# 10XGenomics/thermite

Measured on AMD Instinct MI355X. Metric: aligned reads/sec (91 bp), higher is better.
Workload: dtype i32

## Files before the change

### thermite_amd/capi.py

```python
import ctypes as C
import os

import numpy as np

from .refdata import EXON_DT, REF_DT, SPAN_DT, TX_DT

_HERE = os.path.dirname(os.path.abspath(__file__))
SO_PATH = os.environ.get("THM_LIB") or os.path.join(_HERE, "_build", "libthermite_amd.so")

MEM_DT = np.dtype([("ref_idx", "<u8"), ("query_idx", "<u4"), ("len", "<u4")])
ALN_DT = np.dtype(
    [
        ("ystart", "<u8"),
        ("yend", "<u8"),
        ("ylen", "<u8"),
        ("ops_off", "<u8"),
        ("tx_ystart", "<u8"),
        ("tx_yend", "<u8"),
        ("tx_ylen", "<u8"),
        ("tx_ops_off", "<u8"),
        ("score", "<i4"),
        ("ref_id", "<u4"),
        ("xstart", "<u4"),
        ("xend", "<u4"),
# ... 142 lines not shown
        return _lib
    if not os.path.exists(SO_PATH):
        raise ThermiteError(ERR_INTERNAL, "HIP library not built: %s is missing (run __graft_entry__.build())" % SO_PATH)
    L = C.CDLL(SO_PATH)
    vp, u64, i32, u32 = C.c_void_p, C.c_uint64, C.c_int32, C.c_uint32
    L.thm_index_create_in_memory.restype = i32
    L.thm_index_create_in_memory.argtypes = [vp, u64, vp, u32, vp, u32, vp, u64, vp, u64, vp, u32, vp, u32, vp, vp]
    L.thm_index_create_in_memory_ex.restype = i32
    L.thm_index_create_in_memory_ex.argtypes = [vp, u64, vp, u32, vp, u32, vp, u64, vp, u64, vp, u32, vp, u32, vp, u32, u32, vp]
    L.thm_index_coord_bytes.restype = u32
    L.thm_index_coord_bytes.argtypes = [vp]
    L.thm_index_suffix_array64.restype = vp
    L.thm_index_suffix_array64.argtypes = [vp]
    L.thm_build_suffix_array64.restype = i32
    L.thm_build_suffix_array64.argtypes = [vp, u64, vp]
    L.thm_build_suffix_array_gpu.restype = i32
    L.thm_build_suffix_array_gpu.argtypes = [vp, u64, vp, u32]
    if hasattr(L, "thm_debug_check_lut"):
        L.thm_debug_check_lut.restype = i32
        L.thm_debug_check_lut.argtypes = [vp]
    if hasattr(L, "thm_debug_host_lut"):
        L.thm_debug_host_lut.restype = i32
        L.thm_debug_host_lut.argtypes = [vp, vp, vp, u64]
    L.thm_index_free.argtypes = [vp]
    L.thm_index_text_len.restype = u64
    L.thm_index_text_len.argtypes = [vp]
    L.thm_index_suffix_array.restype = vp
    L.thm_index_suffix_array.argtypes = [vp]
    L.thm_index_idx_to_ref.restype = i32
    L.thm_index_idx_to_ref.argtypes = [vp, u64, vp]
    L.thm_build_suffix_array.restype = i32
    L.thm_build_suffix_array.argtypes = [vp, u64, vp]
    L.thm_aligner_create.restype = i32
    L.thm_aligner_create.argtypes = [vp, vp, i32, vp]
    L.thm_aligner_free.argtypes = [vp]
    L.thm_last_error.restype = C.c_char_p
    L.thm_last_error.argtypes = [vp]
    L.thm_aligner_set_opts.restype = i32
    L.thm_aligner_set_opts.argtypes = [vp, vp]
    L.thm_aligner_stream.restype = vp
    L.thm_aligner_stream.argtypes = [vp]
    L.thm_align_batch.restype = i32
    L.thm_align_batch.argtypes = [vp, vp, vp, u64, vp]
    L.thm_batch_upload.restype = i32
    L.thm_batch_upload.argtypes = [vp, vp, vp, u64]
    for f in ("thm_batch_run", "thm_batch_sync", "thm_counters_reset"):
        getattr(L, f).restype = i32
        getattr(L, f).argtypes = [vp]
    L.thm_batch_fetch.restype = i32
    L.thm_batch_fetch.argtypes = [vp, vp]
    L.thm_batch_fetch_cigars.restype = i32
    L.thm_batch_fetch_cigars.argtypes = [vp, vp]
    L.thm_align_batch_cigars.restype = i32
    L.thm_align_batch_cigars.argtypes = [vp, vp, vp, u64, vp]
    L.thm_cigar_encode_batch.restype = i32
    L.thm_cigar_encode_batch.argtypes = [vp, vp, vp, u64, vp]
    L.thm_smems_batch.restype = i32
    L.thm_smems_batch.argtypes = [vp, vp, vp, u64, u64, vp]
    L.thm_swg_extend_batch.restype = i32
    L.thm_swg_extend_batch.argtypes = [vp, vp, vp, vp, vp, vp, vp, u32, u64, vp]
    L.thm_counters_get.restype = i32
    L.thm_extend_left_right_batch.restype = i32
    L.thm_extend_left_right_batch.argtypes = [vp, vp, vp, vp, vp, vp, vp, vp, u32, u64, vp]
    L.thm_align_seed_hits_batch.restype = i32
    L.thm_align_seed_hits_batch.argtypes = [vp, vp, vp, u64, vp, vp, u64, vp, vp, u32, vp]
    L.thm_counters_get.argtypes = [vp, vp]
    L.thm_counters_device_ptr.restype = vp
    L.thm_counters_device_ptr.argtypes = [vp]
    L.thm_timings_get.restype = i32
    L.thm_timings_get.argtypes = [vp, vp]
    L.thm_version.restype = C.c_char_p
    L.thm_device_count.restype = i32
    L.thm_aligner_index.restype = vp
    L.thm_aligner_index.argtypes = [vp]
    L.thm_comm_unique_id.restype = i32
    L.thm_comm_unique_id.argtypes = [vp]
    L.thm_comm_create.restype = i32
    L.thm_comm_create.argtypes = [vp, i32, i32, i32, vp]
    L.thm_comm_free.argtypes = [vp]
    L.thm_counters_allreduce.restype = i32
    L.thm_counters_allreduce.argtypes = [vp, vp]
    cp = C.c_char_p
    L.thm_index_create_from_files.restype = i32
    L.thm_index_create_from_files.argtypes = [cp, cp, vp]
    L.thm_index_set_names.restype = i32
    L.thm_index_set_names.argtypes = [vp, vp, u32, vp, u32, vp, vp, u32]
    L.thm_index_save.restype = i32
    L.thm_index_save.argtypes = [vp, cp]
    L.thm_index_load.restype = i32
    L.thm_index_load.argtypes = [cp, vp]
    L.thm_index_tables.restype = i32
    L.thm_index_tables.argtypes = [vp, vp]
    for f in ("thm_index_contig_name", "thm_index_tx_id", "thm_index_gene_id", "thm_index_gene_name"):
        getattr(L, f).restype = cp
        getattr(L, f).argtypes = [vp, u32]
    L.thm_fastq_open.restype = i32
    L.thm_fastq_open.argtypes = [cp, vp]
    L.thm_fastq_next_batch.restype = i32
    L.thm_fastq_next_batch.argtypes = [vp, u64, vp]
    L.thm_fastq_close.argtypes = [vp]
    if hasattr(L, "thm_debug_deflate_block"):
        L.thm_debug_deflate_block.restype = i32
        L.thm_debug_deflate_block.argtypes = [vp, u64, vp, u64, C.POINTER(u64)]
    if hasattr(L, "thm_debug_gunzip_mt"):
        L.thm_debug_gunzip_mt.restype = i32
        L.thm_debug_gunzip_mt.argtypes = [C.c_char_p, u64, u32, vp, u64, C.POINTER(u64)]
    if hasattr(L, "thm_debug_gunzip"):
        L.thm_debug_gunzip.restype = i32
        L.thm_debug_gunzip.argtypes = [C.c_char_p, u64, vp, u64, C.POINTER(u64)]
    if hasattr(L, "thm_debug_fastq_blocks"):
        L.thm_debug_fastq_blocks.restype = i32
        L.thm_debug_fastq_blocks.argtypes = [vp, u64, vp]
    L.thm_writer_create.restype = i32
    L.thm_writer_create.argtypes = [vp, i32, u32, vp]
    L.thm_writer_free.argtypes = [vp]
    L.thm_writer_header.restype = i32
    L.thm_writer_header.argtypes = [vp, vp]
    L.thm_writer_trailer.restype = i32
    L.thm_writer_trailer.argtypes = [vp, vp]
    L.thm_writer_format_batch.restype = i32
    L.thm_writer_format_batch.argtypes = [vp, vp, vp, vp]
    L.thm_writer_format_batch_cigars.restype = i32
    L.thm_writer_format_batch_cigars.argtypes = [vp, vp, vp, vp]
    L.thm_batch_upload_reads.restype = i32
    L.thm_batch_upload_reads.argtypes = [vp, vp]
    L.thm_batch_fetch_bam.restype = i32
    L.thm_batch_fetch_bam.argtypes = [vp, u32, vp]
    L.thm_align_batch_bam.restype = i32
    L.thm_align_batch_bam.argtypes = [vp, vp, u32, vp]
    L.thm_batch_fetch_bgzf.restype = i32
    L.thm_batch_fetch_bgzf.argtypes = [vp, u32, vp]
    L.thm_align_batch_bgzf.restype = i32
    L.thm_align_batch_bgzf.argtypes = [vp, vp, u32, vp]
    L.thm_debug_bgzf_device.restype = i32
    L.thm_debug_bgzf_device.argtypes = [vp, vp, u64, vp, u64, vp, vp]
    L.thm_batch_upload_fastq.restype = i32
    L.thm_batch_upload_fastq.argtypes = [vp, vp, u64, cp, u64, i32, vp]
    L.thm_batch_fetch_reads.restype = i32
    L.thm_batch_fetch_reads.argtypes = [vp, vp]
    L.thm_debug_fastq_device_blocks.restype = i32
    L.thm_debug_fastq_device_blocks.argtypes = [vp, vp, vp]
    L.thm_writer_wrap_bam.restype = i32
    L.thm_writer_wrap_bam.argtypes = [vp, vp, vp]
    L.thm_align_files.restype = i32
    L.thm_align_files.argtypes = [vp, vp, u32, cp, i32, u64, u32, vp]
    L.thm_align_files_multi.restype = i32
    L.thm_align_files_multi.argtypes = [vp, u32, vp, u32, cp, i32, u64, u32, vp]
    if hasattr(L, "thm_debug_prof_get"):
        L.thm_debug_prof_get.restype = i32
        L.thm_debug_prof_get.argtypes = [vp, vp, i32]
    if hasattr(L, "thm_debug_set_pool_caps"):
        L.thm_debug_set_pool_caps.restype = i32
        L.thm_debug_set_pool_caps.argtypes = [vp, u64, u64, u64, vp]
    if hasattr(L, "thm_debug_set_flags"):
        L.thm_debug_set_flags.restype = i32
        L.thm_debug_set_flags.argtypes = [vp, C.c_uint32]
        L.thm_debug_set_band_clip.restype = i32
        L.thm_debug_set_band_clip.argtypes = [vp, C.c_uint32]
        L.thm_debug_tpr_stats.restype = i32
        L.thm_debug_tpr_stats.argtypes = [vp, vp]
    if hasattr(L, "thm_debug_seed_stats"):
        L.thm_debug_seed_stats.restype = i32
        L.thm_debug_seed_stats.argtypes = [vp, vp]
    if hasattr(L, "thm_debug_seed_direct_stats"):
        L.thm_debug_seed_direct_stats.restype = i32
        L.thm_debug_seed_direct_stats.argtypes = [vp, vp]
    if hasattr(L, "thm_debug_fetch_lut"):
        L.thm_debug_fetch_lut.restype = i32
        L.thm_debug_fetch_lut.argtypes = [vp, vp, u64]
    if hasattr(L, "thm_debug_knobs"):
        L.thm_debug_knobs.restype = i32
        L.thm_debug_knobs.argtypes = [vp, vp]
    if hasattr(L, "thm_debug_calib_gather"):
        L.thm_debug_calib_gather.restype = i32
        L.thm_debug_calib_gather.argtypes = [vp, i32, u64, vp]
    if hasattr(L, "thm_debug_wave_prims"):
        L.thm_debug_wave_prims.restype = i32
        L.thm_debug_wave_prims.argtypes = [vp, vp, vp]
    _lib = L
    return L


def _ptr(a):
    return a.ctypes.data_as(C.c_void_p) if a is not None else None


def _copy(ptr, count, dtype, copy=True):
    if count == 0 or not ptr:
        return np.zeros(0, dtype=dtype)
    nbytes = int(count) * np.dtype(dtype).itemsize
    buf = (C.c_uint8 * nbytes).from_address(ptr)
    a = np.frombuffer(buf, dtype=dtype, count=int(count))
    return a.copy() if copy else a


def _u8(b):
    if isinstance(b, np.ndarray):
        return np.ascontiguousarray(b, np.uint8)
    return np.frombuffer(bytes(b), np.uint8)


def build_suffix_array_gpu(text, wide=False):
    text = np.ascontiguousarray(text, np.uint8)
    out = np.empty(len(text), "<u8" if wide else "<u4")
    rc = lib().thm_build_suffix_array_gpu(_ptr(text), len(text), _ptr(out), 8 if wide else 4)
    if rc != 0:
        raise ThermiteError(rc, _last_error())
    return out


def build_suffix_array(text, wide=False):
    t = _u8(text)
    sa = np.zeros(len(t), "<u8" if wide else "<u4")
    f = lib().thm_build_suffix_array64 if wide else lib().thm_build_suffix_array
    rc = f(_ptr(t), len(t), _ptr(sa))
    if rc != 0:
        raise ThermiteError(rc, "thm_build_suffix_array")
    return sa


INDEX_WIDE = 1


class TablesView(C.Structure):
    _fields_ = [("n_text", C.c_uint64), ("text", C.c_void_p), ("n_refs", C.c_uint32), ("refs", C.c_void_p),
                ("n_txs", C.c_uint32), ("txs", C.c_void_p), ("n_exons", C.c_uint64), ("exons", C.c_void_p),
                ("n_tx_seq", C.c_uint64), ("tx_seq", C.c_void_p), ("n_genes", C.c_uint32), ("genes", C.c_void_p),
                ("name_rank", C.c_void_p), ("n_contigs", C.c_uint32)]


class ReadBatch(C.Structure):

    _fields_ = [("n_reads", C.c_uint64), ("n_bases", C.c_uint64), ("bases", C.c_void_p), ("offsets", C.c_void_p),
                ("quals", C.c_void_p), ("names", C.c_void_p), ("name_off", C.c_void_p)]


class Text(C.Structure):
    _fields_ = [("data", C.c_void_p), ("len", C.c_uint64)]


class RunStats(C.Structure):
    _fields_ = [("n_reads", C.c_uint64), ("n_aligned_reads", C.c_uint64), ("n_records", C.c_uint64),
                ("n_batches", C.c_uint64), ("n_output_bytes", C.c_uint64), ("parse_s", C.c_double),
                ("gpu_s", C.c_double), ("format_s", C.c_double), ("write_s", C.c_double), ("wall_s", C.c_double)]


def _last_error(h=None):
    return (lib().thm_last_error(h) or b"").decode()


def _cstr_array(strs):
    arr = (C.c_char_p * len(strs))(*[s.encode() if isinstance(s, str) else bytes(s) for s in strs])
    return arr


class Index:

    @classmethod
    def _wrap(cls, h):
        self = cls.__new__(cls)
        self.h = h
        self.tables = None
        return self

    @classmethod
    def from_files(cls, fasta_path, gtf_path):
        h = C.c_void_p()
        rc = lib().thm_index_create_from_files(str(fasta_path).encode(), str(gtf_path).encode(), C.byref(h))
        if rc != 0:
            raise ThermiteError(rc, _last_error())
        return cls._wrap(h)

    @classmethod
    def load(cls, path):
        h = C.c_void_p()
        rc = lib().thm_index_load(str(path).encode(), C.byref(h))
        if rc != 0:
            raise ThermiteError(rc, _last_error())
        return cls._wrap(h)

    def save(self, path):
        rc = lib().thm_index_save(self.h, str(path).encode())
        if rc != 0:
            raise ThermiteError(rc, _last_error())

    def set_names(self, contig_names, tx_ids, gene_ids, gene_names):
        a, b, c, d = (_cstr_array(x) for x in (contig_names, tx_ids, gene_ids, gene_names))
        rc = lib().thm_index_set_names(self.h, a, len(contig_names), b, len(tx_ids), c, d, len(gene_ids))
        if rc != 0:
            raise ThermiteError(rc, _last_error())

    def native_tables(self):
        v = TablesView()
        rc = lib().thm_index_tables(self.h, C.byref(v))
        if rc != 0:
            raise ThermiteError(rc, "thm_index_tables")
        L = lib()
        dec = lambda f, n: [f(self.h, i).decode() for i in range(n)]
        names = dec(L.thm_index_contig_name, v.n_contigs)
        refs = _copy(v.refs, v.n_refs, REF_DT)
        rank_per_ref = _copy(v.name_rank, v.n_refs, "<u4")
        name_rank = np.zeros(v.n_contigs, "<u4")
        if v.n_contigs:
            name_rank[refs["name_id"]] = rank_per_ref
        have = v.n_contigs > 0
        return dict(
            text=_copy(v.text, v.n_text, np.uint8), refs=refs, names=names, name_rank=name_rank,
            txs=_copy(v.txs, v.n_txs, TX_DT), exons=_copy(v.exons, v.n_exons, EXON_DT),
            tx_seq=_copy(v.tx_seq, v.n_tx_seq, np.uint8), genes=_copy(v.genes, v.n_genes, SPAN_DT),
            gene_ids=dec(L.thm_index_gene_id, v.n_genes) if have else [],
            gene_names=dec(L.thm_index_gene_name, v.n_genes) if have else [],
            tx_ids=dec(L.thm_index_tx_id, v.n_txs) if have else [],
        )

    def __init__(self, tables, sa=None, wide=False):
        t = tables
        self.tables = t
        h = C.c_void_p()
        sa_arr, sa_bytes = None, 0
        if sa is not None:
            sa_bytes = 8 if np.asarray(sa).dtype.itemsize == 8 else 4
            sa_arr = np.ascontiguousarray(sa, "<u8" if sa_bytes == 8 else "<u4")
        rc = lib().thm_index_create_in_memory_ex(
            _ptr(t["text"]), len(t["text"]), _ptr(t["refs"]), len(t["refs"]), _ptr(t["txs"]), len(t["txs"]),
            _ptr(t["exons"]), len(t["exons"]), _ptr(t["tx_seq"]), len(t["tx_seq"]), _ptr(t["genes"]), len(t["genes"]),
            _ptr(t["name_rank"]), len(t["name_rank"]), _ptr(sa_arr), sa_bytes, INDEX_WIDE if wide else 0, C.byref(h),
        )
        if rc != 0:
            raise ThermiteError(rc, (lib().thm_last_error(None) or b"").decode())
        self.h = h
        if t.get("names") and "tx_ids" in t:
            self.set_names(t["names"], t["tx_ids"], t["gene_ids"], t["gene_names"])

    @property
    def coord_bytes(self):
        return lib().thm_index_coord_bytes(self.h)

    def suffix_array(self):
        n = lib().thm_index_text_len(self.h)
        if self.coord_bytes == 8:
            return _copy(lib().thm_index_suffix_array64(self.h), n, "<u8")
        return _copy(lib().thm_index_suffix_array(self.h), n, "<u4")

    def check_lut(self):
        return lib().thm_debug_check_lut(self.h) == 0

    def debug_host_lut(self):
        kt = C.c_uint32()
        if lib().thm_debug_host_lut(self.h, C.byref(kt), None, 0) != 0:
            raise ThermiteError(ERR_INTERNAL, "thm_debug_host_lut")
        out = np.zeros((4 ** kt.value, 2), "<u8" if self.coord_bytes == 8 else "<u4")
        if lib().thm_debug_host_lut(self.h, C.byref(kt), _ptr(out), out.nbytes) != 0:
            raise ThermiteError(ERR_INTERNAL, "thm_debug_host_lut")
        return out

    def idx_to_ref(self, idx):
        off = C.c_uint64()
        r = lib().thm_index_idx_to_ref(self.h, idx, C.byref(off))
        if r < 0:
            raise ThermiteError(r, "idx_to_ref")
        return r, off.value

    def close(self):
        if getattr(self, "h", None):
            lib().thm_index_free(self.h)
            self.h = None

    def __del__(self):
        self.close()


class BatchResult:

    def __init__(self, view, copy=True):
        self.n_reads = view.n_reads
        self.offsets = _copy(view.read_aln_off, view.n_reads + 1, "<u8", copy)
        self.alns = _copy(view.alns, view.n_alns, ALN_DT, copy)
        self.ops = _copy(view.ops, view.n_op_bytes, np.uint8, copy)
        self.n_failed = view.n_failed_reads
        self.status = _copy(view.read_status, view.n_reads, "<i4", copy) if view.read_status else None


class CigarResult:

    def __init__(self, view, copy=True):
        self.n_reads = view.n_reads
        self.offsets = _copy(view.read_aln_off, view.n_reads + 1, "<u8", copy) if view.read_aln_off else None
        self.alns = _copy(view.alns, view.n_alns, ALN_DT, copy) if view.alns else None
        self.digests = _copy(view.digests, view.n_alns, DIGEST_DT, copy)
        self.cigar = _copy(view.cigar, view.n_cigar_words, "<u4", copy)
        self.n_failed = view.n_failed_reads
        self.status = _copy(view.read_status, view.n_reads, "<i4", copy) if view.read_status else None

    @property
    def nbytes(self):
        return sum(a.nbytes for a in (self.offsets, self.alns, self.digests, self.cigar, self.status) if a is not None)

    def words(self, i, tx=False):
        d = self.digests[i]
        o = int(d["cigar_off"]) + (int(d["n_cigar"]) if tx else 0)
        return self.cigar[o: o + int(d["n_tx_cigar"] if tx else d["n_cigar"])]


class BamResult:

    def __init__(self, view, copy=True):
        self.n_reads = view.n_reads
        self.n_records = view.n_records
        self.data = _copy(view.data, view.n_bytes, np.uint8, copy)
        self.read_rec_off = _copy(view.read_rec_off, view.n_reads + 1, "<u8", copy)
        self.n_failed = view.n_failed_reads
        self.status = _copy(view.read_status, view.n_reads, "<i4", copy) if view.read_status else None

    @property
    def nbytes(self):
        return sum(a.nbytes for a in (self.data, self.read_rec_off, self.status) if a is not None)

    def records(self, r):
        b = self.data[int(self.read_rec_off[r]): int(self.read_rec_off[r + 1])].tobytes()
        out, at = [], 0
        while at < len(b):
            n = 4 + int.from_bytes(b[at: at + 4], "little")
            out.append(b[at: at + n])
            at += n
        return out


class BgzfResult:

    def __init__(self, view, copy=True):
        self.n_reads = view.n_reads
        self.n_records = view.n_records
        self.n_raw_bytes = view.n_raw_bytes
        self.n_blocks = view.n_blocks
        self.data = _copy(view.data, view.n_bytes, np.uint8, copy)
        self.block_off = _copy(view.block_off, view.n_blocks + 1, "<u8", copy)
        self.n_failed = view.n_failed_reads
        self.status = _copy(view.read_status, view.n_reads, "<i4", copy) if view.read_status else None

    @property
    def nbytes(self):
        return sum(a.nbytes for a in (self.data, self.block_off, self.status) if a is not None)

    def block(self, b):
        return self.data[int(self.block_off[b]): int(self.block_off[b + 1])].tobytes()


def cigar_text(words):
    return "".join("%d%s" % (int(w) >> 4, "MIDNSHP=X"[int(w) & 15]) for w in words) or "*"


class Aligner:

    def __init__(self, index, opts=None, device=0):
        self.index = index
        o = dict(DEFAULT_OPTS)
        o.update(opts or {})
        self._opts = self._mk(o)
        h = C.c_void_p()
        rc = lib().thm_aligner_create(index.h, C.byref(self._opts), device, C.byref(h))
        if rc != 0:
            raise ThermiteError(rc, (lib().thm_last_error(None) or b"").decode())
        self.h = h

    @staticmethod
    def _mk(o):
        return Opts(o["min_seed_len"], o["min_aln_score_percent"], o["min_aln_score"], o["multimap_score_range"],
                    int(bool(o["intron_mode"])), 0)

    def _chk(self, rc):
        if rc != 0:
            raise ThermiteError(rc, (lib().thm_last_error(self.h) or b"").decode())

    def set_opts(self, opts):
        o = dict(DEFAULT_OPTS)
        o.update(opts)
        self._opts = self._mk(o)
        self._chk(lib().thm_aligner_set_opts(self.h, C.byref(self._opts)))

    @property
    def stream(self):
        return lib().thm_aligner_stream(self.h)

    def align_batch(self, bases, offsets, copy=True):
        bases, offsets = _u8(bases), np.ascontiguousarray(offsets, "<u8")
        v = BatchView()
        self._chk(lib().thm_align_batch(self.h, _ptr(bases), _ptr(offsets), len(offsets) - 1, C.byref(v)))
        return BatchResult(v, copy)

    def upload(self, bases, offsets):
        bases, offsets = _u8(bases), np.ascontiguousarray(offsets, "<u8")
        self._chk(lib().thm_batch_upload(self.h, _ptr(bases), _ptr(offsets), len(offsets) - 1))

    def run(self):
        self._chk(lib().thm_batch_run(self.h))

    def sync(self):
        self._chk(lib().thm_batch_sync(self.h))

    def fetch(self, copy=True):
        v = BatchView()
        self._chk(lib().thm_batch_fetch(self.h, C.byref(v)))
        return BatchResult(v, copy)

    def fetch_cigars(self, copy=True):
        v = CigarView()
        self._chk(lib().thm_batch_fetch_cigars(self.h, C.byref(v)))
        return CigarResult(v, copy)

    def align_batch_cigars(self, bases, offsets, copy=True):
        bases, offsets = _u8(bases), np.ascontiguousarray(offsets, "<u8")
        v = CigarView()
        self._chk(lib().thm_align_batch_cigars(self.h, _ptr(bases), _ptr(offsets), len(offsets) - 1, C.byref(v)))
        return CigarResult(v, copy)

    def upload_reads(self, batch):
        rb, keep = read_batch_struct(batch)
        self._chk(lib().thm_batch_upload_reads(self.h, C.byref(rb)))

    def fetch_bam(self, flags=0, copy=True):
        v = BamView()
        self._chk(lib().thm_batch_fetch_bam(self.h, flags, C.byref(v)))
        return BamResult(v, copy)

    def align_batch_bam(self, batch, flags=0, copy=True):
        rb, keep = read_batch_struct(batch)
        v = BamView()
        self._chk(lib().thm_align_batch_bam(self.h, C.byref(rb), flags, C.byref(v)))
        return BamResult(v, copy)

    def fetch_bgzf(self, flags=0, copy=True):
        v = BgzfView()
        self._chk(lib().thm_batch_fetch_bgzf(self.h, flags, C.byref(v)))
        return BgzfResult(v, copy)

    def align_batch_bgzf(self, batch, flags=0, copy=True):
        rb, keep = read_batch_struct(batch)
        v = BgzfView()
        self._chk(lib().thm_align_batch_bgzf(self.h, C.byref(rb), flags, C.byref(v)))
        return BgzfResult(v, copy)

    def upload_fastq(self, raw, path=b"", first_line=1, last_block=True):
        src = np.frombuffer(bytes(raw), np.uint8) if len(raw) else None
        info = FastqUploadInfo()
        self._chk(lib().thm_batch_upload_fastq(self.h, _ptr(src), len(raw), os.fsencode(path), first_line, int(bool(last_block)),
                                               C.byref(info)))
        return {k: getattr(info, k) for k, _ in FastqUploadInfo._fields_}

    def fetch_reads(self):
        v = ReadBatch()
        self._chk(lib().thm_batch_fetch_reads(self.h, C.byref(v)))
        off = _copy(v.offsets, v.n_reads + 1, "<u8")
        noff = _copy(v.name_off, v.n_reads + 1, "<u8")
        return dict(bases=_copy(v.bases, v.n_bases, np.uint8), offsets=off,
                    quals=_copy(v.quals, v.n_bases, np.uint8) if v.quals else None,
                    names=_copy(v.names, int(noff[-1]), np.uint8), name_off=noff)

    def debug_fastq_device_blocks(self):
        d, h = C.c_uint64(0), C.c_uint64(0)
        self._chk(lib().thm_debug_fastq_device_blocks(self.h, C.byref(d), C.byref(h)))
        return d.value, h.value

    def debug_bgzf_device(self, data):
        src = np.frombuffer(bytes(data), np.uint8) if len(data) else np.zeros(1, np.uint8)
        out = np.empty(len(data) + 31 * (len(data) // 0xff00 + 1) + 64, np.uint8)
        n, nb = C.c_uint64(0), C.c_uint64(0)
        self._chk(lib().thm_debug_bgzf_device(self.h, src.ctypes.data, len(data), out.ctypes.data, len(out), C.byref(n), C.byref(nb)))
        return out[: n.value].tobytes(), nb.value

    def cigar_encode_batch(self, ops, off):
        ops, off = _u8(ops), np.ascontiguousarray(off, "<u8")
        v = CigarView()
        self._chk(lib().thm_cigar_encode_batch(self.h, _ptr(ops), _ptr(off), len(off) - 1, C.byref(v)))
        return CigarResult(v)

    def smems_batch(self, bases, offsets, min_seed_len):
        bases, offsets = _u8(bases), np.ascontiguousarray(offsets, "<u8")
        v = MemsView()
        self._chk(lib().thm_smems_batch(self.h, _ptr(bases), _ptr(offsets), len(offsets) - 1, min_seed_len, C.byref(v)))
        return _copy(v.read_mem_off, v.n_reads + 1, "<u8"), _copy(v.mems, v.n_mems, MEM_DT)

    def swg_extend_batch(self, x_bases, x_off, y_bases, y_off, bw, xd, max_bw):
        xb, yb = _u8(x_bases), _u8(y_bases)
        xo, yo = np.ascontiguousarray(x_off, "<u8"), np.ascontiguousarray(y_off, "<u8")
        bw, xd = np.ascontiguousarray(bw, "<u4"), np.ascontiguousarray(xd, "<i4")
        v = SwgView()
        self._chk(lib().thm_swg_extend_batch(self.h, _ptr(xb), _ptr(xo), _ptr(yb), _ptr(yo), _ptr(bw), _ptr(xd),
                                             max_bw, len(bw), C.byref(v)))
        return _copy(v.alns, v.n, SWG_DT), _copy(v.ops, v.n_op_bytes, np.uint8)

    def extend_left_right_batch(self, x_bases, x_off, y_bases, y_off, hits, bw, xd, max_bw):
        xb, yb = _u8(x_bases), _u8(y_bases)
        xo, yo = np.ascontiguousarray(x_off, "<u8"), np.ascontiguousarray(y_off, "<u8")
        hits = np.ascontiguousarray(hits, MEM_DT)
        bw, xd = np.ascontiguousarray(bw, "<u4"), np.ascontiguousarray(xd, "<i4")
        v = LrView()
        self._chk(lib().thm_extend_left_right_batch(self.h, _ptr(xb), _ptr(xo), _ptr(yb), _ptr(yo), _ptr(hits), _ptr(bw),
                                                    _ptr(xd), max_bw, len(bw), C.byref(v)))
        return _copy(v.alns, v.n, LR_DT), _copy(v.ops, v.n_op_bytes, np.uint8)

    def align_seed_hits(self, bases, offsets, hit_off, hits, band_width, x_drop, max_band_width):
        bases, offsets = _u8(bases), np.ascontiguousarray(offsets, "<u8")
        hit_off, hits = np.ascontiguousarray(hit_off, "<u8"), np.ascontiguousarray(hits, MEM_DT)
        bw, xd = np.ascontiguousarray(band_width, "<u4"), np.ascontiguousarray(x_drop, "<i4")
        if not (len(hits) == len(bw) == len(xd)):
            raise ThermiteError(ERR_INVALID_ARG, "hits, band_width and x_drop differ in length")
        v = HitsView()
        self._chk(lib().thm_align_seed_hits_batch(self.h, _ptr(bases), _ptr(offsets), len(offsets) - 1, _ptr(hit_off),
                                                  _ptr(hits), len(hits), _ptr(bw), _ptr(xd), max_band_width, C.byref(v)))
        status = (_copy(v.hit_status, v.n_hits, "<i4") if v.hit_status else np.zeros(int(v.n_hits), "<i4"))
        return _copy(v.alns, v.n_hits, ALN_DT), _copy(v.ops, v.n_op_bytes, np.uint8), status

    def counters(self):
        out = np.zeros(N_COUNTERS, "<u8")
        self._chk(lib().thm_counters_get(self.h, _ptr(out)))
        return out

    def reset_counters(self):
        self._chk(lib().thm_counters_reset(self.h))

    def counters_allreduce(self, comm):
        self._chk(lib().thm_counters_allreduce(self.h, comm.h))

    def counters_device_ptr(self):
        return lib().thm_counters_device_ptr(self.h)

    def timings(self):
        out = np.zeros(N_TIMINGS, "<f4")
        self._chk(lib().thm_timings_get(self.h, _ptr(out)))
        return dict(zip(TIMING_NAMES, out.tolist()))

    def debug_prof(self, reset=True):
        out = np.zeros(16, "<u8")
        self._chk(lib().thm_debug_prof_get(self.h, _ptr(out), int(reset)))
        return out

    def debug_set_pool_caps(self, smem_cap=0, cand_cap=0, ops_cap=0):
        n = C.c_uint32()
        self._chk(lib().thm_debug_set_pool_caps(self.h, smem_cap, cand_cap, ops_cap, C.byref(n)))
        return n.value

    def debug_set_flags(self, tpr=None, rounds=0, seed_infer=None, seed_stats=None, seed_direct=None):
        word = (0 if tpr is None else (2 if tpr else 1)) | (int(rounds) << 8)
        word |= 0 if seed_infer is None else (16 if seed_infer else 4)
        word |= 0 if seed_stats is None else (8 if seed_stats else 32)
        word |= 0 if seed_direct is None else (128 if seed_direct else 64)
        self._chk(lib().thm_debug_set_flags(self.h, word))

    def debug_seed_stats(self):
        out = np.zeros(2, "<u8")
        self._chk(lib().thm_debug_seed_stats(self.h, _ptr(out)))
        return int(out[0]), int(out[1])

    def debug_seed_direct_stats(self):
        out = np.zeros(4, "<u8")
        self._chk(lib().thm_debug_seed_direct_stats(self.h, _ptr(out)))
        return tuple(int(x) for x in out)

    def debug_fetch_lut(self, like):
        out = np.zeros_like(like)
        self._chk(lib().thm_debug_fetch_lut(self.h, _ptr(out), out.nbytes))
        return out

    def debug_set_band_clip(self, max_bw=None):
        self._chk(lib().thm_debug_set_band_clip(self.h, 0 if max_bw is None else int(max_bw) + 1))

    def debug_tpr_stats(self):
        out = np.zeros(32, "<u8")
        self._chk(lib().thm_debug_tpr_stats(self.h, _ptr(out)))
        return out

    def debug_knobs(self):
        out = np.zeros(16, "<u4")
        self._chk(lib().thm_debug_knobs(self.h, _ptr(out)))
        return out

    def debug_calib_gather(self, pattern, n_threads):
        b = C.c_uint64()
        self._chk(lib().thm_debug_calib_gather(self.h, pattern, n_threads, C.byref(b)))
        return b.value

    def debug_wave_prims(self, v):
        v = np.ascontiguousarray(v, "<i4")
        out = np.zeros(384, "<i4")
        self._chk(lib().thm_debug_wave_prims(self.h, _ptr(v), _ptr(out)))
        return out.reshape(6, 64)

    def close(self):
        if getattr(self, "h", None):
            lib().thm_aligner_free(self.h)
            self.h = None

    def __del__(self):
        self.close()


KNOB_NAMES = {0: "seed_fill", 1: "compact_k", 2: "hit_gl", 11: "team_div_per_cu", 12: "swg_bpc", 13: "use_tpr", 14: "tpr_rounds",
              15: "n_cu"}


def knobs_dict(raw):
    d = {name: int(raw[i]) for i, name in KNOB_NAMES.items()}
    d["ext_minw"] = {(cpl, bool(wide)): int(raw[3 + 2 * (cpl - 1) + wide]) for cpl in (1, 2, 3, 4) for wide in (0, 1)}
    return d


def comm_unique_id():
    out = np.zeros(128, np.uint8)
    rc = lib().thm_comm_unique_id(_ptr(out))
    if rc != 0:
        raise ThermiteError(rc, _last_error())
    return out


class Comm:

    def __init__(self, unique_id, nranks, rank, device=0):
        uid = np.ascontiguousarray(unique_id, np.uint8)
        h = C.c_void_p()
        rc = lib().thm_comm_create(_ptr(uid), nranks, rank, device, C.byref(h))
        if rc != 0:
            raise ThermiteError(rc, _last_error())
        self.h = h

    def close(self):
        if getattr(self, "h", None):
            lib().thm_comm_free(self.h)
            self.h = None

    def __del__(self):
        self.close()


def debug_deflate_block(data):
    src = np.frombuffer(bytes(data), np.uint8) if len(data) else np.zeros(1, np.uint8)
    out = np.empty(len(data) + len(data) // 8 + 1024, np.uint8)
    n = C.c_uint64(0)
    rc = lib().thm_debug_deflate_block(src.ctypes.data, len(data), out.ctypes.data, len(out), C.byref(n))
    if rc != 0:
        raise ThermiteError(rc, _last_error())
    return out[: n.value].tobytes()


def debug_gunzip(path, chunk=1 << 20, cap=None, threads=1):
    cap = cap if cap is not None else 64 * os.path.getsize(path) + (1 << 20)
    out = np.empty(cap, np.uint8)
    n = C.c_uint64(0)
    rc = lib().thm_debug_gunzip_mt(os.fsencode(str(path)), chunk, threads, out.ctypes.data, cap, C.byref(n))
    if rc != 0:
        raise ThermiteError(rc, _last_error())
    return out[: n.value].tobytes()


class FastqReader:

    def __init__(self, path):
        h = C.c_void_p()
        rc = lib().thm_fastq_open(str(path).encode(), C.byref(h))
        if rc != 0:
            raise ThermiteError(rc, _last_error())
        self.h = h

    def all_by_blocks(self, reads_per_block):
        v = ReadBatch()
        rc = lib().thm_debug_fastq_blocks(self.h, reads_per_block, C.byref(v))
        if rc != 0:
            raise ThermiteError(rc, _last_error())
        off = _copy(v.offsets, v.n_reads + 1, "<u8")
        noff = _copy(v.name_off, v.n_reads + 1, "<u8")
        return dict(bases=_copy(v.bases, v.n_bases, np.uint8), offsets=off, quals=_copy(v.quals, v.n_bases, np.uint8),
                    names=_copy(v.names, int(noff[-1]), np.uint8), name_off=noff)

    def next_batch(self, max_reads):
        v = ReadBatch()
        rc = lib().thm_fastq_next_batch(self.h, max_reads, C.byref(v))
        if rc != 0:
            raise ThermiteError(rc, _last_error())
        if v.n_reads == 0:
            return None
        off = _copy(v.offsets, v.n_reads + 1, "<u8")
        noff = _copy(v.name_off, v.n_reads + 1, "<u8")
        return dict(bases=_copy(v.bases, v.n_bases, np.uint8), offsets=off,
                    quals=_copy(v.quals, v.n_bases, np.uint8) if v.quals else None,
                    names=_copy(v.names, int(noff[-1]), np.uint8), name_off=noff)

    def close(self):
        if getattr(self, "h", None):
            lib().thm_fastq_close(self.h)
            self.h = None

    def __del__(self):
        self.close()


def read_batch_struct(batch):
    keep = [_u8(batch["bases"]), np.ascontiguousarray(batch["offsets"], "<u8"),
            None if batch.get("quals") is None else _u8(batch["quals"]), _u8(batch["names"]),
            np.ascontiguousarray(batch["name_off"], "<u8")]
    rb = ReadBatch(len(keep[1]) - 1, len(keep[0]), _ptr(keep[0]), _ptr(keep[1]), _ptr(keep[2]), _ptr(keep[3]), _ptr(keep[4]))
    return rb, keep


class Writer:

    def __init__(self, index, fmt=FMT_SAM, n_threads=1):
# ... 73 lines not shown
```

### thermite_amd/csrc/aligner.hip

```cpp
#include <hip/hip_runtime.h>

#include <algorithm>
#include <cstdarg>
#include <cstdio>
#include <cstdlib>
#include <cstring>
#include <mutex>
#include <string>
#include <type_traits>
#include <vector>

#include "aligner_internal.h"
#include "lut_direct.h"

namespace thm {
const char* global_error_cstr();
}
using namespace thm;

static int swg_blocks_per_cu() {
  static const int v = [] {
    const char* e = getenv("THM_SWG_BPC");
    const int v = e ? atoi(e) : 4;
    return (v >= 1 && v <= 8) ? v : 4;
// ... 65 lines not shown
    const bool tag = lut_direct_wanted() && (ix->wide ? lutd::can_tag<uint64_t>(ix->n) : lutd::can_tag<uint32_t>(ix->n)) &&
                     (ix->wide ? !ix->lut64.empty() : !ix->lut.empty());
    if (tag) {
      if (e == hipSuccess) e = d->lut_cnt.ensure(16);
      if (e == hipSuccess) e = hipMemsetAsync(d->lut_cnt.p, 0, 16, s);
      if (e == hipSuccess)
        e = ix->wide ? launch_lut_tag(d->lut.as<LutEntryT<uint64_t>>(), d->sa.as<uint64_t>(), ix->lut64.size(), ix->n,
                                      d->lut_cnt.as<unsigned long long>(), s)
                     : launch_lut_tag(d->lut.as<LutEntryT<uint32_t>>(), d->sa.as<uint32_t>(), ix->lut.size(), ix->n,
                                      d->lut_cnt.as<unsigned long long>(), s);
      if (e == hipSuccess) e = hipMemcpyAsync(&d->lut_tagged, d->lut_cnt.p, 8, hipMemcpyDeviceToHost, s);
      d->lut_direct = true;
    }
    if (e == hipSuccess) e = hipStreamSynchronize(s);
    if (e != hipSuccess) {
      free_dev_copy(d);
      return fail(a, e == hipErrorOutOfMemory ? THM_ERR_OOM : THM_ERR_HIP, "index upload failed: %s",
                  hipGetErrorString(e));
    }
    auto fill_view = [&](auto& v) {
      typedef typename std::remove_reference<decltype(v)>::type::coord_t C;
      v.text = d->text.as<uint8_t>() + 16;
      v.sa = d->sa.as<C>();
      v.lut = d->lut.as<LutEntryT<C>>();
      v.refs = d->refs.as<thm_ref>();
      v.name_rank = d->name_rank.as<uint32_t>();
      v.ref_recs = d->ref_recs.as<RefRecT<C>>();
      v.ref_bin = d->ref_bin.as<uint32_t>();
      v.txs = d->txs.as<thm_tx>();
      v.exons = d->exons.as<thm_exon>();
      v.exon_txoff = d->exon_txoff.as<uint64_t>();
      v.tx_seq = d->tx_seq.as<uint8_t>() + 16;
      v.exon_grid_off = d->exon_grid_off.as<uint32_t>();
      v.exon_grid = d->exon_grid.as<ExonEntryT<C>>();
      v.gene_grid_off = d->gene_grid_off.as<uint32_t>();
      v.gene_grid = d->gene_grid.as<GridEntryT<C>>();
      v.n = ix->n;
      v.n_refs = (uint32_t)ix->refs.size();
      v.n_txs = (uint32_t)ix->txs.size();
      v.kt = ix->kt;
      v.max_tx_exons = ix->max_tx_exons;
      v.lut_direct = d->lut_direct ? 1u : 0u;
    };
    memset(&d->view, 0, sizeof d->view);
    memset(&d->view64, 0, sizeof d->view64);
    if (ix->wide)
      fill_view(d->view64);
    else
      fill_view(d->view);
    ix->dev[a->device] = d;
  }
  a->dix = ix->dev[a->device];
  return THM_OK;
}

int reset_queue(thm_aligner* a) {
  HIPCHK(a, hipMemsetAsync(a->d_queue.p, 0, thm::QUEUE_BYTES, a->stream));
  HIPCHK(a, hipMemsetAsync(a->d_fault.p, 0, 64, a->stream));
  return THM_OK;
}

int grid_blocks(const thm_aligner* a, uint64_t n_items, int waves_per_block, int blocks_per_cu) {
  uint64_t need = (n_items + waves_per_block - 1) / waves_per_block;
  uint64_t cap = (uint64_t)a->n_cu * blocks_per_cu;
  return (int)std::max<uint64_t>(1, std::min(need, cap));
}

extern "C" {

const char* thm_version(void) { return "thermite_amd 0.1 (gfx950)"; }

int32_t thm_device_count(void) {
  int n = 0;
  if (hipGetDeviceCount(&n) != hipSuccess) return 0;
  return n;
}

void thm_index_free(thm_index* ix) {
  if (!ix) return;
  for (auto* d : ix->dev) free_dev_copy(d);
  delete (std::mutex*)ix->dev_mu;
  delete ix;
}

const char* thm_last_error(const thm_aligner* a) { return a ? a->err.c_str() : global_error_cstr(); }

int32_t thm_aligner_create(const thm_index* ix, const thm_align_opts* opts, int32_t device_id, thm_aligner** out) {
  if (!out) return THM_ERR_INVALID_ARG;
  *out = nullptr;
  if (!ix || !opts) return fail(nullptr, THM_ERR_INVALID_ARG, "thm_aligner_create: null index or opts");
  int n = 0;
  if (hipGetDeviceCount(&n) != hipSuccess || n <= 0)
    return fail(nullptr, THM_ERR_NO_DEVICE, "no HIP device visible: the MI355X path has no CPU fallback");
  if (device_id < 0 || device_id >= n) return fail(nullptr, THM_ERR_NO_DEVICE, "device id %d out of range", device_id);
  thm_aligner* a = new thm_aligner();
  a->ix = ix;
  a->device = device_id;
  a->opts = *opts;
  {
    const char* e = getenv("THM_TPR");
    if (e && e[0] == '0') a->use_tpr = false;
    if (e && e[0] == '1') a->use_tpr = true;
    e = getenv("THM_TPR_ROUNDS");
    if (e && atoi(e) >= 1 && atoi(e) <= TPR_MAX_ROUNDS) a->tpr_rounds = atoi(e);
  }
  auto bail = [&](int code) {
    thm_aligner_free(a);
    return code;
  };
  if (hipSetDevice(device_id) != hipSuccess) return bail(fail(nullptr, THM_ERR_HIP, "hipSetDevice failed"));
  hipDeviceProp_t prop;
  if (hipGetDeviceProperties(&prop, device_id) == hipSuccess) a->n_cu = prop.multiProcessorCount;
  if (hipStreamCreateWithFlags(&a->stream, hipStreamNonBlocking) != hipSuccess)
    return bail(fail(nullptr, THM_ERR_HIP, "hipStreamCreate failed"));
  for (auto& e : a->ev)
    if (hipEventCreate(&e) != hipSuccess) return bail(fail(nullptr, THM_ERR_HIP, "hipEventCreate failed"));
  if (hipStreamCreateWithFlags(&a->stream2, hipStreamNonBlocking) != hipSuccess ||
      hipStreamCreateWithFlags(&a->stream3, hipStreamNonBlocking) != hipSuccess ||
      hipStreamCreateWithFlags(&a->stream4, hipStreamNonBlocking) != hipSuccess ||
      hipEventCreateWithFlags(&a->ev_dpt_fork, hipEventDisableTiming) != hipSuccess ||
      hipEventCreateWithFlags(&a->ev_dpt_join, hipEventDisableTiming) != hipSuccess ||
      hipEventCreateWithFlags(&a->ev_join3, hipEventDisableTiming) != hipSuccess ||
      hipEventCreateWithFlags(&a->ev_fork, hipEventDisableTiming) != hipSuccess ||
      hipEventCreateWithFlags(&a->ev_join, hipEventDisableTiming) != hipSuccess)
    return bail(fail(nullptr, THM_ERR_HIP, "second stream / events: creation failed"));
  if (a->d_counters.ensure(THM_N_COUNTERS * 8 * 3) != hipSuccess || a->d_ctl.ensure(thm_aligner::CTL_BYTES) != hipSuccess)
    return bail(fail(nullptr, THM_ERR_OOM, "scratch allocation failed"));
  {
    uint8_t* ctl = a->d_ctl.as<uint8_t>();
    a->s_work_counts = {ctl + thm_aligner::CTL_WORK_COUNTS, 128};
    a->d_cursors = {ctl + thm_aligner::CTL_CURSORS, 64};
    a->d_fault = {ctl + thm_aligner::CTL_FAULT, 64};
    a->d_queue = {ctl + thm_aligner::CTL_QUEUE, thm::QUEUE_BYTES};
    a->d_queue_ext = {ctl + thm_aligner::CTL_QUEUE_EXT, thm::QUEUE_BYTES};
  }
  (void)hipMemsetAsync(a->d_counters.p, 0, THM_N_COUNTERS * 8 * 3, a->stream);
  (void)hipMemsetAsync(a->d_ctl.p, 0, thm_aligner::CTL_BYTES, a->stream);
  int rc = get_dev_copy(a);
  if (rc != THM_OK) return bail(rc);
  rc = thm_aligner_set_opts(a, opts);
  if (rc != THM_OK) return bail(rc);
  *out = a;
  return THM_OK;
}

void thm_aligner_free(thm_aligner* a) {
  if (!a) return;
  (void)hipSetDevice(a->device);
  if (a->stream) (void)hipStreamSynchronize(a->stream);
  if (a->stream2) (void)hipStreamSynchronize(a->stream2);
  if (a->stream3) (void)hipStreamSynchronize(a->stream3);
  if (a->stream4) (void)hipStreamSynchronize(a->stream4);
  DBuf* all[] = {&a->d_counters, &a->d_ctl, &a->b0, &a->b1, &a->b2, &a->b3, &a->b4,
                 &a->b5, &a->b6, &a->b7, &a->b8, &a->r_bases, &a->r_offsets, &a->r_san, &a->s_ms_end, &a->s_ms_lo, &a->s_ms_hi, &a->s_work_reads, &a->s_work_long, &a->s_work_cells, &a->s_fill_keys, &a->s_fill_perm, &a->s_fill_hist, &a->s_sel_scratch, &a->s_heavy, &a->s_slow, &a->s_team, &a->r_status, &a->e_slow, &a->e_recs, &a->e_wcnt, &a->t_memos, &a->t_recs, &a->t_dpops, &a->t_qlist, &a->t_act[0], &a->t_act[1], &a->t_ctl, &a->t_bail, &a->t_queue2, &a->t_trace, &a->t_ttrace, &a->t_hdr, &a->t_sums, &a->s_smems, &a->s_off, &a->s_cnt,
                 &a->s_hits, &a->s_cand_off, &a->scan_tmp, &a->e_cands, &a->e_heavy, &a->e_rel, &a->e_order, &a->e_ops, &a->e_nalns,
                 &a->e_opbytes, &a->e_aln_off, &a->e_ops_off, &a->e_trace, &a->o_alns, &a->o_ops, &a->o_mems,
                 &a->sh_bases, &a->sh_san, &a->sh_off, &a->sh_hits, &a->sh_read, &a->sh_bw, &a->sh_xd, &a->sh_list, &a->sh_out,
                 &a->sh_status, &a->sh_ops, &a->sh_ctl, &a->sh_trace, &a->sh_slow, &a->c_sums, &a->c_nwords, &a->c_woff,
                 &a->c_scan_tmp, &a->c_flags, &a->c_dig, &a->c_words, &a->c_in_ops, &a->c_in_off,
                 &a->bn_names, &a->bn_name_off, &a->bn_quals, &a->bt_tx_pool, &a->bt_tx_off, &a->bt_gid_pool, &a->bt_gid_off,
                 &a->bt_gname_pool, &a->bt_gname_off, &a->bt_tx_gene, &a->bt_ref_sq, &a->bm_cnt, &a->bm_first, &a->bm_qn,
                 &a->bm_rec_read, &a->bm_len, &a->bm_off, &a->bm_out, &a->bm_read_off, &a->bm_err, &a->bm_scan_tmp,
                 &a->bz_match, &a->bz_slots, &a->bz_sizes, &a->bz_off, &a->bz_out, &a->bz_scan_tmp, &a->bz_dbg_in,
                 &a->fq_raw, &a->fq_cnt, &a->fq_base, &a->fq_lines, &a->fq_name_len, &a->fq_seq_len, &a->fq_flag, &a->fq_scan_tmp};
  for (DBuf* b : all) b->release();
  for (int k = 0; k < 2; k++) {
    a->r_off[k].release();
    a->r_alns[k].release();
    a->r_ops[k].release();
    a->r_stat[k].release();
    a->ch_off[k].release();
    a->ch_alns[k].release();
    a->ch_dig[k].release();
    a->ch_words[k].release();
    a->ch_stat[k].release();
    a->bh_data[k].release();
    a->bh_off[k].release();
    a->bh_stat[k].release();
    a->zh_data[k].release();
    a->zh_off[k].release();
    a->zh_stat[k].release();
  }
  HBuf* pinned[] = {&a->fq_h_off, &a->fr_bases, &a->fr_off, &a->fr_quals, &a->fr_names, &a->fr_name_off};
  for (HBuf* b : pinned) b->release();
  for (auto& e : a->ev_fq)
    if (e) (void)hipEventDestroy(e);
  for (auto& e : a->ev_cig)
    if (e) (void)hipEventDestroy(e);
  for (auto& e : a->ev_bam)
    if (e) (void)hipEventDestroy(e);
  for (auto& e : a->ev_bgzf)
    if (e) (void)hipEventDestroy(e);
  for (auto& e : a->ev)
    if (e) (void)hipEventDestroy(e);
  if (a->ev_fork) (void)hipEventDestroy(a->ev_fork);
  if (a->ev_join) (void)hipEventDestroy(a->ev_join);
  if (a->ev_join3) (void)hipEventDestroy(a->ev_join3);
  if (a->ev_dpt_fork) (void)hipEventDestroy(a->ev_dpt_fork);
  if (a->ev_dpt_join) (void)hipEventDestroy(a->ev_dpt_join);
  if (a->stream4) (void)hipStreamDestroy(a->stream4);
  if (a->stream3) (void)hipStreamDestroy(a->stream3);
  if (a->stream2) (void)hipStreamDestroy(a->stream2);
  if (a->stream) (void)hipStreamDestroy(a->stream);
  delete a;
}

int32_t thm_aligner_set_opts(thm_aligner* a, const thm_align_opts* o) {
  if (!a || !o) return THM_ERR_INVALID_ARG;
  if (o->min_seed_len < 1 || o->min_seed_len > 65535) return fail(a, THM_ERR_INVALID_ARG, "min_seed_len out of range");
  if (!(o->min_aln_score_percent >= 0.0f && o->min_aln_score_percent <= 1.0f))
    return fail(a, THM_ERR_INVALID_ARG, "min_aln_score_percent must be within [0,1] (src/main.rs:46-49)");
  a->opts = *o;
  return THM_OK;
}

void* thm_aligner_stream(thm_aligner* a) { return a ? (void*)a->stream : nullptr; }

const thm_index* thm_aligner_index(const thm_aligner* a) { return a ? a->ix : nullptr; }

int32_t thm_counters_get(thm_aligner* a, uint64_t out[THM_N_COUNTERS]) {
  if (!a || !out) return THM_ERR_INVALID_ARG;
  HIPCHK(a, hipSetDevice(a->device));
  HIPCHK(a, hipMemcpyAsync(out, a->d_counters.p, THM_N_COUNTERS * 8, hipMemcpyDeviceToHost, a->stream));
  HIPCHK(a, hipStreamSynchronize(a->stream));
  return THM_OK;
}
int32_t thm_counters_reset(thm_aligner* a) {
  if (!a) return THM_ERR_INVALID_ARG;
  HIPCHK(a, hipSetDevice(a->device));
  HIPCHK(a, hipMemsetAsync(a->d_counters.p, 0, THM_N_COUNTERS * 8, a->stream));
  return THM_OK;
}
void* thm_counters_device_ptr(thm_aligner* a) { return a ? a->d_counters.p : nullptr; }

int32_t thm_timings_get(thm_aligner* a, float out[THM_N_TIMINGS]) {
  if (!a || !out) return THM_ERR_INVALID_ARG;
  memcpy(out, a->timings, sizeof(a->timings));
  return THM_OK;
}

int32_t thm_swg_extend_batch(thm_aligner* a, const uint8_t* x_bases, const uint64_t* x_off, const uint8_t* y_bases,
                             const uint64_t* y_off, const uint32_t* band_width, const int32_t* x_drop,
                             uint32_t max_band_width, uint64_t n, thm_swg_view* out) {
  if (!a || !out || !x_off || !y_off || !band_width || !x_drop) return THM_ERR_INVALID_ARG;
  memset(out, 0, sizeof(*out));
  if (n == 0) return THM_OK;
  if (n >= 0xFFFFFFFFull) return fail(a, THM_ERR_UNSUPPORTED, "more than 2^32-1 problems in one call");
  HIPCHK(a, hipSetDevice(a->device));
  uint32_t bw_max = 0, x_max = 0, y_max = 0;
  std::vector<uint64_t> ops_off(n + 1, 0);
  for (uint64_t i = 0; i < n; i++) {
    if (band_width[i] > max_band_width)
      return fail(a, THM_ERR_OUT_OF_CONTRACT, "problem %llu: band_width %u > max_band_width %u (src/swg.rs:32)",
                  (unsigned long long)i, band_width[i], max_band_width);
    if (x_drop[i] < (int64_t)band_width[i])
      return fail(a, THM_ERR_OUT_OF_CONTRACT, "problem %llu: x_drop < band_width is undefined in the reference",
                  (unsigned long long)i);
    uint64_t xl = x_off[i + 1] - x_off[i], yl = y_off[i + 1] - y_off[i];
    if (x_off[i + 1] < x_off[i] || y_off[i + 1] < y_off[i]) return fail(a, THM_ERR_INVALID_ARG, "offsets not monotone");
    if (xl > MAX_READ_LEN || band_width[i] > 2 * MAX_READ_LEN)
      return fail(a, THM_ERR_UNSUPPORTED, "x longer than %u or band wider than +-%u", MAX_READ_LEN, 2 * MAX_READ_LEN);
    uint64_t cols = std::min<uint64_t>(yl, xl + band_width[i] + 1);
    bw_max = std::max(bw_max, band_width[i]);
    x_max = std::max<uint32_t>(x_max, (uint32_t)xl);
    y_max = std::max<uint32_t>(y_max, (uint32_t)cols);
    ops_off[i + 1] = ops_off[i] + xl + cols + 8;
  }
  int cpl = (int)((2 * bw_max + 1 + 63) / 64);
  SwgBatchParams p;
  p.x_cap = (x_max + 15u) & ~15u;
  p.y_cap = (y_max + 15u) & ~15u;
  if (p.x_cap == 0) p.x_cap = 16;
  if (p.y_cap == 0) p.y_cap = 16;
  p.max_bw = bw_max;
  p.scratch = nullptr;
  p.scratch_per_wave = 0;
  if (cpl > 4 || swg_batch_lds_bytes(p, cpl) > EXTEND_LDS_LIMIT) cpl = 0;
  const uint64_t xb_n = x_off[n], yb_n = y_off[n], pool = ops_off[n];
  HIPCHK(a, a->b0.ensure(xb_n + 16));
  HIPCHK(a, a->b1.ensure((n + 1) * 8));
  HIPCHK(a, a->b2.ensure(yb_n + 16));
  HIPCHK(a, a->b3.ensure((n + 1) * 8));
  HIPCHK(a, a->b4.ensure(n * 4));
  HIPCHK(a, a->b5.ensure(n * 4));
  HIPCHK(a, a->b6.ensure((n + 1) * 8));
  HIPCHK(a, a->b7.ensure(pool + 16));
  HIPCHK(a, a->b8.ensure(n * sizeof(thm_swg_aln)));
  hipStream_t s = a->stream;
  if (xb_n) HIPCHK(a, hipMemcpyAsync(a->b0.p, x_bases, xb_n, hipMemcpyHostToDevice, s));
  HIPCHK(a, hipMemcpyAsync(a->b1.p, x_off, (n + 1) * 8, hipMemcpyHostToDevice, s));
  if (yb_n) HIPCHK(a, hipMemcpyAsync(a->b2.p, y_bases, yb_n, hipMemcpyHostToDevice, s));
  HIPCHK(a, hipMemcpyAsync(a->b3.p, y_off, (n + 1) * 8, hipMemcpyHostToDevice, s));
  HIPCHK(a, hipMemcpyAsync(a->b4.p, band_width, n * 4, hipMemcpyHostToDevice, s));
  HIPCHK(a, hipMemcpyAsync(a->b5.p, x_drop, n * 4, hipMemcpyHostToDevice, s));
  HIPCHK(a, hipMemcpyAsync(a->b6.p, ops_off.data(), (n + 1) * 8, hipMemcpyHostToDevice, s));
  int rc = reset_queue(a);
  if (rc != THM_OK) return rc;
  p.xb = a->b0.as<uint8_t>();
  p.xo = a->b1.as<uint64_t>();
  p.yb = a->b2.as<uint8_t>();
  p.yo = a->b3.as<uint64_t>();
  p.bw = a->b4.as<uint32_t>();
  p.xd = a->b5.as<int32_t>();
  p.ops_off = a->b6.as<uint64_t>();
  p.ops = a->b7.as<uint8_t>();
  p.out = a->b8.as<thm_swg_aln>();
  p.counters = a->d_counters.as<unsigned long long>();
// ... 36 lines not shown
  return THM_OK;
}

int32_t thm_extend_left_right_batch(thm_aligner* a, const uint8_t* x_bases, const uint64_t* x_off, const uint8_t* y_bases,
                                    const uint64_t* y_off, const thm_mem* hits, const uint32_t* band_width,
                                    const int32_t* x_drop, uint32_t max_band_width, uint64_t n, thm_lr_view* out) {
  if (!a || !out || !x_off || !y_off || !hits || !band_width || !x_drop) return THM_ERR_INVALID_ARG;
  memset(out, 0, sizeof(*out));
  if (n == 0) return THM_OK;
  if (n >= 0xFFFFFFFFull) return fail(a, THM_ERR_UNSUPPORTED, "more than 2^32-1 problems in one call");
  if ((!x_bases && x_off[n] > 0) || (!y_bases && y_off[n] > 0)) return THM_ERR_INVALID_ARG;
  HIPCHK(a, hipSetDevice(a->device));
  uint32_t bw_max = 0, x_max = 0, y_max = 0;
  std::vector<uint64_t> ops_off(n + 1, 0);
  for (uint64_t i = 0; i < n; i++) {
    if (x_off[i + 1] < x_off[i] || y_off[i + 1] < y_off[i]) return fail(a, THM_ERR_INVALID_ARG, "offsets not monotone");
    const uint64_t xl = x_off[i + 1] - x_off[i], yl = y_off[i + 1] - y_off[i];
    const thm_mem& h = hits[i];
    if (band_width[i] > max_band_width)
      return fail(a, THM_ERR_OUT_OF_CONTRACT, "problem %llu: band_width %u > max_band_width %u (src/swg.rs:32)",
                  (unsigned long long)i, band_width[i], max_band_width);
    if (x_drop[i] < (int64_t)band_width[i])
      return fail(a, THM_ERR_OUT_OF_CONTRACT, "problem %llu: x_drop < band_width is undefined in the reference",
                  (unsigned long long)i);
    if ((uint64_t)h.query_idx + h.len > xl)
      return fail(a, THM_ERR_OUT_OF_CONTRACT, "problem %llu: query_idx + len > read length (src/aligner.rs:360)",
                  (unsigned long long)i);
    if (h.ref_idx > yl || h.ref_idx + h.len > yl)
      return fail(a, THM_ERR_OUT_OF_CONTRACT, "problem %llu: ref_idx + len > reference length (src/aligner.rs:361)",
                  (unsigned long long)i);
    if (xl > MAX_READ_LEN || band_width[i] > 2 * MAX_READ_LEN)
      return fail(a, THM_ERR_UNSUPPORTED, "read longer than %u or band wider than +-%u", MAX_READ_LEN, 2 * MAX_READ_LEN);
    const uint64_t xr = xl - (h.query_idx + h.len), xlft = h.query_idx;
    const uint64_t yr = std::min<uint64_t>(yl - (h.ref_idx + h.len), xr + band_width[i] + 1);
    const uint64_t ylft = std::min<uint64_t>(std::min<uint64_t>(h.ref_idx, xl + band_width[i]), xlft + band_width[i] + 1);
    bw_max = std::max(bw_max, band_width[i]);
    x_max = std::max<uint32_t>(x_max, (uint32_t)std::max(xr, xlft));
    y_max = std::max<uint32_t>(y_max, (uint32_t)std::max(yr, ylft));
    ops_off[i + 1] = ops_off[i] + xr + yr + xlft + ylft + h.len + 16;
  }
  int cpl = (int)((2 * bw_max + 1 + 63) / 64);
  ElrBatchParams p;
  p.x_cap = (x_max + 15u) & ~15u;
  p.y_cap = (y_max + 15u) & ~15u;
  if (p.x_cap == 0) p.x_cap = 16;
  if (p.y_cap == 0) p.y_cap = 16;
  p.max_bw = bw_max;
  p.scratch = nullptr;
  p.scratch_per_wave = 0;
  if (cpl > 4 || elr_batch_lds_bytes(p, cpl) > EXTEND_LDS_LIMIT) cpl = 0;
  const uint64_t xb_n = x_off[n], yb_n = y_off[n], pool = ops_off[n];
  HIPCHK(a, a->b0.ensure(xb_n + 16));
  HIPCHK(a, a->b1.ensure((n + 1) * 8));
  HIPCHK(a, a->b2.ensure(yb_n + 16));
  HIPCHK(a, a->b3.ensure((n + 1) * 8));
  HIPCHK(a, a->b4.ensure(n * 4));
  HIPCHK(a, a->b5.ensure(n * 4));
  HIPCHK(a, a->b6.ensure((n + 1) * 8));
  HIPCHK(a, a->b7.ensure(pool + 16));
  HIPCHK(a, a->b8.ensure(n * sizeof(thm_lr_aln)));
  HIPCHK(a, a->sh_hits.ensure(n * sizeof(thm_mem)));
  hipStream_t s = a->stream;
  if (xb_n) HIPCHK(a, hipMemcpyAsync(a->b0.p, x_bases, xb_n, hipMemcpyHostToDevice, s));
  HIPCHK(a, hipMemcpyAsync(a->b1.p, x_off, (n + 1) * 8, hipMemcpyHostToDevice, s));
  if (yb_n) HIPCHK(a, hipMemcpyAsync(a->b2.p, y_bases, yb_n, hipMemcpyHostToDevice, s));
  HIPCHK(a, hipMemcpyAsync(a->b3.p, y_off, (n + 1) * 8, hipMemcpyHostToDevice, s));
  HIPCHK(a, hipMemcpyAsync(a->b4.p, band_width, n * 4, hipMemcpyHostToDevice, s));
  HIPCHK(a, hipMemcpyAsync(a->b5.p, x_drop, n * 4, hipMemcpyHostToDevice, s));
  HIPCHK(a, hipMemcpyAsync(a->b6.p, ops_off.data(), (n + 1) * 8, hipMemcpyHostToDevice, s));
  HIPCHK(a, hipMemcpyAsync(a->sh_hits.p, hits, n * sizeof(thm_mem), hipMemcpyHostToDevice, s));
  int rc = reset_queue(a);
  if (rc != THM_OK) return rc;
  p.xb = a->b0.as<uint8_t>();
  p.xo = a->b1.as<uint64_t>();
  p.yb = a->b2.as<uint8_t>();
  p.yo = a->b3.as<uint64_t>();
  p.hits = a->sh_hits.as<thm_mem>();
  p.bw = a->b4.as<uint32_t>();
  p.xd = a->b5.as<int32_t>();
  p.ops_off = a->b6.as<uint64_t>();
  p.ops = a->b7.as<uint8_t>();
  p.out = a->b8.as<thm_lr_aln>();
  p.counters = a->d_counters.as<unsigned long long>();
  p.queue = a->d_queue.as<unsigned int>();
  p.fault = a->d_fault.as<int>();
  p.n = n;
  int n_blocks = grid_blocks(a, n, 4, 4);
  if (cpl == 0) {
    p.scratch_per_wave = (elr_batch_scratch_bytes(p) + 255) & ~255ull;
    const uint64_t budget = 16ull << 30;
    if (p.scratch_per_wave > budget) return fail(a, THM_ERR_UNSUPPORTED, "DP trace of %llu bytes per problem exceeds the device-memory budget",
                                                 (unsigned long long)p.scratch_per_wave);
    n_blocks = (int)std::max<uint64_t>(1, std::min<uint64_t>((uint64_t)n_blocks, budget / p.scratch_per_wave / 4));
    HIPCHK(a, a->e_slow.ensure((size_t)n_blocks * 4 * p.scratch_per_wave + 256));
    p.scratch = a->e_slow.as<uint8_t>();
  }
  HIPCHK(a, launch_elr_batch(p, cpl, n_blocks, s));
  std::vector<thm_lr_aln> raw(n);
  std::vector<uint8_t> pool_h(pool);
  int fault = 0;
  HIPCHK(a, hipMemcpyAsync(raw.data(), a->b8.p, n * sizeof(thm_lr_aln), hipMemcpyDeviceToHost, s));
  if (pool) HIPCHK(a, hipMemcpyAsync(pool_h.data(), a->b7.p, pool, hipMemcpyDeviceToHost, s));
  HIPCHK(a, hipMemcpyAsync(&fault, a->d_fault.p, 4, hipMemcpyDeviceToHost, s));
  HIPCHK(a, hipStreamSynchronize(s));
  if (fault) return fail(a, THM_ERR_INTERNAL, "inconsistent trace in elr_batch_kernel");
  a->h_lr.resize(n);
  a->h_ops.clear();
  for (uint64_t i = 0; i < n; i++) {
    thm_lr_aln r = raw[i];
    const uint64_t off = a->h_ops.size();
    a->h_ops.insert(a->h_ops.end(), pool_h.begin() + r.ops_off, pool_h.begin() + r.ops_off + r.ops_len);
    r.ops_off = off;
    a->h_lr[i] = r;
  }
  out->n = n;
  out->n_op_bytes = a->h_ops.size();
  out->alns = a->h_lr.data();
  out->ops = a->h_ops.data();
  return THM_OK;
}

int32_t thm_debug_prof_get(thm_aligner* a, uint64_t out[16], int32_t reset) {
  if (!a || !out) return THM_ERR_INVALID_ARG;
  HIPCHK(a, hipSetDevice(a->device));
  uint8_t* p = a->d_counters.as<uint8_t>() + 2 * THM_N_COUNTERS * 8;
  HIPCHK(a, hipMemcpyAsync(out, p, 16 * 8, hipMemcpyDeviceToHost, a->stream));
  if (reset) HIPCHK(a, hipMemsetAsync(p, 0, 16 * 8, a->stream));
  HIPCHK(a, hipStreamSynchronize(a->stream));
  return THM_OK;
}

int32_t thm_debug_set_pool_caps(thm_aligner* a, uint64_t smem_cap, uint64_t cand_cap, uint64_t ops_cap, uint32_t* n_replays) {
  if (!a) return THM_ERR_INVALID_ARG;
  a->dbg_smem_cap = smem_cap;
  a->dbg_cand_cap = cand_cap;
  a->dbg_ops_cap = ops_cap;
  a->smem_cap = a->cand_cap = a->cand_ops_cap = 0;
  if (n_replays) *n_replays = a->n_replays;
  return THM_OK;
}

int32_t thm_debug_set_flags(thm_aligner* a, uint32_t flags) {
  if (!a) return THM_ERR_INVALID_ARG;
  if (flags & 1u) a->use_tpr = false;
  if (flags & 2u) a->use_tpr = true;
  const int r = (int)((flags >> 8) & 15u);
  if (r >= 1 && r <= TPR_MAX_ROUNDS) a->tpr_rounds = r;
  if (flags & 4u) a->dbg_seed_noinfer = true;
  if (flags & 16u) a->dbg_seed_noinfer = false;
  if (flags & 8u) a->dbg_seed_stats = true;
  if (flags & 32u) a->dbg_seed_stats = false;
  if (flags & 64u) a->dbg_seed_nodirect = true;
  if (flags & 128u) a->dbg_seed_nodirect = false;
  return THM_OK;
}
int32_t thm_debug_seed_stats(thm_aligner* a, uint64_t stats[2]) {
  if (!a || !stats) return THM_ERR_INVALID_ARG;
  stats[0] = stats[1] = 0;
  if (!a->s_work_counts.p || a->s_work_counts.cap < 128) return THM_OK;
  HIPCHK(a, hipSetDevice(a->device));
  HIPCHK(a, hipStreamSynchronize(a->stream));
  HIPCHK(a, hipMemcpy(stats, a->s_work_counts.as<unsigned long long>() + 8, 16, hipMemcpyDeviceToHost));
  return THM_OK;
}
int32_t thm_debug_seed_direct_stats(thm_aligner* a, uint64_t stats[4]) {
  if (!a || !stats) return THM_ERR_INVALID_ARG;
  stats[0] = stats[1] = stats[2] = stats[3] = 0;
  if (!a->dix) return THM_OK;
  stats[0] = a->dix->lut_direct ? 1 : 0;
  stats[1] = a->dix->lut_tagged;
  if (!a->s_work_counts.p || a->s_work_counts.cap < 128) return THM_OK;
  HIPCHK(a, hipSetDevice(a->device));
  HIPCHK(a, hipStreamSynchronize(a->stream));
  HIPCHK(a, hipMemcpy(stats + 2, a->s_work_counts.as<unsigned long long>() + 10, 16, hipMemcpyDeviceToHost));
  return THM_OK;
}
int32_t thm_debug_fetch_lut(thm_aligner* a, void* out, uint64_t bytes) {
  if (!a || !out || !a->dix) return THM_ERR_INVALID_ARG;
  const uint64_t have = a->dix->wide ? a->ix->lut64.size() * sizeof(LutEntryT<uint64_t>) : a->ix->lut.size() * sizeof(LutEntryT<uint32_t>);
  if (bytes != have) return fail(a, THM_ERR_INVALID_ARG, "thm_debug_fetch_lut: the table has %llu bytes", (unsigned long long)have);
  HIPCHK(a, hipSetDevice(a->device));
  HIPCHK(a, hipStreamSynchronize(a->stream));
  if (bytes) HIPCHK(a, hipMemcpy(out, a->dix->lut.p, bytes, hipMemcpyDeviceToHost));
  return THM_OK;
}
int32_t thm_debug_set_band_clip(thm_aligner* a, uint32_t max_bw_plus_1) {
  if (!a) return THM_ERR_INVALID_ARG;
  a->dbg_band_clip = max_bw_plus_1;
  return THM_OK;
}
int32_t thm_debug_tpr_stats(thm_aligner* a, uint64_t stats[32]) {
  if (!a || !stats) return THM_ERR_INVALID_ARG;
  memset(stats, 0, 256);
  if (!a->t_ctl.p) return THM_OK;
  HIPCHK(a, hipSetDevice(a->device));
  HIPCHK(a, hipStreamSynchronize(a->stream));
  unsigned long long c[40];
  HIPCHK(a, hipMemcpy(c, a->t_ctl.p, sizeof c, hipMemcpyDeviceToHost));
  for (int k = 0; k < 16; k++) stats[k] = c[TPRC_STATS + k];
  stats[16] = c[TPRC_REC_CUR];
  stats[17] = c[TPRC_Q_CUR];
  for (int k = 0; k < 4; k++) stats[18 + k] = c[TPRC_Q_CUR + 1 + k];
  stats[22] = c[TPRC_N_ACT + a->tpr_rounds + 1];
  return THM_OK;
}
int32_t thm_debug_knobs(thm_aligner* a, uint32_t out[16]) {
  if (!a || !out) return THM_ERR_INVALID_ARG;
  out[0] = seed_fill_mode();
  out[1] = (uint32_t)compact_k();
  out[2] = (uint32_t)hit_gl();
  for (int cpl = 1; cpl <= 4; cpl++)
    for (int wide = 0; wide < 2; wide++) out[3 + 2 * (cpl - 1) + wide] = (uint32_t)extend_waves_per_simd(cpl, wide != 0);
  out[11] = team_div_per_cu();
  out[12] = (uint32_t)swg_blocks_per_cu();
  out[13] = a->use_tpr ? 1u : 0u;
  out[14] = (uint32_t)a->tpr_rounds;
  out[15] = (uint32_t)a->n_cu;
  return THM_OK;
}

int32_t thm_debug_calib_gather(thm_aligner* a, int32_t pattern, uint64_t n_threads, uint64_t* bytes_requested) {
  if (!a || pattern < 0 || pattern > 2) return THM_ERR_INVALID_ARG;
  HIPCHK(a, hipSetDevice(a->device));
  const uint64_t span = a->dix->lut.cap & ~255ull;
  if (span < 4096) return fail(a, THM_ERR_INVALID_ARG, "k-mer table too small for the calibration gather");
  HIPCHK(a, launch_calib_gather(a->dix->lut.as<uint8_t>(), span, n_threads, pattern, a->d_cursors.as<unsigned long long>() + 4, a->stream));
  HIPCHK(a, hipStreamSynchronize(a->stream));
  if (bytes_requested) *bytes_requested = n_threads * (pattern == 0 ? 8 : (pattern == 1 ? 4 : 16));
  return THM_OK;
}

int32_t thm_debug_wave_prims(thm_aligner* a, const int32_t in[64], int32_t out[384]) {
  if (!a || !in || !out) return THM_ERR_INVALID_ARG;
  HIPCHK(a, hipSetDevice(a->device));
  HIPCHK(a, a->b0.ensure(64 * 4));
  HIPCHK(a, a->b1.ensure(384 * 4));
  HIPCHK(a, hipMemcpyAsync(a->b0.p, in, 64 * 4, hipMemcpyHostToDevice, a->stream));
  HIPCHK(a, launch_wave_prims(a->b0.as<int>(), a->b1.as<int>(), a->stream));
  HIPCHK(a, hipMemcpyAsync(out, a->b1.p, 384 * 4, hipMemcpyDeviceToHost, a->stream));
  HIPCHK(a, hipStreamSynchronize(a->stream));
  return THM_OK;
}

}
```

### thermite_amd/csrc/aligner_internal.h

```cpp
#ifndef THERMITE_ALIGNER_INTERNAL_H
#define THERMITE_ALIGNER_INTERNAL_H
#include <hip/hip_runtime.h>

#include <cstdarg>
#include <cstdio>
#include <string>
#include <vector>

#include "launch.h"
#include "thermite_internal.h"

struct DBuf {
  void* p = nullptr;
  size_t cap = 0;
  hipError_t ensure(size_t bytes) {
    if (bytes <= cap) return hipSuccess;
    if (p) (void)hipFree(p);
    p = nullptr;
    cap = 0;
    size_t want = bytes + bytes / 4 + 256;
    hipError_t e = hipMalloc(&p, want);
    if (e == hipSuccess) cap = want;
    return e;
  }
  void release() {
    if (p) (void)hipFree(p);
    p = nullptr;
    cap = 0;
  }
  template <class T>
  T* as() const {
    return (T*)p;
  }
};

struct DView {
  void* p = nullptr;
  size_t cap = 0;
  template <class T>
  T* as() const {
    return (T*)p;
  }
};

struct HBuf {
  void* p = nullptr;
  size_t cap = 0;
  hipError_t ensure(size_t bytes) {
    if (bytes <= cap) return hipSuccess;
    if (p) (void)hipHostFree(p);
    p = nullptr;
    cap = 0;
    size_t want = bytes + bytes / 4 + 4096;
    hipError_t e = hipHostMalloc(&p, want, hipHostMallocDefault);
    if (e == hipSuccess) cap = want;
    return e;
  }
  void release() {
    if (p) (void)hipHostFree(p);
    p = nullptr;
    cap = 0;
  }
  template <class T>
  T* as() const {
    return (T*)p;
  }
};

struct thm_index::DevCopy {
  int device = -1;
  DBuf text, sa, lut, refs, name_rank, ref_recs, ref_bin, txs, exons, exon_txoff, tx_seq, exon_grid_off, exon_grid, gene_grid_off, gene_grid;
  bool wide = false;
  bool lut_direct = false;
  uint64_t lut_tagged = 0;
  DBuf lut_cnt;
  thm::DeviceIndexT<uint32_t> view;
  thm::DeviceIndexT<uint64_t> view64;
};

inline void free_dev_copy(thm_index::DevCopy* d) {
  if (!d) return;
  int cur = 0;
  (void)hipGetDevice(&cur);
  (void)hipSetDevice(d->device);
  DBuf* all[] = {&d->text, &d->sa,         &d->lut,    &d->refs,      &d->name_rank, &d->ref_recs, &d->ref_bin, &d->txs,
                 &d->exons, &d->exon_txoff, &d->tx_seq, &d->exon_grid_off, &d->exon_grid, &d->gene_grid_off, &d->gene_grid, &d->lut_cnt};
  for (DBuf* b : all) b->release();
  (void)hipSetDevice(cur);
  delete d;
}

struct thm_aligner {
  const thm_index* ix = nullptr;
  thm_index::DevCopy* dix = nullptr;
  int device = 0;
  int n_cu = 256;
  hipStream_t stream = nullptr;
  hipStream_t stream2 = nullptr;
  hipStream_t stream3 = nullptr;
  hipEvent_t ev_join3 = nullptr;
  hipStream_t stream4 = nullptr;
  hipEvent_t ev_dpt_fork = nullptr, ev_dpt_join = nullptr;
  hipEvent_t ev_fork = nullptr, ev_join = nullptr;
  thm_align_opts opts;
  std::string err;

  DBuf d_counters;
  DBuf d_ctl;
  static constexpr size_t CTL_WORK_COUNTS = 0, CTL_CURSORS = 128, CTL_FAULT = 192, CTL_QUEUE = 256,
                          CTL_QUEUE_EXT = CTL_QUEUE + thm::QUEUE_BYTES, CTL_BYTES = CTL_QUEUE_EXT + thm::QUEUE_BYTES;
  static_assert(CTL_BYTES % 16 == 0 && thm::QUEUE_BYTES % 16 == 0, "the block is zeroed 16 bytes at a time");
  DView d_queue;
  DView d_queue_ext;
  DView d_fault, d_cursors;
  DView s_work_counts;
  DBuf b0, b1, b2, b3, b4, b5, b6, b7, b8;

  DBuf r_bases, r_offsets, r_san;
  DBuf r_status;
  uint64_t n_reads = 0, n_bases = 0;
  uint32_t max_read_len = 0;
  std::vector<std::pair<uint32_t, uint64_t>> len_hist;
  uint64_t n_over = 0;
  bool uploaded = false;
  DBuf s_smems, s_off, s_cnt, s_hits, s_cand_off, scan_tmp, s_ms_end, s_ms_lo, s_ms_hi, s_work_reads, s_work_long, s_work_cells,
      s_sel_scratch, s_heavy, s_slow, s_team, s_fill_keys, s_fill_perm, s_fill_hist;
  uint64_t smem_cap = 0;
  DBuf e_heavy, e_rel;
  DBuf e_cands, e_order, e_ops, e_nalns, e_opbytes, e_aln_off, e_ops_off, e_trace, e_slow, e_recs, e_wcnt;
  size_t wcnt_clean_cap = 0;
  DBuf t_memos, t_recs, t_dpops, t_qlist, t_act[2], t_ctl, t_bail, t_queue2, t_trace, t_ttrace, t_hdr, t_sums;
  bool use_tpr = false;
  int tpr_rounds = 8;
  uint64_t n_slow_host = 0;
  uint32_t fast_max_len = 0, slow_max_len = 0;
  uint64_t cand_cap = 0, cand_ops_cap = 0;
  DBuf o_alns, o_ops, o_mems;
  uint64_t out_alns_cap = 0, out_ops_cap = 0;
  uint64_t dbg_smem_cap = 0, dbg_cand_cap = 0, dbg_ops_cap = 0;
  uint32_t dbg_band_clip = 0;
  bool dbg_seed_noinfer = false, dbg_seed_stats = false;
  bool dbg_seed_nodirect = false;
  uint32_t n_replays = 0;
  bool ran = false, synced = false;
  hipEvent_t ev[6] = {nullptr, nullptr, nullptr, nullptr, nullptr, nullptr};
  float timings[THM_N_TIMINGS] = {0};

  HBuf r_off[2], r_alns[2], r_ops[2], r_stat[2];
  int r_cur = 0;
  std::vector<uint64_t> h_off;
  std::vector<thm_aln> h_alns;
  std::vector<uint8_t> h_ops;
  std::vector<thm_mem> h_mems;
  std::vector<thm_swg_aln> h_swg;
  std::vector<thm_lr_aln> h_lr;
  DBuf sh_bases, sh_san, sh_off, sh_hits, sh_read, sh_bw, sh_xd, sh_list, sh_out, sh_status, sh_ops, sh_ctl, sh_trace, sh_slow;
  std::vector<thm_aln> h_hit_alns;
  std::vector<int32_t> h_hit_status;
  std::vector<uint8_t> h_hit_ops;
  DBuf c_sums, c_nwords, c_woff, c_scan_tmp, c_flags, c_dig, c_words, c_in_ops, c_in_off;
  HBuf ch_off[2], ch_alns[2], ch_dig[2], ch_words[2], ch_stat[2];
  int c_cur = 0;
  hipEvent_t ev_cig[4] = {nullptr, nullptr, nullptr, nullptr};
  std::vector<thm_aln_digest> h_cig_dig;
  std::vector<uint32_t> h_cig_words;
  DBuf bn_names, bn_name_off, bn_quals;
  bool reads_named = false, reads_have_quals = false;
  DBuf bt_tx_pool, bt_tx_off, bt_gid_pool, bt_gid_off, bt_gname_pool, bt_gname_off, bt_tx_gene, bt_ref_sq;
  bool bam_tables = false;
  DBuf bm_cnt, bm_first, bm_qn, bm_rec_read, bm_len, bm_off, bm_out, bm_read_off, bm_err, bm_scan_tmp;
  HBuf bh_data[2], bh_off[2], bh_stat[2];
  int b_cur = 0;
  int bam_stage = -1;
  hipEvent_t ev_bam[4] = {nullptr, nullptr, nullptr, nullptr};
  DBuf bz_match, bz_slots, bz_sizes, bz_off, bz_out, bz_scan_tmp, bz_dbg_in;
  HBuf zh_data[2], zh_off[2], zh_stat[2];
  int z_cur = 0;
  hipEvent_t ev_bgzf[2] = {nullptr, nullptr};
  DBuf fq_raw, fq_cnt, fq_base, fq_lines, fq_name_len, fq_seq_len, fq_flag, fq_scan_tmp;
  HBuf fq_h_off;
  uint64_t fq_on_device = 0, fq_on_host = 0;
  hipEvent_t ev_fq[6] = {nullptr, nullptr, nullptr, nullptr, nullptr, nullptr};
  HBuf fr_bases, fr_off, fr_quals, fr_names, fr_name_off;
};

inline int fail(thm_aligner* a, int code, const char* fmt, ...) {
  char buf[512];
  va_list ap;
  va_start(ap, fmt);
  vsnprintf(buf, sizeof buf, fmt, ap);
  va_end(ap);
  if (a) a->err = buf;
  thm::set_global_error(buf);
  return code;
}

#define HIPCHK(a, call)                                                                             \
  do {                                                                                              \
    hipError_t e_ = (call);                                                                         \
    if (e_ != hipSuccess)                                                                           \
      return fail(a, e_ == hipErrorOutOfMemory ? THM_ERR_OOM : THM_ERR_HIP, "%s failed: %s (%s:%d)", \
                  #call, hipGetErrorString(e_), __FILE__, __LINE__);                                \
  } while (0)

int run_cigar_passes(thm_aligner* a, thm::CigarParams p, uint64_t n_digests, uint64_t* n_words, unsigned* any_flags);
int cigar_ensure_events(thm_aligner* a);
struct BamOnDevice {
  uint64_t n_reads = 0, n_alns = 0, n_records = 0, n_bytes = 0;
  bool any_failed = false;
};
int bam_records_on_device(thm_aligner* a, uint32_t flags, int timing, BamOnDevice* r);
void bam_failed_reads(const int32_t* st, uint64_t n, uint64_t* n_failed, const int32_t** status);
int batch_length_classes(thm_aligner* a, const uint64_t* offsets, uint64_t n_reads);
int reset_queue(thm_aligner* a);
int grid_blocks(const thm_aligner* a, uint64_t n_items, int waves_per_block, int blocks_per_cu);
uint32_t seed_fill_mode();
unsigned team_div_per_cu();
#endif
```

### thermite_amd/csrc/index.cpp

```cpp
#include <algorithm>
#include <cmath>
#include <cstdio>
#include <chrono>
#include <cstdlib>
#include <cstring>
#include <mutex>
#include <thread>
#include <new>
#include <string>
#include <type_traits>

#include "thermite_internal.h"

namespace thm {

static thread_local std::string g_err;
void set_global_error(const std::string& msg) { g_err = msg; }
const char* global_error_cstr() { return g_err.c_str(); }

template <class C>
bool verify_suffix_array(const uint8_t* text, uint64_t n, const C* sa) {
  if (n == 0) return true;
  std::vector<C> rank(n + 1, 0);
  std::vector<uint8_t> seen(n, 0);
// ... 424 lines not shown
    }
    if (n >= (4u << 20) && !getenv("THM_SA_HOST")) {
      const int grc = build_suffix_array_gpu(text, n, dst.data(), (int)sizeof(C));
      if (grc == 0) {
        sa_on_gpu = true;
        return THM_OK;
      }
      if (getenv("THM_INDEX_TIMING")) fprintf(stderr, "thm_index_create: device suffix sort declined (%d): sorting on the host\n", grc);
    }
    if (sizeof(C) == 4) return build_suffix_array(text, n, (uint32_t*)dst.data()) == 0 ? THM_OK : THM_ERR_UNSUPPORTED;
    return build_suffix_array64(text, n, (uint64_t*)dst.data()) == 0 ? THM_OK : THM_ERR_UNSUPPORTED;
  };
  const bool timing = getenv("THM_INDEX_TIMING") != nullptr;
  auto now = [] { return std::chrono::steady_clock::now(); };
  auto lap = [&](const char* what, std::chrono::steady_clock::time_point& t0) {
    const auto t1 = now();
    if (timing) fprintf(stderr, "thm_index_create: %-28s %8.2f s\n", what, std::chrono::duration<double>(t1 - t0).count());
    t0 = t1;
  };
  auto t_phase = now();
  const int src = wide ? fill_sa(ix->sa64) : fill_sa(ix->sa);
  if (src != THM_OK) {
    delete ix;
    return src;
  }
  lap(sa ? "suffix array (checked)" : sa_on_gpu ? "suffix array (GPU)" : "suffix array (SA-IS)", t_phase);
  if (wide)
    build_lut<uint64_t>(ix, ix->lut64);
  else
    build_lut<uint32_t>(ix, ix->lut);
  lap("k-mer table", t_phase);

  {
    Avl a;
    int32_t root = -1;
    for (uint32_t t = 0; t < n_txs; t++) {
      const thm_tx& tx = ix->txs[t];
      for (uint32_t k = 0; k < tx.n_exons; k++) {
        uint32_t e = tx.strand ? k : tx.n_exons - 1 - k;
        const thm_exon& x = ix->exons[tx.exon_begin + e];
        root = a.insert(root, x.start, x.end, x.tx_idx);
        ix->exon_node_exon.push_back((uint32_t)(tx.exon_begin + e));
      }
    }
    ix->exon_tree.swap(a.nd);
    ix->exon_root = root;
  }
  {
    Avl a;
    int32_t root = -1;
    for (uint32_t g = 0; g < n_genes; g++) root = a.insert(root, genes[g].start, genes[g].end, g);
    ix->gene_tree.swap(a.nd);
    ix->gene_root = root;
  }
  if (wide) {
    build_exon_grid<uint64_t>(ix, ix->exon_grid_off, ix->exon_grid64);
    build_grid<uint64_t>(ix->gene_tree, ix->gene_root, n, ix->gene_grid_off, ix->gene_grid64);
  } else {
    build_exon_grid<uint32_t>(ix, ix->exon_grid_off, ix->exon_grid);
    build_grid<uint32_t>(ix->gene_tree, ix->gene_root, n, ix->gene_grid_off, ix->gene_grid);
  }
  lap("interval trees and grids", t_phase);
  {
    const uint64_t nbins = (n >> GRID_SHIFT) + 1;
    ix->ref_bin.assign(nbins, 0);
    uint32_t r = 0;
    for (uint64_t b = 0; b < nbins; b++) {
      const uint64_t pos0 = b << GRID_SHIFT;
      while (r + 1 < n_refs && ix->refs[r].end_idx <= pos0) r++;
      ix->ref_bin[b] = r;
    }
    auto fill = [&](auto& v) {
      typedef typename std::remove_reference<decltype(v)>::type::value_type R;
      v.resize(n_refs);
      for (uint32_t i = 0; i < n_refs; i++) {
        R x;
        x.start = (decltype(x.start))ix->refs[i].start_idx;
        x.end = (decltype(x.end))ix->refs[i].end_idx;
        x.len = (decltype(x.len))ix->refs[i].len;
        x.name_rank = ix->name_rank[i];
        x.strand = ix->refs[i].strand ? 1u : 0u;
        v[i] = x;
      }
    };
    if (wide)
      fill(ix->ref_recs64);
    else
      fill(ix->ref_recs);
  }
  ix->dev_mu = new std::mutex();
  *out = ix;
  return THM_OK;
}

template <class F>
static int32_t guarded(F&& f) {
  try {
    return f();
  } catch (const std::bad_alloc&) {
    set_global_error("out of memory");
    return THM_ERR_OOM;
  } catch (const std::exception& e) {
    set_global_error(std::string("internal error: ") + e.what());
    return THM_ERR_INTERNAL;
  } catch (...) {
    set_global_error("internal error");
    return THM_ERR_INTERNAL;
  }
}

extern "C" {

int32_t thm_index_create_in_memory(const uint8_t* text, uint64_t n, const thm_ref* refs, uint32_t n_refs,
                                   const thm_tx* txs, uint32_t n_txs, const thm_exon* exons, uint64_t n_exons,
                                   const uint8_t* tx_seq, uint64_t n_tx_seq, const thm_span* genes, uint32_t n_genes,
                                   const uint32_t* name_rank, uint32_t n_names, const uint32_t* sa, thm_index** out) {
  return guarded([&] {
    return index_create_impl(text, n, refs, n_refs, txs, n_txs, exons, n_exons, tx_seq, n_tx_seq, genes, n_genes, name_rank,
                             n_names, sa, 4, 0, out);
  });
}

int32_t thm_index_create_in_memory_ex(const uint8_t* text, uint64_t n, const thm_ref* refs, uint32_t n_refs,
                                      const thm_tx* txs, uint32_t n_txs, const thm_exon* exons, uint64_t n_exons,
                                      const uint8_t* tx_seq, uint64_t n_tx_seq, const thm_span* genes, uint32_t n_genes,
                                      const uint32_t* name_rank, uint32_t n_names, const void* sa, uint32_t sa_elem_bytes,
                                      uint32_t flags, thm_index** out) {
  return guarded([&] {
    return index_create_impl(text, n, refs, n_refs, txs, n_txs, exons, n_exons, tx_seq, n_tx_seq, genes, n_genes, name_rank,
                             n_names, sa, sa_elem_bytes, flags, out);
  });
}

uint32_t thm_index_coord_bytes(const thm_index* ix) { return ix ? (ix->wide ? 8u : 4u) : 0u; }
const uint64_t* thm_index_suffix_array64(const thm_index* ix) { return (ix && ix->wide) ? ix->sa64.data() : nullptr; }

int32_t thm_debug_check_lut(const thm_index* ix) {
  if (!ix) return THM_ERR_INVALID_ARG;
  const bool ok = ix->wide ? check_lut<uint64_t>(ix, ix->lut64, ix->sa64.data()) : check_lut<uint32_t>(ix, ix->lut, ix->sa.data());
  return ok ? THM_OK : THM_ERR_INTERNAL;
}

int32_t thm_debug_host_lut(const thm_index* ix, uint32_t* kt, void* out, uint64_t bytes) {
  if (!ix || !kt) return THM_ERR_INVALID_ARG;
  *kt = ix->kt;
  if (!out) return THM_OK;
  const void* src = ix->wide ? (const void*)ix->lut64.data() : (const void*)ix->lut.data();
  const uint64_t have = ix->wide ? ix->lut64.size() * sizeof(ix->lut64[0]) : ix->lut.size() * sizeof(ix->lut[0]);
  if (bytes != have) return THM_ERR_INVALID_ARG;
  if (bytes) memcpy(out, src, bytes);
  return THM_OK;
}

uint64_t thm_index_text_len(const thm_index* ix) { return ix ? ix->n : 0; }
const uint32_t* thm_index_suffix_array(const thm_index* ix) { return (ix && !ix->wide) ? ix->sa.data() : nullptr; }

int32_t thm_index_idx_to_ref(const thm_index* ix, uint64_t idx, uint64_t* offset) {
  if (!ix || idx >= ix->n) return THM_ERR_INVALID_ARG;
  size_t lo = 0, hi = ix->refs.size();
  while (lo < hi) {
    size_t mid = (lo + hi) / 2;
    if (ix->refs[mid].end_idx <= idx)
      lo = mid + 1;
    else
      hi = mid;
  }
  if (offset) *offset = idx - ix->refs[lo].start_idx;
  return (int32_t)lo;
}

}
```

### thermite_amd/csrc/kernels_seed.hip

```cpp
#include <hip/hip_runtime.h>

#include <algorithm>

#include "launch.h"
#include "lut_direct.h"
#include "swg_device.h"

namespace thm {
namespace dev {

__device__ __forceinline__ int base_code(uint8_t c) {
  return c == 'A' ? 0 : c == 'C' ? 1 : c == 'G' ? 2 : c == 'T' ? 3 : -1;
}
__device__ __forceinline__ uint8_t sanitize_base(uint8_t c) {
  if (c >= 'a' && c <= 'z') c = (uint8_t)(c - 32);
  return (c == 'A' || c == 'C' || c == 'G' || c == 'T' || c == 'N') ? c : (uint8_t)0;
}
__device__ __forceinline__ uint64_t load8_global(const uint8_t* p) {
  uint64_t v;
  __builtin_memcpy(&v, p, 8);
  return v;
}
__device__ __forceinline__ uint64_t load8_lds(const uint8_t* base16, int off) {
  const uint64_t* q = (const uint64_t*)(base16 + (off & ~7));
// ... 702 lines not shown
        int rank = 0;
        for (int u = 0; u < n_sm; u++) {
          const int lu = s_len[u], eu = s_em[u];
          rank += (lu > len || (lu == len && eu > em)) ? 1 : 0;
        }
        if (fits) {
          SmemT<C> sm;
          sm.lo = s_lo[t];
          sm.hi = s_hi[t];
          sm.qpos = s_pos[t];
          sm.len = (uint16_t)len;
          p.smems[base_out + rank] = sm;
        }
        hits += (unsigned long long)(s_hi[t] - s_lo[t]);
      }
    }
    for (int o = 32; o > 0; o >>= 1) hits += __shfl_xor(hits, o);
    if (lane == 0) {
      if (!fits) atomicExch(p.fault, 1);
      p.read_smem_off[idx] = base_out;
      p.read_smem_cnt[idx] = (uint32_t)n_sm;
      p.read_hits[idx] = hits;
    }
    c_smems += (unsigned long long)n_sm;
    c_hits += hits;
    sync();
  }
  if (lane == 0 && (c_smems | c_hits)) {
    atomicAdd(&p.counters[THM_CNT_SMEMS], c_smems);
    atomicAdd(&p.counters[THM_CNT_HITS], c_hits);
  }
}

constexpr int SEL_CAP = 6;

template <class C>
__global__ __launch_bounds__(256) void seed_select_thread_kernel(SeedParamsT<C> p, unsigned long long* over_list,
                                                                 unsigned long long* over_count) {
  extern __shared__ __attribute__((aligned(16))) uint8_t smem[];
  const unsigned T = blockDim.x, tid = threadIdx.x;
  C* l_lo = (C*)smem;
  C* l_hi = l_lo + (size_t)SEL_CAP * T;
  uint32_t* l_pl = (uint32_t*)(l_hi + (size_t)SEL_CAP * T);
  const int lane = lane_id();
  const uint64_t wi = (uint64_t)blockIdx.x * T + tid;
  const bool active = wi < p.work_counts[0];
  const int k = (int)p.min_seed_len;
  int n_sm = 0;
  bool overflow = false;
  uint64_t read = 0;
  if (active) {
    read = p.work_short[wi];
    const uint64_t r0 = p.reads.offsets[read];
    const int L = (int)(p.reads.offsets[read + 1] - r0);
    const int npos = max(L - k + 1, 0);
    const uint64_t item0 = ms_row(r0, read);
    int prev = 0;
    const uint4* row = (const uint4*)(p.ms_end + item0);
    for (int c0 = 0; c0 < npos; c0 += 8) {
      const uint4 v = row[c0 >> 3];
      const uint32_t w[4] = {v.x, v.y, v.z, v.w};
#pragma unroll
      for (int j = 0; j < 8; j++) {
        const int pos = c0 + j;
        const int e = (int)((w[j >> 1] >> (16 * (j & 1))) & 0xffffu);
        if (pos < npos && e > 0 && e > prev) {
          if (n_sm < SEL_CAP) {
            l_lo[(size_t)n_sm * T + tid] = p.ms_lo[item0 + (uint64_t)pos];
            l_hi[(size_t)n_sm * T + tid] = p.ms_hi[item0 + (uint64_t)pos];
            l_pl[(size_t)n_sm * T + tid] = (uint32_t)pos | ((uint32_t)(e - pos) << 8);
          } else {
            overflow = true;
          }
          n_sm++;
        }
        prev = e;
      }
    }
    if (overflow) n_sm = 0;
  }
  block_append(overflow, read, over_list, over_count);

  if (n_sm > 1) {
    int t = 0, em = 0, i0 = 0;
    while (t < n_sm) {
      const int st = (int)(l_pl[(size_t)t * T + tid] & 0xffu);
      if (st > i0) i0 = st;
      int u = t;
      while (u < n_sm && (int)(l_pl[(size_t)u * T + tid] & 0xffu) <= i0) u++;
      for (int v = u - 1; v >= t; v--) l_pl[(size_t)v * T + tid] |= (uint32_t)(em + (u - 1 - v)) << 16;
      em += u - t;
      const uint32_t z = l_pl[(size_t)(u - 1) * T + tid];
      i0 = (int)(z & 0xffu) + (int)((z >> 8) & 0xffu);
      t = u;
    }
  }
  int incl = n_sm;
  for (int o = 1; o < 64; o <<= 1) {
    const int v = __shfl_up(incl, o);
    if (lane >= o) incl += v;
  }
  const int total = __shfl(incl, 63);
  unsigned long long base = 0;
  if (total > 0) {
    if (lane == 0) base = atomicAdd(p.cursor, (unsigned long long)total);
    base = ((unsigned long long)(unsigned)bcast_first((int)(base >> 32)) << 32) | (unsigned)bcast_first((int)(base & 0xffffffffu));
  }
  const bool fits = base + (unsigned long long)total <= p.smem_cap;
  const unsigned long long mine = base + (unsigned long long)(incl - n_sm);
  unsigned long long hits = 0;
  for (int t = 0; t < n_sm; t++) {
    const uint32_t a = l_pl[(size_t)t * T + tid];
    const int len = (int)((a >> 8) & 0xffu), em = (int)(a >> 16);
    int rank = 0;
    for (int u = 0; u < n_sm; u++) {
      const uint32_t b = l_pl[(size_t)u * T + tid];
      const int lu = (int)((b >> 8) & 0xffu), eu = (int)(b >> 16);
      rank += (lu > len || (lu == len && eu > em)) ? 1 : 0;
    }
    const C slo = l_lo[(size_t)t * T + tid], shi = l_hi[(size_t)t * T + tid];
    if (fits) {
      SmemT<C> sm;
      sm.lo = slo;
      sm.hi = shi;
      sm.qpos = (uint16_t)(a & 0xffu);
      sm.len = (uint16_t)len;
      p.smems[mine + rank] = sm;
    }
    hits += (unsigned long long)(shi - slo);
  }
  if (active && !overflow) {
    p.read_smem_off[read] = mine;
    p.read_smem_cnt[read] = (uint32_t)n_sm;
    p.read_hits[read] = hits;
  }
  int fault = (total > 0 && !fits) ? 1 : 0;
  for (int o = 32; o > 0; o >>= 1) {
    hits += __shfl_xor(hits, o);
    fault |= __shfl_xor(fault, o);
  }
  if (lane == 0) {
    if (fault) atomicExch(p.fault, 1);
    if (total > 0) {
      atomicAdd(&p.counters[THM_CNT_SMEMS], (unsigned long long)total);
      atomicAdd(&p.counters[THM_CNT_HITS], hits);
    }
  }
}

template <class C>
__global__ __launch_bounds__(256) void plan_pack_kernel(PlanParams p, PackParamsT<C> q) {
  const uint64_t r = (uint64_t)blockIdx.x * 256 + threadIdx.x;
  const bool active = r < p.n_reads;
  uint64_t b0 = 0, L = 0, hits = 0;
  if (active) {
    b0 = p.offsets[r];
    L = p.offsets[r + 1] - b0;
    hits = p.read_hits[r];
  }
  const bool fast = active && L <= p.fast_max_len;
  const bool slow = active && !fast && L <= p.slow_max_len;
  if (active && !fast && !slow) {
    p.read_status[r] = THM_ERR_UNSUPPORTED;
    p.read_n_alns[r] = 0;
    p.read_op_bytes[r] = 0;
  }
  const uint64_t team_thr = p.tpr_max_hits ? (uint64_t)max(p.tpr_max_hits, TEAM_MIN_HITS)
                                           : min((uint64_t)TEAM_HITS, max((uint64_t)TEAM_MIN_HITS, *p.total_hits / max(p.team_div, 1u)));
  const bool team = fast && p.team_ok && hits >= team_thr && hits <= TEAM_MAX_HITS;
  block_append(fast && !team && hits >= (p.tpr_max_hits ? (uint64_t)p.tpr_max_hits : (uint64_t)HEAVY_HITS), r, p.heavy, &p.counts[2]);
  block_append(slow, r, p.slow, &p.counts[5]);
  block_append(team, r, p.team, &p.counts[7]);
  if (!active) return;
  ReadRecT<C> rec;
  rec.base_off = b0;
  rec.len = L > 0xFFFFFFFEull ? 0xFFFFFFFFu : (uint32_t)L;
  rec.smem_off = q.read_smem_off[r];
  rec.smem_cnt = q.read_smem_cnt[r];
  const uint64_t c0 = q.read_cand_off[r] + q.tile_offs[r / SCAN_TILE];
  q.read_cand_off[r] = c0;
  rec.cand_off = c0;
  rec.n_hits = hits > 0xFFFFFFFFull ? 0xFFFFFFFFu : (uint32_t)hits;
  rec.qpos0 = rec.len0 = 0;
  rec.lo0 = rec.hi0 = rec.sa0 = 0;
  if (rec.smem_cnt > 0 && *q.fault_seed == 0) {
    const SmemT<C> sm = q.smems[rec.smem_off];
    rec.qpos0 = sm.qpos;
    rec.len0 = sm.len;
    rec.lo0 = sm.lo;
    rec.hi0 = sm.hi;
    if (sm.hi > sm.lo) rec.sa0 = q.sa[sm.hi - 1];
  }
  q.recs[r] = rec;
}

template <class C>
__global__ __launch_bounds__(256) void expand_kernel(ExpandParamsT<C> p) {
  const int lane = lane_id();
  const uint64_t r = (uint64_t)blockIdx.x * 4 + (threadIdx.x >> 6);
  if (r >= p.n_reads) return;
  const uint64_t s0 = p.read_smem_off[r];
  const uint32_t ns = p.read_smem_cnt[r];
  uint64_t out = p.read_mem_off[r];
  for (uint32_t s = 0; s < ns; s++) {
    const SmemT<C> sm = p.smems[s0 + s];
    const uint64_t cnt = (uint64_t)(sm.hi - sm.lo);
    for (uint64_t t = lane; t < cnt; t += 64) {
      thm_mem m;
      m.ref_idx = p.ix.sa[sm.hi - 1 - t];
      m.query_idx = sm.qpos;
      m.len = sm.len;
      p.mems[out + t] = m;
    }
    out += cnt;
  }
}

}

static uint32_t sel_lcap(uint32_t max_read_len) { return (max_read_len + 31u) & ~15u; }
size_t seed_select_scratch_bytes(uint32_t max_read_len) { return (size_t)sel_lcap(max_read_len) * (2 * 8 + 8); }
size_t seed_select_lds_bytes(uint32_t max_read_len) { return 4 * seed_select_scratch_bytes(max_read_len); }

hipError_t launch_sanitize(const uint8_t* in, uint8_t* out, uint64_t n, uint64_t n_padded, hipStream_t s) {
  if (n_padded == 0) return hipSuccess;
  hipLaunchKernelGGL(dev::sanitize_kernel, dim3((unsigned)((n_padded / 16 + 255) / 256 + 1)), dim3(256), 0, s, in, out, n, n_padded);
  return hipGetLastError();
}

hipError_t launch_sanitize_reset(const uint8_t* in, uint8_t* out, uint64_t n, uint64_t n_padded, const RunResetParams& rp, hipStream_t s) {
  const uint64_t threads = std::max<uint64_t>(std::max<uint64_t>(n_padded / 16 + 1, rp.status_vec4), std::max<uint64_t>(rp.ctl_vec4, THM_N_COUNTERS));
  hipLaunchKernelGGL(dev::sanitize_reset_kernel, dim3((unsigned)((threads + 255) / 256)), dim3(256), 0, s, in, out, n, n_padded, rp);
  return hipGetLastError();
}

template <class C>
static hipError_t launch_seed_t(const SeedParamsT<C>& p, int n_blocks, hipStream_t s) {
  const uint64_t n = p.reads.n_reads;
  if (n == 0) return hipSuccess;
  const uint32_t k = p.min_seed_len;
  auto blocks = [](uint64_t threads) { return dim3((unsigned)((threads + 255) / 256)); };
  auto cells_of = [&](uint32_t max_len) -> uint64_t {
    const uint32_t P = (max_len >= k) ? max_len - k + 1 : 1;
    return (P + dev::PROBE_STRIDE - 1) / dev::PROBE_STRIDE;
  };
  hipError_t e;
  hipLaunchKernelGGL(dev::seed_first_kernel<C>, blocks(n), dim3(256), 0, s, p);
  if ((e = hipGetLastError()) != hipSuccess) return e;
  const uint64_t n_short = n - p.n_long;
  struct Cls {
    uint64_t n;
    uint32_t max_len;
    const unsigned long long* list;
    const unsigned long long* count;
    bool fused;
  } cls[2] = {{n_short, p.max_len_short, p.work_short, p.work_counts + 0, true},
              {p.n_long, p.max_len_long, p.work_long, p.work_counts + 4, false}};
  uint64_t fill_cells = 0;
  for (const Cls& c : cls) {
    if (c.n == 0 || c.max_len < k + 1) continue;
    const uint64_t NC = cells_of(c.max_len), G = NC + 1;
    if (c.fused && G <= 256) {
      const uint64_t per = 256 / G;
      hipLaunchKernelGGL(dev::seed_grid_cells_kernel<C>, dim3((unsigned)((c.n + per - 1) / per)), dim3(256), 0, s, p, c.list, c.count,
                         (uint32_t)G);
      if ((e = hipGetLastError()) != hipSuccess) return e;
    } else {
      hipLaunchKernelGGL(dev::seed_grid_kernel<C>, blocks(c.n * G), dim3(256), 0, s, p, c.list, c.count, (uint32_t)G);
      if ((e = hipGetLastError()) != hipSuccess) return e;
      hipLaunchKernelGGL(dev::seed_cells_kernel<C>, blocks(c.n * NC), dim3(256), 0, s, p, c.list, c.count, (uint32_t)NC);
      if ((e = hipGetLastError()) != hipSuccess) return e;
    }
    fill_cells += c.n * NC;
  }
  if (fill_cells) {
    const dim3 worst = blocks(fill_cells * dev::PROBE_STRIDE);
    const dim3 fixed(std::min<unsigned>(worst.x, 256u * 8u * 4u));
    if (p.fill_mode == 2 && fill_cells * dev::PROBE_STRIDE < (1ull << 32)) {
      hipLaunchKernelGGL(dev::seed_fill_keys_kernel<C>, fixed, dim3(256), 0, s, p);
      hipLaunchKernelGGL(dev::seed_fill_scan_kernel, dim3(1), dim3(1024), 0, s, p.fill_hist);
      hipLaunchKernelGGL(dev::seed_fill_scatter_kernel<C>, fixed, dim3(256), 0, s, p);
      hipLaunchKernelGGL(dev::seed_fill_bucketed_kernel<C>, fixed, dim3(256), 0, s, p);
    } else {
      hipLaunchKernelGGL(dev::seed_fill_kernel<C>, p.fill_mode == 1 ? fixed : worst, dim3(256), 0, s, p);
    }
    if ((e = hipGetLastError()) != hipSuccess) return e;
  }
  auto select_waves = [&](const unsigned long long* list, const unsigned long long* count, unsigned int* queue, uint32_t max_len,
                          int nb) -> hipError_t {
    const uint32_t lcap = sel_lcap(max_len);
    const size_t lds = 4 * (size_t)lcap * (2 * sizeof(C) + 8);
    if (lds <= SEED_SELECT_LDS_LIMIT) {
      hipLaunchKernelGGL((dev::seed_select_kernel<C, false>), dim3(nb), dim3(256), lds, s, p, list, count, queue, lcap);
    } else {
      hipLaunchKernelGGL((dev::seed_select_kernel<C, true>), dim3(nb), dim3(256), 0, s, p, list, count, queue, lcap);
    }
    return hipGetLastError();
  };
  if (n_short) {
    unsigned long long* over_list = p.work_cells;
    unsigned long long* over_count = p.work_counts + 3;
    hipLaunchKernelGGL(dev::seed_select_thread_kernel<C>, dim3((unsigned)((n_short + 255) / 256)), dim3(256),
                       (size_t)256 * (2 * sizeof(C) + 4) * dev::SEL_CAP, s, p, over_list, over_count);
    if ((e = hipGetLastError()) != hipSuccess) return e;
    if ((e = select_waves(over_list, over_count, p.queue, p.max_len_short, std::min(n_blocks, 256))) != hipSuccess) return e;
  }
// ... 30 lines not shown
```

### thermite_amd/csrc/launch.h

```cpp
#ifndef THERMITE_LAUNCH_H
#define THERMITE_LAUNCH_H

#include <hip/hip_runtime.h>

#include "thermite_internal.h"

namespace thm {

struct SwgBatchParams {
  const uint8_t* xb;
  const uint64_t* xo;
  const uint8_t* yb;
  const uint64_t* yo;
  const uint32_t* bw;
  const int32_t* xd;
  const uint64_t* ops_off;
  uint8_t* ops;
  thm_swg_aln* out;
  unsigned long long* counters;
  unsigned int* queue;
  int* fault;
  uint64_t n;
  uint32_t x_cap, y_cap;
  uint8_t* scratch;
  uint64_t scratch_per_wave;
  uint32_t max_bw;
};
size_t swg_batch_lds_bytes(const SwgBatchParams& p, int cpl);
size_t swg_batch_scratch_bytes(const SwgBatchParams& p);
hipError_t launch_swg_batch(const SwgBatchParams& p, int cpl, int n_blocks, hipStream_t s);
hipError_t launch_wave_prims(const int* in, int* out, hipStream_t s);

struct ElrBatchParams {
  const uint8_t* xb;
  const uint64_t* xo;
  const uint8_t* yb;
  const uint64_t* yo;
  const thm_mem* hits;
  const uint32_t* bw;
  const int32_t* xd;
  const uint64_t* ops_off;
  uint8_t* ops;
  thm_lr_aln* out;
  unsigned long long* counters;
  unsigned int* queue;
  int* fault;
  uint64_t n;
  uint32_t x_cap, y_cap;
  uint8_t* scratch;
  uint64_t scratch_per_wave;
  uint32_t max_bw;
};
size_t elr_batch_lds_bytes(const ElrBatchParams& p, int cpl);
size_t elr_batch_scratch_bytes(const ElrBatchParams& p);
hipError_t launch_elr_batch(const ElrBatchParams& p, int cpl, int n_blocks, hipStream_t s);

struct ReadBatch {
  const uint8_t* bases;
  const uint64_t* offsets;
  uint64_t n_reads;
};

constexpr uint32_t MAX_READ_LEN = 65535;
constexpr uint32_t SHORT_READ_MAX = 255;

__host__ __device__ inline uint64_t ms_row(uint64_t base_off, uint64_t r) { return (base_off + 8 * r) & ~7ull; }

template <class C>
struct SeedParamsT {
  DeviceIndexT<C> ix;
  ReadBatch reads;
  uint32_t min_seed_len;
  uint32_t max_len_short;
  uint32_t max_len_long;
  uint64_t n_long;
  uint16_t* ms_end;
  C* ms_lo;
  C* ms_hi;
  unsigned long long* work_short;
  unsigned long long* work_long;
  unsigned long long* work_cells;
  unsigned long long* work_counts;
  uint32_t flags;
  SmemT<C>* smems;
  uint64_t smem_cap;
  unsigned long long* cursor;
  uint64_t* read_smem_off;
  uint32_t* read_smem_cnt;
  uint64_t* read_hits;
  int32_t* read_status;
  unsigned long long* counters;
  unsigned int* queue;
  int* fault;
  uint8_t* sel_scratch;
  uint64_t sel_scratch_per_wave;
  uint32_t fill_mode;
  uint16_t* fill_keys;
  uint32_t* fill_perm;
  unsigned int* fill_hist;
};
constexpr uint32_t SEED_INFER = 1u, SEED_STATS = 2u, SEED_NODIRECT = 4u;
constexpr int FILL_KEY_BASES = 7;
constexpr unsigned FILL_BUCKETS = 1u << (2 * FILL_KEY_BASES);
size_t seed_select_lds_bytes(uint32_t max_read_len);
size_t seed_select_scratch_bytes(uint32_t max_read_len);
constexpr size_t SEED_SELECT_LDS_LIMIT = 64 * 1024;
hipError_t launch_seed(const SeedParamsT<uint32_t>& p, int n_blocks, hipStream_t s);
hipError_t launch_seed(const SeedParamsT<uint64_t>& p, int n_blocks, hipStream_t s);
hipError_t launch_sanitize(const uint8_t* in, uint8_t* out, uint64_t n, uint64_t n_padded, hipStream_t s);
hipError_t launch_lut_tag(LutEntryT<uint32_t>* lut, const uint32_t* sa, uint64_t n_entries, uint64_t n, unsigned long long* count, hipStream_t s);
hipError_t launch_lut_tag(LutEntryT<uint64_t>* lut, const uint64_t* sa, uint64_t n_entries, uint64_t n, unsigned long long* count, hipStream_t s);

struct RunResetParams {
  uint4* ctl;
  uint32_t ctl_vec4;
  uint4* status;
  uint64_t status_vec4;
  uint4* san_head;
  unsigned long long* counters;
};
hipError_t launch_sanitize_reset(const uint8_t* in, uint8_t* out, uint64_t n, uint64_t n_padded, const RunResetParams& rp, hipStream_t s);

struct PlanParams {
  const uint64_t* offsets;
  const uint64_t* read_hits;
  uint64_t n_reads;
  uint32_t fast_max_len;
  uint32_t slow_max_len;
  unsigned long long* heavy;
  unsigned long long* slow;
  unsigned long long* team;
  uint32_t team_ok;
  const uint64_t* total_hits;
  uint32_t team_div;
  uint32_t tpr_max_hits;
  unsigned long long* counts;
  int32_t* read_status;
  uint32_t* read_n_alns;
  uint64_t* read_op_bytes;
};

template <class C>
struct ReadRecT {
  uint64_t base_off;
  uint64_t smem_off;
  uint64_t cand_off;
  uint32_t len;
  uint32_t smem_cnt;
  uint32_t n_hits;
  uint16_t qpos0, len0;
  C lo0, hi0;
  C sa0;
};
static_assert(sizeof(ReadRecT<uint32_t>) == 56 && sizeof(ReadRecT<uint64_t>) == 64, "ReadRec layout");
template <class C>
struct PackParamsT {
  const C* sa;
  const uint64_t* offsets;
  uint64_t n_reads;
  const SmemT<C>* smems;
  const uint64_t* read_smem_off;
  const uint32_t* read_smem_cnt;
  uint64_t* read_cand_off;
  const uint64_t* tile_offs;
  const int* fault_seed;
  ReadRecT<C>* recs;
};
hipError_t launch_plan_pack(const PlanParams& pl, const PackParamsT<uint32_t>& pk, hipStream_t s);
hipError_t launch_plan_pack(const PlanParams& pl, const PackParamsT<uint64_t>& pk, hipStream_t s);

template <class C>
struct ExpandParamsT {
  DeviceIndexT<C> ix;
  uint64_t n_reads;
  const SmemT<C>* smems;
  const uint64_t* read_smem_off;
  const uint32_t* read_smem_cnt;
  const uint64_t* read_mem_off;
  thm_mem* mems;
};
hipError_t launch_expand(const ExpandParamsT<uint32_t>& p, hipStream_t s);
hipError_t launch_expand(const ExpandParamsT<uint64_t>& p, hipStream_t s);

hipError_t launch_exclusive_scan_u64(const uint64_t* in, uint64_t* out, uint64_t n, uint64_t* block_tmp,
                                     hipStream_t s);
size_t scan_tmp_entries(uint64_t n);
constexpr unsigned SCAN_TILE = 2048;
hipError_t launch_scan_tiles_sums_u64(const uint64_t* in, uint64_t* out, uint64_t n, uint64_t* block_tmp, hipStream_t s);
hipError_t launch_exclusive_scan2(const uint32_t* in_a, const uint64_t* in_b, uint64_t* out_a, uint64_t* out_b, uint64_t n,
                                  uint64_t* block_tmp, hipStream_t s);

struct Cand {
  uint64_t ystart, yend, ylen;
  uint64_t tx_ystart, tx_yend, tx_ylen;
  uint64_t ops_off;
  uint64_t tx_ops_off;
  int32_t score;
  uint32_t ref_id;
  uint32_t xstart, xend;
  uint32_t ops_len, tx_ops_len;
  uint32_t tx_or_gene_idx;
  int32_t tx_score;
  uint32_t tx_xstart, tx_xend;
  uint32_t name_rank;
  uint8_t strand, aln_type, primary, pad_;
};

constexpr unsigned EXT_NQ = 8, EXT_QSTRIDE = 64;
constexpr size_t QUEUE_BYTES = (EXT_NQ + 3) * EXT_QSTRIDE * 4;
constexpr unsigned HEAVY_HITS = 8;
constexpr unsigned TEAM_HITS = 256;
constexpr unsigned TEAM_MIN_HITS = 32;
constexpr unsigned TEAM_DIV_PER_CU = 22;
constexpr int TEAM_WAVES = 16;
constexpr unsigned TEAM_MAX_HITS = 60000;
constexpr int FAST_MAX_YCLIPS = 64;

template <class C>
struct ExtendParamsT {
  DeviceIndexT<C> ix;
  ReadBatch reads;
  thm_align_opts opts;
  const SmemT<C>* smems;
  const ReadRecT<C>* read_recs;
  const unsigned long long* heavy;
  const unsigned long long* heavy_count;
  const unsigned long long* team;
  const unsigned long long* team_count;
  uint32_t team_limit;
  Cand* cands;
  uint64_t cand_cap;
  uint32_t* order;
  uint8_t* cand_ops;
  uint64_t cand_ops_cap;
  unsigned long long* ops_cursor;
  uint32_t* read_n_alns;
  uint64_t* read_op_bytes;
  int32_t* read_status;
  unsigned long long* retry;
  unsigned long long* retry_count;
  unsigned long long* n_contract;
  unsigned long long* counters;
  unsigned long long* wave_counters;
  unsigned int* queue;
  int* fault;
  const int* fault_seed;
  uint32_t max_read_len;
  uint32_t max_bw;
  uint32_t mk_cap;
  uint32_t list_only;
  uint32_t skip_scan;
  unsigned long long* trace_scratch;
  uint8_t* slow_scratch;
  uint64_t slow_scratch_per_wave;
  unsigned long long* prof;
};
size_t extend_lds_bytes(uint32_t max_read_len, uint32_t max_bw, int cpl);
int extend_waves_per_simd(int cpl, bool wide);
int compact_k();
int hit_gl();
size_t extend_trace_scratch_bytes(uint32_t max_read_len, uint32_t max_bw, int cpl);
size_t extend_slow_scratch_bytes(uint32_t max_read_len, uint32_t max_bw, uint32_t mk_cap);
constexpr size_t EXTEND_LDS_LIMIT = 160 * 1024;
constexpr size_t TEAM_STATIC_LDS = 16384 + TEAM_WAVES * 32 + 64;
inline bool team_fits_lds(size_t lds4) { return lds4 / 4 * TEAM_WAVES + TEAM_STATIC_LDS + 256 <= EXTEND_LDS_LIMIT; }
hipError_t launch_extend(const ExtendParamsT<uint32_t>& p, int cpl, int n_blocks, hipStream_t s, bool team = false);
hipError_t launch_extend(const ExtendParamsT<uint64_t>& p, int cpl, int n_blocks, hipStream_t s, bool team = false);
enum : uint16_t {
  SK_EMPTY = 0,
  SK_SINGLE = 1,
  SK_SHORTCUT = 2,
  SK_UNK_DEL = 3,
  SK_UNK = 4,
  SK_UNK_EQ = 5
};
struct HitSide {
  uint16_t kind;
  uint16_t eq;
  uint32_t A;
};
struct HitTgt {
  uint32_t tx, ent;
  int32_t tr;
  uint16_t t_q, t_len;
  HitSide r, l;
  uint32_t pos;
};
constexpr int HIT_MAX_OPEN = 3;
constexpr int HIT_MAX_VAR = 4;
enum : uint8_t { HF_COMPLEX = 1, HF_KNOWN = 2 };
struct HitSum {
  uint64_t hr;
  uint32_t ref_id;
  uint16_t q, len;
  HitSide gr, gl;
  uint32_t win_fixed;
  uint8_t win_nl, win_nr, win_nvl, win_nvr;
  uint16_t win_var[HIT_MAX_VAR];
  uint8_t n_tgt;
  uint8_t n_open;
  uint8_t flags;
  uint8_t why;
  HitTgt known;
  HitTgt open[HIT_MAX_OPEN];
  uint32_t pad_;
};
static_assert(sizeof(HitSide) == 8 && sizeof(HitTgt) == 36 && sizeof(HitSum) == 200, "hit summary layout");
struct HitHdr {
  uint64_t hr;
  uint32_t read;
  uint16_t q, len;
};
template <class C>
struct HitParamsT {
  DeviceIndexT<C> ix;
  ReadBatch reads;
  thm_align_opts opts;
  const SmemT<C>* smems;
  const ReadRecT<C>* read_recs;
  uint32_t max_read_len, max_hits;
  HitHdr* hdr;
  HitSum* sums;
  const uint64_t* total_hits;
  uint64_t slot_cap;
  const int* fault_seed;
};
hipError_t launch_hit_expand(const HitParamsT<uint32_t>& p, hipStream_t s);
hipError_t launch_hit_expand(const HitParamsT<uint64_t>& p, hipStream_t s);
hipError_t launch_hit_summaries(const HitParamsT<uint32_t>& p, int n_blocks, hipStream_t s);
hipError_t launch_hit_summaries(const HitParamsT<uint64_t>& p, int n_blocks, hipStream_t s);

constexpr int DP_MAX_EDITS = 8;
struct DpRec {
  const uint8_t* x0;
  const uint8_t* y0;
  uint64_t pad0_;
  uint16_t xlen, ylen, bw, xd;
  int8_t dir;
  uint8_t cls;
  uint16_t n_edits;
  uint32_t read;
  int32_t score;
  uint16_t xend, yend, nops;
  uint16_t done;
  uint32_t cells, cols;
  uint32_t pad2_;
};
static_assert(sizeof(DpRec) == 64, "DpRec layout");
constexpr int DPT_SLOTS = 16;
constexpr int DP_NQ = 5;
constexpr int TPR_MAX_ROUNDS = 8;
constexpr unsigned TPR_MAX_HITS = 32;
struct ReadMemo {
  uint32_t base[TPR_MAX_ROUNDS];
  uint16_t cnt[TPR_MAX_ROUNDS];
  uint16_t first_hit[TPR_MAX_ROUNDS];
  uint8_t n_rounds;
  uint8_t pad_[7];
};
static_assert(sizeof(ReadMemo) == 72, "ReadMemo layout");
template <class C>
struct TprParamsT {
  ReadRecT<C>* recs_rw;
  ReadMemo* memos;
  DpRec* recs;
  uint64_t rec_cap;
  unsigned long long* rec_cursor;
  uint32_t* q_list;
  uint64_t q_stride;
  unsigned long long* q_cur;
  const uint32_t* act_in;
  const unsigned long long* n_act_in;
  uint32_t* act_out;
  unsigned long long* n_act_out;
  unsigned long long* bail;
  unsigned long long* bail_count;
  unsigned long long* team;
  unsigned long long* team_count;
  uint32_t max_hits;
  uint32_t dpt_cols;
  const HitSum* sums;
  uint32_t round;
  uint32_t last_round;
  unsigned long long* stats;
};
struct DpParams {
  DpRec* recs;
  const uint32_t* q_list;
  uint64_t q_stride;
  const unsigned long long* q_cur;
  const unsigned long long* q_done;
  unsigned int* work;
  int* fault;
  uint32_t x_cap, y_cap;
  unsigned long long* trace_scratch;
  uint64_t trace_per_wave;
  uint32_t tcols;
};
size_t extend_dpt_lds_bytes(uint32_t tcols);
hipError_t launch_extend_dpt(const DpParams& p, int n_blocks, hipStream_t s);
size_t extend_dp_lds_bytes(uint32_t x_cap, uint32_t y_cap);
size_t extend_dp_trace_bytes(uint32_t y_cap, int cpl_max);
hipError_t launch_extend_ctl(const ExtendParamsT<uint32_t>& p, const TprParamsT<uint32_t>& tp, int n_blocks, hipStream_t s);
hipError_t launch_extend_ctl(const ExtendParamsT<uint64_t>& p, const TprParamsT<uint64_t>& tp, int n_blocks, hipStream_t s);
hipError_t launch_extend_dp(const DpParams& p, int cpl_max, int n_blocks, hipStream_t s);
hipError_t launch_tpr_order(const ReadRecT<uint32_t>* recs, uint64_t n, uint32_t max_len, uint32_t max_hits, unsigned long long* bins, uint32_t* out,
                            unsigned long long* n_out, const int* fault_seed, hipStream_t s);
hipError_t launch_tpr_order(const ReadRecT<uint64_t>* recs, uint64_t n, uint32_t max_len, uint32_t max_hits, unsigned long long* bins, uint32_t* out,
                            unsigned long long* n_out, const int* fault_seed, hipStream_t s);
constexpr int TPR_CTL_BLOCKS_PER_CU = 4, TPR_DP_BLOCKS_PER_CU = 8;
enum { TPRC_REC_CUR = 0, TPRC_Q_CUR = 2 , TPRC_Q_DONE = 7 , TPRC_N_ACT = 12 , TPRC_STATS = 24 , TPRC_BAIL_CNT = 23,
       TPRC_BINS = 40 ,
       TPRC_WORK_BYTES = 2048  };
constexpr size_t TPRC_BYTES = TPRC_WORK_BYTES + (size_t)(TPR_MAX_ROUNDS + 1) * 4 * 64;

struct CompactParams {
  uint64_t n_reads;
  const uint64_t* read_cand_off;
  const Cand* cands;
  const uint32_t* order;
// ... 139 lines not shown
```

### thermite_amd/csrc/pipeline.hip

```cpp
#include <hip/hip_runtime.h>

#include <algorithm>
#include <cstring>

#include "aligner_internal.h"

using namespace thm;

uint32_t seed_fill_mode() {
  static const uint32_t v = [] {
    const char* e = getenv("THM_SEED_FILL");
    const int v = e ? atoi(e) : 0;
    return (uint32_t)(v >= 0 && v <= 2 ? v : 0);
  }();
  return v;
}
unsigned team_div_per_cu() {
  static const unsigned v = [] {
    const char* e = getenv("THM_TEAM_DIV_PER_CU");
    const int v = e ? atoi(e) : 0;
    return v > 0 ? (unsigned)v : TEAM_DIV_PER_CU;
  }();
  return v;
}

namespace {

int band_for_len(const thm_align_opts& o, uint32_t L) {
  volatile float prod = o.min_aln_score_percent * (float)L;
  float pv = prod;
  int pct = (pv != pv) ? 0 : (pv >= 2147483648.0f ? 2147483647 : (pv <= -2147483648.0f ? (-2147483647 - 1) : (int)pv));
  int ms = std::max(pct, o.min_aln_score);
  if (ms < 0) return 0;
  return std::max((int)L - ms, 0);
}

int blocks_for(const thm_aligner* a, uint64_t n, size_t lds_per_block) {
  int per_cu = 8;
  if (lds_per_block > 0) per_cu = (int)std::min<size_t>(8, (160 * 1024) / lds_per_block);
  if (per_cu < 1) per_cu = 1;
  return grid_blocks(a, n, 4, per_cu);
}

constexpr uint64_t SLOW_SCRATCH_BUDGET = 24ull << 30;

template <class C>
const DeviceIndexT<C>& dev_view(const thm_aligner* a);
template <>
const DeviceIndexT<uint32_t>& dev_view<uint32_t>(const thm_aligner* a) {
  return a->dix->view;
}
template <>
const DeviceIndexT<uint64_t>& dev_view<uint64_t>(const thm_aligner* a) {
  return a->dix->view64;
}

template <class C>
int enqueue_seed_t(thm_aligner* a, uint32_t min_seed_len, bool finish_scan) {
  const uint64_t n = a->n_reads;
  hipStream_t s = a->stream;
  HIPCHK(a, a->s_off.ensure((n + 1) * 8));
  HIPCHK(a, a->s_cnt.ensure((n + 1) * 4));
  HIPCHK(a, a->s_hits.ensure((n + 1) * 8));
  HIPCHK(a, a->s_cand_off.ensure((n + 2) * 8));
  HIPCHK(a, a->scan_tmp.ensure(2 * scan_tmp_entries(n + 1) * 8 + 64));
  HIPCHK(a, a->r_status.ensure((n + 1) * 4 + 16));
  const uint64_t smem_min = a->dbg_smem_cap ? a->dbg_smem_cap : n * 4 + (4u << 20);
  if (a->smem_cap < smem_min) a->smem_cap = smem_min;
  HIPCHK(a, a->s_smems.ensure(a->smem_cap * sizeof(SmemT<C>)));
  if (!a->dbg_smem_cap) a->smem_cap = std::max<uint64_t>(a->smem_cap, a->s_smems.cap / sizeof(SmemT<C>));
  HIPCHK(a, a->r_san.ensure(a->n_bases + 256 + 16));
  {
    RunResetParams rp;
    rp.ctl = a->d_ctl.as<uint4>();
    rp.ctl_vec4 = (uint32_t)(thm_aligner::CTL_BYTES / 16);
    rp.status = a->r_status.as<uint4>();
    rp.status_vec4 = ((n + 1) * 4 + 15) / 16;
    rp.san_head = a->r_san.as<uint4>();
    rp.counters = a->d_counters.as<unsigned long long>();
    HIPCHK(a, launch_sanitize_reset(a->r_bases.as<uint8_t>(), a->r_san.as<uint8_t>() + 16, a->n_bases, a->n_bases + 128, rp, s));
  }
  uint64_t n_long = 0;
  uint32_t max_short = 0, max_long = 0;
  for (const auto& lc : a->len_hist) {
    if (lc.first <= SHORT_READ_MAX) {
      max_short = std::max(max_short, lc.first);
    } else {
      max_long = std::max(max_long, lc.first);
      n_long += lc.second;
    }
  }
  const uint64_t n_short = n - n_long;
  const uint64_t items = ms_row(a->n_bases, n) + 64;
  HIPCHK(a, a->s_ms_end.ensure(items * 2 + 64));
  HIPCHK(a, a->s_ms_lo.ensure(items * sizeof(C) + 64));
  HIPCHK(a, a->s_ms_hi.ensure(items * sizeof(C) + 64));
  auto cells_of = [&](uint32_t max_len) -> uint64_t {
    const uint32_t P = (max_len >= min_seed_len) ? max_len - min_seed_len + 1 : 1;
    return (P + 7) / 8;
  };
  const uint64_t cells = n_short * cells_of(max_short) + n_long * cells_of(max_long);
  HIPCHK(a, a->s_work_reads.ensure((n + 1) * 8));
  HIPCHK(a, a->s_work_long.ensure((n_long + 1) * 8));
  HIPCHK(a, a->s_work_cells.ensure((std::max(cells, n) + 1) * 8));
  const int n_blocks = blocks_for(a, n, std::min(seed_select_lds_bytes(std::max(max_short, 1u)), SEED_SELECT_LDS_LIMIT));
  SeedParamsT<C> sp;
  sp.ix = dev_view<C>(a);
  sp.reads.bases = a->r_san.as<uint8_t>() + 16;
  sp.reads.offsets = a->r_offsets.as<uint64_t>();
  sp.reads.n_reads = n;
  sp.min_seed_len = min_seed_len;
  sp.max_len_short = max_short;
  sp.max_len_long = max_long;
  sp.n_long = n_long;
  sp.ms_end = a->s_ms_end.as<uint16_t>();
  sp.ms_lo = a->s_ms_lo.as<C>();
  sp.ms_hi = a->s_ms_hi.as<C>();
  sp.work_short = a->s_work_reads.as<unsigned long long>();
  sp.work_long = a->s_work_long.as<unsigned long long>();
  sp.work_cells = a->s_work_cells.as<unsigned long long>();
  sp.work_counts = a->s_work_counts.as<unsigned long long>();
  sp.flags = (a->dbg_seed_noinfer ? 0u : SEED_INFER) | (a->dbg_seed_stats ? SEED_STATS : 0u) | (a->dbg_seed_nodirect ? SEED_NODIRECT : 0u);
  sp.smems = a->s_smems.as<SmemT<C>>();
  sp.smem_cap = a->smem_cap;
  sp.cursor = a->d_cursors.as<unsigned long long>();
  sp.read_smem_off = a->s_off.as<uint64_t>();
  sp.read_smem_cnt = a->s_cnt.as<uint32_t>();
  sp.read_hits = a->s_hits.as<uint64_t>();
  sp.read_status = a->r_status.as<int32_t>();
  sp.counters = a->d_counters.as<unsigned long long>();
  sp.queue = a->d_queue.as<unsigned int>();
  sp.fault = a->d_fault.as<int>();
  sp.sel_scratch = nullptr;
  sp.sel_scratch_per_wave = 0;
  const uint32_t fill_mode = seed_fill_mode();
  sp.fill_mode = fill_mode;
  sp.fill_keys = nullptr;
  sp.fill_perm = nullptr;
  sp.fill_hist = nullptr;
  if (fill_mode == 2) {
    const uint64_t slots = (std::max(cells, n) + 1) * 8;
    HIPCHK(a, a->s_fill_keys.ensure(slots * 2));
    HIPCHK(a, a->s_fill_perm.ensure(slots * 4));
    HIPCHK(a, a->s_fill_hist.ensure((2 * (FILL_BUCKETS + 1) + 1) * 4));
    HIPCHK(a, hipMemsetAsync(a->s_fill_hist.p, 0, (2 * (FILL_BUCKETS + 1) + 1) * 4, s));
    sp.fill_keys = a->s_fill_keys.as<uint16_t>();
    sp.fill_perm = a->s_fill_perm.as<uint32_t>();
    sp.fill_hist = a->s_fill_hist.as<unsigned int>();
  }
  if (n_long && seed_select_lds_bytes(max_long) > SEED_SELECT_LDS_LIMIT) {
    const int nb = (int)std::max<uint64_t>(1, std::min<uint64_t>((uint64_t)n_blocks, (n_long + 3) / 4));
    sp.sel_scratch_per_wave = (seed_select_scratch_bytes(max_long) + 255) & ~255ull;
    HIPCHK(a, a->s_sel_scratch.ensure((size_t)nb * 4 * sp.sel_scratch_per_wave + 256));
    sp.sel_scratch = a->s_sel_scratch.as<uint8_t>();
  }
  HIPCHK(a, launch_seed(sp, n_blocks, s));
  if (finish_scan)
    HIPCHK(a, launch_exclusive_scan_u64(a->s_hits.as<uint64_t>(), a->s_cand_off.as<uint64_t>(), n, a->scan_tmp.as<uint64_t>(), s));
  else
    HIPCHK(a, launch_scan_tiles_sums_u64(a->s_hits.as<uint64_t>(), a->s_cand_off.as<uint64_t>(), n, a->scan_tmp.as<uint64_t>(), s));
  return THM_OK;
}

int enqueue_seed(thm_aligner* a, uint32_t min_seed_len, bool finish_scan) {
  return a->dix->wide ? enqueue_seed_t<uint64_t>(a, min_seed_len, finish_scan) : enqueue_seed_t<uint32_t>(a, min_seed_len, finish_scan);
}

template <class C>
int enqueue_plan_pack_t(thm_aligner* a, const PlanParams& pp) {
  HIPCHK(a, a->e_recs.ensure((a->n_reads + 1) * sizeof(ReadRecT<C>)));
  PackParamsT<C> pk;
  pk.sa = dev_view<C>(a).sa;
  pk.offsets = a->r_offsets.as<uint64_t>();
  pk.n_reads = a->n_reads;
  pk.smems = a->s_smems.as<SmemT<C>>();
  pk.read_smem_off = a->s_off.as<uint64_t>();
  pk.read_smem_cnt = a->s_cnt.as<uint32_t>();
  pk.read_cand_off = a->s_cand_off.as<uint64_t>();
  pk.tile_offs = a->scan_tmp.as<uint64_t>();
  pk.fault_seed = a->d_fault.as<int>();
  pk.recs = a->e_recs.as<ReadRecT<C>>();
  HIPCHK(a, launch_plan_pack(pp, pk, a->stream));
  return THM_OK;
}

struct ExtClasses {
  uint32_t fast_max = 0, fast_len = 0, fast_bw = 0;
  uint32_t slow_max = 0, slow_len = 0, slow_bw = 0;
  uint64_t n_slow = 0;
};
ExtClasses classify(const thm_aligner* a, uint32_t mk_cap_slow) {
  ExtClasses c;
  bool fast_open = true;
  for (const auto& lc : a->len_hist) {
    const uint32_t L = lc.first;
    const uint32_t bw = (uint32_t)band_for_len(a->opts, L);
    const int cpl = (int)((2 * bw + 1 + 63) / 64);
    if (fast_open && cpl <= 4 && extend_lds_bytes(L, bw, cpl) <= EXTEND_LDS_LIMIT) {
      c.fast_len = L;
      c.fast_bw = bw;
      continue;
    }
    fast_open = false;
    if (extend_slow_scratch_bytes(L, bw, mk_cap_slow) > SLOW_SCRATCH_BUDGET) break;
    c.slow_len = L;
    c.slow_bw = bw;
    c.n_slow += lc.second;
  }
  c.fast_max = c.fast_len;
  c.slow_max = std::max(c.slow_len, c.fast_len);
  return c;
}

template <class C>
int enqueue_extend_t(thm_aligner* a, const ExtClasses& cls, uint32_t mk_cap_slow, bool retry_possible) {
  const uint64_t n = a->n_reads;
  hipStream_t s = a->stream;
  ExtendParamsT<C> ep;
  ep.ix = dev_view<C>(a);
  ep.reads.bases = a->r_san.as<uint8_t>() + 16;
  ep.reads.offsets = a->r_offsets.as<uint64_t>();
  ep.reads.n_reads = n;
  ep.opts = a->opts;
  ep.smems = a->s_smems.as<SmemT<C>>();
  ep.read_recs = a->e_recs.as<ReadRecT<C>>();
  ep.heavy = a->s_heavy.as<unsigned long long>();
  ep.heavy_count = a->s_work_counts.as<unsigned long long>() + 2;
  ep.team = a->s_team.as<unsigned long long>();
  ep.team_count = a->s_work_counts.as<unsigned long long>() + 7;
  ep.team_limit = 2u * (uint32_t)a->n_cu;
  ep.cands = a->e_cands.as<Cand>();
  ep.cand_cap = a->cand_cap;
  ep.order = a->e_order.as<uint32_t>();
  ep.cand_ops = a->e_ops.as<uint8_t>();
  ep.cand_ops_cap = a->cand_ops_cap;
  ep.ops_cursor = a->d_cursors.as<unsigned long long>() + 1;
  ep.read_n_alns = a->e_nalns.as<uint32_t>();
  ep.read_op_bytes = a->e_opbytes.as<uint64_t>();
  ep.read_status = a->r_status.as<int32_t>();
  ep.retry = a->s_slow.as<unsigned long long>();
  ep.retry_count = a->s_work_counts.as<unsigned long long>() + 5;
  ep.n_contract = a->s_work_counts.as<unsigned long long>() + 6;
  ep.counters = a->d_counters.as<unsigned long long>();
  ep.queue = a->d_queue_ext.as<unsigned int>();
  ep.fault = a->d_fault.as<int>() + 1;
  ep.fault_seed = a->d_fault.as<int>();
  ep.prof = a->d_counters.as<unsigned long long>() + 2 * THM_N_COUNTERS;
  ep.slow_scratch = nullptr;
  ep.slow_scratch_per_wave = 0;
  ep.trace_scratch = nullptr;
  ep.max_read_len = cls.fast_len;
  ep.max_bw = cls.fast_bw;
  if (a->dbg_band_clip) ep.max_bw = std::min<uint32_t>(ep.max_bw, a->dbg_band_clip - 1);
  ep.mk_cap = FAST_MAX_YCLIPS;
  ep.list_only = 0;
  const int cpl = std::max(1, (int)((2 * cls.fast_bw + 1 + 63) / 64));
  const size_t lds = extend_lds_bytes(cls.fast_len, cls.fast_bw, cpl);
  const int ext_blocks = std::min(blocks_for(a, n, lds), a->n_cu * extend_waves_per_simd(cpl, sizeof(C) == 8));
  const bool team_ok = cpl <= 2 && team_fits_lds(lds);
  const size_t trace_per_wave = extend_trace_scratch_bytes(cls.fast_len, cls.fast_bw, cpl);
  const size_t main_trace_waves = (size_t)ext_blocks * 4, team_trace_waves = team_ok ? (size_t)a->n_cu * TEAM_WAVES : 0;
  HIPCHK(a, a->e_trace.ensure((main_trace_waves + team_trace_waves) * trace_per_wave + 64));
  ep.trace_scratch = a->e_trace.as<unsigned long long>();
  uint64_t slow_waves = 0, slow_per_wave = 0;
  if (cls.n_slow || retry_possible) {
    const uint32_t sl_len = std::max(cls.slow_len, cls.fast_len), sl_bw = std::max(cls.slow_bw, cls.fast_bw);
    slow_per_wave = (extend_slow_scratch_bytes(sl_len, sl_bw, mk_cap_slow) + 255) & ~255ull;
    slow_waves = std::max<uint64_t>(1, std::min<uint64_t>(SLOW_SCRATCH_BUDGET / std::max<uint64_t>(slow_per_wave, 1), (uint64_t)a->n_cu * 8));
    if (!retry_possible) slow_waves = std::min(slow_waves, std::max<uint64_t>(cls.n_slow, 1));
    slow_waves = (slow_waves + 3) / 4 * 4;
  }
  const uint64_t main_rows = (uint64_t)ext_blocks * 4, team_rows = team_ok ? (uint64_t)a->n_cu * TEAM_WAVES : 0;
  const bool tpr = a->use_tpr && n > 0 && cpl <= 4;
  const int ctl_blocks = tpr ? (int)std::min<uint64_t>((n + 255) / 256, (uint64_t)a->n_cu * TPR_CTL_BLOCKS_PER_CU) : 0;
  const uint32_t dp_x_cap = (cls.fast_len + 64u + 15u) & ~15u, dp_y_cap = (cls.fast_len + cls.fast_bw + 2u + 64u + 15u) & ~15u;
  const int dp_per_cu = (int)std::max<size_t>(1, std::min<size_t>(TPR_DP_BLOCKS_PER_CU, EXTEND_LDS_LIMIT / std::max<size_t>(1, extend_dp_lds_bytes(dp_x_cap, dp_y_cap))));
  const int dp_blocks = tpr ? a->n_cu * dp_per_cu : 0;
  const uint32_t dpt_tcols = std::min<uint32_t>(std::min<uint32_t>(dp_y_cap, 128u), std::max<uint32_t>(cls.fast_len + DPT_SLOTS / 2 + 2, DPT_SLOTS + cls.fast_bw + 2));
  const int dpt_per_cu = (int)std::max<size_t>(1, std::min<size_t>(8, EXTEND_LDS_LIMIT / std::max<size_t>(1, extend_dpt_lds_bytes(dpt_tcols))));
  const int dpt_blocks = tpr ? a->n_cu * dpt_per_cu : 0;
  const int bail_blocks = tpr ? std::min(ext_blocks, a->n_cu) : 0;
  const uint64_t tpr_rows = (uint64_t)ctl_blocks + (uint64_t)bail_blocks * 4;
  const uint64_t n_rows = main_rows + team_rows + slow_waves + tpr_rows;
  HIPCHK(a, a->e_wcnt.ensure(n_rows * THM_N_COUNTERS * 8 + 64));
  if (a->wcnt_clean_cap != a->e_wcnt.cap) HIPCHK(a, hipMemsetAsync(a->e_wcnt.p, 0, a->e_wcnt.cap, s));
  a->wcnt_clean_cap = 0;
  ep.wave_counters = a->e_wcnt.as<unsigned long long>();
  ep.skip_scan = 0;
  if (tpr) {
    const uint64_t rec_cap = std::min<uint64_t>(4 * n + 65536, 64ull << 20);
    HIPCHK(a, a->t_memos.ensure(n * sizeof(ReadMemo) + 64));
    HIPCHK(a, a->t_recs.ensure(rec_cap * sizeof(DpRec) + 64));
    HIPCHK(a, a->t_qlist.ensure((size_t)DP_NQ * rec_cap * 4 + 64));
    HIPCHK(a, a->t_act[0].ensure(n * 4 + 64));
    HIPCHK(a, a->t_act[1].ensure(n * 4 + 64));
    HIPCHK(a, a->t_bail.ensure((n + 1) * 8));
    HIPCHK(a, a->t_queue2.ensure(thm::QUEUE_BYTES));
    HIPCHK(a, hipMemsetAsync(a->t_queue2.p, 0, thm::QUEUE_BYTES, s));
    HIPCHK(a, a->t_ctl.ensure(TPRC_BYTES));
    HIPCHK(a, hipMemsetAsync(a->t_ctl.p, 0, TPRC_BYTES, s));
    unsigned long long* ctl = a->t_ctl.as<unsigned long long>();
    TprParamsT<C> tq;
    tq.recs_rw = a->e_recs.as<ReadRecT<C>>();
    tq.memos = a->t_memos.as<ReadMemo>();
    tq.recs = a->t_recs.as<DpRec>();
    tq.rec_cap = rec_cap;
    tq.rec_cursor = ctl + TPRC_REC_CUR;
    tq.q_list = a->t_qlist.as<uint32_t>();
    tq.q_stride = rec_cap;
    tq.q_cur = ctl + TPRC_Q_CUR;
    tq.bail = a->t_bail.as<unsigned long long>();
    tq.bail_count = ctl + TPRC_BAIL_CNT;
    tq.team = nullptr;
    tq.team_count = nullptr;
    tq.max_hits = TPR_MAX_HITS;
    tq.dpt_cols = dpt_tcols;
    tq.stats = ctl + TPRC_STATS;
    ExtendParamsT<C> zp = ep;
    zp.wave_counters = ep.wave_counters + (main_rows + team_rows + slow_waves) * THM_N_COUNTERS;
    DpParams dq;
    dq.recs = tq.recs;
    dq.q_list = tq.q_list;
    dq.q_stride = tq.q_stride;
    dq.q_cur = ctl + TPRC_Q_CUR;
    dq.q_done = ctl + TPRC_Q_DONE;
    dq.fault = ep.fault;
    dq.x_cap = dp_x_cap;
    dq.y_cap = dp_y_cap;
    {
      const size_t tb = extend_dp_trace_bytes(dp_y_cap, cpl);
      HIPCHK(a, a->t_trace.ensure((size_t)dp_blocks * 4 * tb + 64));
      dq.trace_scratch = a->t_trace.as<unsigned long long>();
      dq.trace_per_wave = tb / 8;
      dq.tcols = dpt_tcols;
    }
    {
      const uint64_t slot_cap = a->cand_cap;
      HIPCHK(a, a->t_hdr.ensure(slot_cap * sizeof(HitHdr) + 64));
      HIPCHK(a, a->t_sums.ensure(slot_cap * sizeof(HitSum) + 64));
      HIPCHK(a, hipMemsetAsync(a->t_hdr.p, 0xFF, slot_cap * sizeof(HitHdr), s));
      HitParamsT<C> hq;
      hq.ix = ep.ix;
      hq.reads = ep.reads;
      hq.opts = ep.opts;
      hq.smems = ep.smems;
      hq.read_recs = ep.read_recs;
      hq.max_read_len = cls.fast_len;
      hq.max_hits = TPR_MAX_HITS;
      hq.hdr = a->t_hdr.as<HitHdr>();
      hq.sums = a->t_sums.as<HitSum>();
      hq.total_hits = a->s_cand_off.as<uint64_t>() + n;
      hq.slot_cap = slot_cap;
      hq.fault_seed = a->d_fault.as<int>();
      HIPCHK(a, launch_hit_expand(hq, s));
      HIPCHK(a, launch_hit_summaries(hq, a->n_cu * 12, s));
      tq.sums = a->t_sums.as<HitSum>();
    }
    {
      ExtendParamsT<C> hp = ep;
      hp.skip_scan = 1;
      hp.team_limit = 16u * (uint32_t)a->n_cu;
      HIPCHK(a, hipEventRecord(a->ev_fork, s));
      HIPCHK(a, hipStreamWaitEvent(a->stream2, a->ev_fork, 0));
      HIPCHK(a, hipStreamWaitEvent(a->stream3, a->ev_fork, 0));
      if (team_ok) {
        ExtendParamsT<C> tp = hp;
        tp.list_only = 1;
        tp.wave_counters = ep.wave_counters + main_rows * THM_N_COUNTERS;
        tp.trace_scratch = ep.trace_scratch + main_trace_waves * trace_per_wave / 8;
        HIPCHK(a, launch_extend(tp, cpl, a->n_cu, a->stream2, true));
      }
      HIPCHK(a, launch_extend(hp, cpl, std::min(ext_blocks, a->n_cu), a->stream3));
      HIPCHK(a, hipEventRecord(a->ev_join, a->stream2));
      HIPCHK(a, hipEventRecord(a->ev_join3, a->stream3));
    }
    HIPCHK(a, launch_tpr_order(a->e_recs.as<ReadRecT<C>>(), n, cls.fast_len, TPR_MAX_HITS, ctl + TPRC_BINS, a->t_act[0].as<uint32_t>(), ctl + TPRC_N_ACT,
                               a->d_fault.as<int>(), s));
    const int n_rounds = a->tpr_rounds;
    for (int r = 0; r <= n_rounds; r++) {
      tq.round = (uint32_t)r;
      tq.act_in = a->t_act[r & 1].as<uint32_t>();
      tq.n_act_in = ctl + TPRC_N_ACT + r;
      tq.act_out = a->t_act[(r + 1) & 1].as<uint32_t>();
      tq.n_act_out = ctl + TPRC_N_ACT + r + 1;
      tq.last_round = r == n_rounds ? 1u : 0u;
      HIPCHK(a, launch_extend_ctl(zp, tq, ctl_blocks, s));
      if (r == n_rounds) break;
      dq.work = (unsigned int*)((uint8_t*)a->t_ctl.p + TPRC_WORK_BYTES + (size_t)r * 4 * 64);
      HIPCHK(a, hipEventRecord(a->ev_dpt_fork, s));
      HIPCHK(a, hipStreamWaitEvent(a->stream4, a->ev_dpt_fork, 0));
      HIPCHK(a, launch_extend_dpt(dq, dpt_blocks, a->stream4));
      HIPCHK(a, hipEventRecord(a->ev_dpt_join, a->stream4));
      HIPCHK(a, launch_extend_dp(dq, cpl, dp_blocks, s));
      HIPCHK(a, hipStreamWaitEvent(s, a->ev_dpt_join, 0));
      HIPCHK(a, hipMemcpyAsync(ctl + TPRC_Q_DONE, ctl + TPRC_Q_CUR, DP_NQ * 8, hipMemcpyDeviceToDevice, s));
    }
    HIPCHK(a, hipStreamWaitEvent(s, a->ev_join, 0));
    HIPCHK(a, hipStreamWaitEvent(s, a->ev_join3, 0));
    {
      ExtendParamsT<C> bp = ep;
      bp.skip_scan = 1;
      bp.heavy = a->t_bail.as<unsigned long long>();
      bp.heavy_count = ctl + TPRC_BAIL_CNT;
      bp.team = nullptr;
      bp.team_count = nullptr;
      bp.queue = a->t_queue2.as<unsigned int>();
      bp.wave_counters = zp.wave_counters + (uint64_t)ctl_blocks * THM_N_COUNTERS;
      HIPCHK(a, launch_extend(bp, cpl, bail_blocks, s));
    }
  } else if (team_ok) {
    ExtendParamsT<C> tp = ep;
    tp.list_only = 1;
    tp.wave_counters = ep.wave_counters + main_rows * THM_N_COUNTERS;
    tp.trace_scratch = ep.trace_scratch + main_trace_waves * trace_per_wave / 8;
    HIPCHK(a, hipEventRecord(a->ev_fork, s));
    HIPCHK(a, launch_extend(tp, cpl, a->n_cu, s, true));
    HIPCHK(a, hipStreamWaitEvent(a->stream2, a->ev_fork, 0));
    HIPCHK(a, launch_extend(ep, cpl, ext_blocks, a->stream2));
    HIPCHK(a, hipEventRecord(a->ev_join, a->stream2));
    HIPCHK(a, hipStreamWaitEvent(s, a->ev_join, 0));
  } else {
    HIPCHK(a, launch_extend(ep, cpl, ext_blocks, s));
  }
  if (cls.n_slow || retry_possible) {
    const uint32_t sl_len = std::max(cls.slow_len, cls.fast_len), sl_bw = std::max(cls.slow_bw, cls.fast_bw);
    const uint64_t per_wave = slow_per_wave;
    const int blocks = (int)(slow_waves / 4);
    ep.wave_counters = a->e_wcnt.as<unsigned long long>() + (main_rows + team_rows) * THM_N_COUNTERS;
    HIPCHK(a, a->e_slow.ensure((size_t)blocks * 4 * per_wave + 256));
    ep.max_read_len = sl_len;
    ep.max_bw = sl_bw;
    ep.mk_cap = mk_cap_slow;
    ep.list_only = 1;
    ep.heavy = a->s_slow.as<unsigned long long>();
    ep.heavy_count = a->s_work_counts.as<unsigned long long>() + 5;
    ep.team = nullptr;
    ep.team_count = nullptr;
    ep.slow_scratch = a->e_slow.as<uint8_t>();
    ep.slow_scratch_per_wave = per_wave;
    HIPCHK(a, launch_extend(ep, 0, blocks, s));
  }
  HIPCHK(a, launch_counters_reduce(a->e_wcnt.as<unsigned long long>(), (uint32_t)n_rows, a->d_counters.as<unsigned long long>(), s));
  a->wcnt_clean_cap = a->e_wcnt.cap;
  return THM_OK;
}

int enqueue_run(thm_aligner* a) {
  const uint64_t n = a->n_reads;
  hipStream_t s = a->stream;
  HIPCHK(a, hipEventRecord(a->ev[0], s));
  int rc = enqueue_seed(a, (uint32_t)a->opts.min_seed_len, false);
  if (rc != THM_OK) return rc;
  HIPCHK(a, hipEventRecord(a->ev[1], s));

  const uint64_t cand_min = a->dbg_cand_cap ? a->dbg_cand_cap : n * 3 + 1024;
  const uint64_t ops_min = a->dbg_ops_cap ? a->dbg_ops_cap : std::max<uint64_t>(n * 384, a->n_bases * 3) + 65536;
  if (a->cand_cap < cand_min) a->cand_cap = cand_min;
  if (a->cand_ops_cap < ops_min) a->cand_ops_cap = ops_min;
  HIPCHK(a, a->e_cands.ensure(a->cand_cap * sizeof(Cand)));
  HIPCHK(a, a->e_order.ensure(a->cand_cap * 2 * 4));
  HIPCHK(a, a->e_heavy.ensure((a->cand_cap / 2 + 16) * 2 * 8));
  HIPCHK(a, a->e_rel.ensure(a->cand_cap * 4));
  HIPCHK(a, a->e_ops.ensure(a->cand_ops_cap + 64));
  HIPCHK(a, a->e_nalns.ensure((n + 1) * 4));
  HIPCHK(a, a->e_opbytes.ensure((n + 1) * 8));
  HIPCHK(a, a->e_aln_off.ensure((n + 2) * 8));
  HIPCHK(a, a->e_ops_off.ensure((n + 2) * 8));
  HIPCHK(a, a->o_alns.ensure(a->cand_cap * sizeof(thm_aln)));
  HIPCHK(a, a->o_ops.ensure(a->cand_ops_cap + 64));
  HIPCHK(a, a->s_heavy.ensure((n + 1) * 8));
  HIPCHK(a, a->s_slow.ensure((n + 1) * 8));
  HIPCHK(a, a->s_team.ensure((n + 1) * 8));

  const uint32_t mk_cap_slow = std::max<uint32_t>(a->ix->max_tx_exons, 1);
  const bool retry_possible = a->ix->max_tx_exons > (uint32_t)FAST_MAX_YCLIPS + 1;
  const ExtClasses cls = classify(a, mk_cap_slow);
  a->n_slow_host = cls.n_slow;
  a->fast_max_len = cls.fast_max;
  a->slow_max_len = cls.slow_max;
  PlanParams pp;
  pp.offsets = a->r_offsets.as<uint64_t>();
  pp.read_hits = a->s_hits.as<uint64_t>();
  pp.n_reads = n;
  pp.fast_max_len = cls.fast_max;
  pp.slow_max_len = cls.slow_max;
  pp.heavy = a->s_heavy.as<unsigned long long>();
  pp.slow = a->s_slow.as<unsigned long long>();
  pp.team = a->s_team.as<unsigned long long>();
  {
    const int cpl_f = std::max(1, (int)((2 * cls.fast_bw + 1 + 63) / 64));
    pp.team_ok = (cpl_f <= 2 && team_fits_lds(extend_lds_bytes(cls.fast_len, cls.fast_bw, cpl_f))) ? 1u : 0u;
  }
  pp.total_hits = a->s_cand_off.as<uint64_t>() + n;
  pp.team_div = team_div_per_cu() * (uint32_t)std::max(a->n_cu, 1);
  pp.tpr_max_hits = (a->use_tpr && std::max(1, (int)((2 * cls.fast_bw + 1 + 63) / 64)) <= 4) ? TPR_MAX_HITS : 0u;
  pp.counts = a->s_work_counts.as<unsigned long long>();
  pp.read_status = a->r_status.as<int32_t>();
  pp.read_n_alns = a->e_nalns.as<uint32_t>();
  pp.read_op_bytes = a->e_opbytes.as<uint64_t>();
  rc = a->dix->wide ? enqueue_plan_pack_t<uint64_t>(a, pp) : enqueue_plan_pack_t<uint32_t>(a, pp);
  if (rc != THM_OK) return rc;
  HIPCHK(a, hipEventRecord(a->ev[2], s));

  rc = a->dix->wide ? enqueue_extend_t<uint64_t>(a, cls, mk_cap_slow, retry_possible)
                    : enqueue_extend_t<uint32_t>(a, cls, mk_cap_slow, retry_possible);
  if (rc != THM_OK) return rc;
  HIPCHK(a, hipEventRecord(a->ev[3], s));

  HIPCHK(a, launch_exclusive_scan2(a->e_nalns.as<uint32_t>(), a->e_opbytes.as<uint64_t>(), a->e_aln_off.as<uint64_t>(),
                                   a->e_ops_off.as<uint64_t>(), n, a->scan_tmp.as<uint64_t>(), s));
  CompactParams cp;
  cp.n_reads = n;
  cp.read_cand_off = a->s_cand_off.as<uint64_t>();
  cp.cands = a->e_cands.as<Cand>();
  cp.order = a->e_order.as<uint32_t>();
  cp.cand_ops = a->e_ops.as<uint8_t>();
  cp.read_n_alns = a->e_nalns.as<uint32_t>();
  cp.read_aln_off = a->e_aln_off.as<uint64_t>();
  cp.read_ops_off = a->e_ops_off.as<uint64_t>();
  cp.read_offsets = a->r_offsets.as<uint64_t>();
  cp.alns = a->o_alns.as<thm_aln>();
  cp.ops = a->o_ops.as<uint8_t>();
  cp.fault = a->d_fault.as<int>();
  cp.alns_cap = a->cand_cap;
  cp.ops_cap = a->cand_ops_cap;
  cp.heavy_cap = a->cand_cap / 2 + 16;
  cp.heavy_cnt = a->d_cursors.as<unsigned long long>() + 2;
  cp.heavy_list = a->e_heavy.as<uint64_t>();
  cp.heavy_desc = a->e_heavy.as<uint64_t>() + cp.heavy_cap;
  cp.rel = a->e_rel.as<uint32_t>();
  HIPCHK(a, launch_compact(cp, s));
  HIPCHK(a, hipEventRecord(a->ev[4], s));
  return THM_OK;
}

struct RunStatus {
  int fault_seed = 0, fault_ext = 0;
  unsigned long long smem_used = 0, ops_used = 0, total_hits = 0;
};
int read_status(thm_aligner* a, RunStatus* st) {
  hipStream_t s = a->stream;
  int f[2] = {0, 0};
  unsigned long long cur[2] = {0, 0};
  HIPCHK(a, hipMemcpyAsync(f, a->d_fault.p, 8, hipMemcpyDeviceToHost, s));
  HIPCHK(a, hipMemcpyAsync(cur, a->d_cursors.p, 16, hipMemcpyDeviceToHost, s));
  HIPCHK(a, hipMemcpyAsync(&st->total_hits, a->s_cand_off.as<uint64_t>() + a->n_reads, 8, hipMemcpyDeviceToHost, s));
  HIPCHK(a, hipStreamSynchronize(s));
  st->fault_seed = f[0];
  st->fault_ext = f[1];
  st->smem_used = cur[0];
  st->ops_used = cur[1];
  return THM_OK;
}

template <class C>
int expand_mems_t(thm_aligner* a, uint64_t n) {
  ExpandParamsT<C> xp;
  xp.ix = dev_view<C>(a);
  xp.n_reads = n;
  xp.smems = a->s_smems.as<SmemT<C>>();
  xp.read_smem_off = a->s_off.as<uint64_t>();
  xp.read_smem_cnt = a->s_cnt.as<uint32_t>();
  xp.read_mem_off = a->s_cand_off.as<uint64_t>();
  xp.mems = a->o_mems.as<thm_mem>();
  HIPCHK(a, launch_expand(xp, a->stream));
  return THM_OK;
}

}

int batch_length_classes(thm_aligner* a, const uint64_t* offsets, uint64_t n_reads) {
  if (n_reads >= 0xFFFFFFF0ull) return fail(a, THM_ERR_UNSUPPORTED, "more than 2^32-16 reads in one batch");
  if (offsets[0] != 0) return fail(a, THM_ERR_INVALID_ARG, "offsets[0] must be 0");
  uint32_t lmax = 0;
  uint64_t n_over = 0;
  a->len_hist.clear();
  {
    std::vector<uint64_t> cnt(1024, 0);
    std::vector<std::pair<uint32_t, uint64_t>> big;
    for (uint64_t i = 0; i < n_reads; i++) {
      if (offsets[i + 1] < offsets[i]) return fail(a, THM_ERR_INVALID_ARG, "read offsets are not monotone");
      const uint64_t L = offsets[i + 1] - offsets[i];
      if (L > MAX_READ_LEN) {
        n_over++;
        continue;
      }
      if (L < cnt.size())
        cnt[L]++;
      else
        big.emplace_back((uint32_t)L, 1);
      lmax = std::max<uint32_t>(lmax, (uint32_t)L);
    }
    for (uint32_t L = 0; L < cnt.size(); L++)
      if (cnt[L]) a->len_hist.emplace_back(L, cnt[L]);
    std::sort(big.begin(), big.end());
    for (const auto& b : big) {
      if (!a->len_hist.empty() && a->len_hist.back().first == b.first)
        a->len_hist.back().second++;
      else
        a->len_hist.push_back(b);
    }
  }
  a->n_over = n_over;
  a->n_reads = n_reads;
  a->n_bases = offsets[n_reads];
  a->max_read_len = lmax;
  return THM_OK;
}

extern "C" {

int32_t thm_batch_upload(thm_aligner* a, const uint8_t* bases, const uint64_t* offsets, uint64_t n_reads) {
  if (!a || !offsets || (!bases && n_reads && offsets[n_reads] > 0)) return THM_ERR_INVALID_ARG;
  HIPCHK(a, hipSetDevice(a->device));
  a->uploaded = a->ran = a->synced = false;
  a->reads_named = false;
  const int rc = batch_length_classes(a, offsets, n_reads);
  if (rc != THM_OK) return rc;
  HIPCHK(a, a->r_bases.ensure(a->n_bases + 64));
  HIPCHK(a, a->r_offsets.ensure((n_reads + 1) * 8));
  if (a->n_bases) HIPCHK(a, hipMemcpyAsync(a->r_bases.p, bases, a->n_bases, hipMemcpyHostToDevice, a->stream));
  HIPCHK(a, hipMemcpyAsync(a->r_offsets.p, offsets, (n_reads + 1) * 8, hipMemcpyHostToDevice, a->stream));
  HIPCHK(a, hipStreamSynchronize(a->stream));
  a->uploaded = true;
  return THM_OK;
}

int32_t thm_batch_run(thm_aligner* a) {
  if (!a) return THM_ERR_INVALID_ARG;
  if (!a->uploaded) return fail(a, THM_ERR_INVALID_ARG, "thm_batch_run before thm_batch_upload");
  HIPCHK(a, hipSetDevice(a->device));
  a->ran = false;
  a->synced = false;
  int rc = enqueue_run(a);
  if (rc == THM_OK) a->ran = true;
  return rc;
}

int32_t thm_batch_sync(thm_aligner* a) {
  if (!a) return THM_ERR_INVALID_ARG;
  if (!a->ran) return fail(a, THM_ERR_INVALID_ARG, "thm_batch_sync before thm_batch_run");
  if (a->synced) return THM_OK;
  HIPCHK(a, hipSetDevice(a->device));
  for (int attempt = 0; attempt < 6; attempt++) {
    RunStatus st;
    int rc = read_status(a, &st);
    if (rc != THM_OK) return rc;
    if (!st.fault_seed && (st.fault_ext & 2)) return fail(a, THM_ERR_INTERNAL, "extend kernel reported an internal inconsistency (fault word 0x%x)", st.fault_ext);
    const bool grow = st.fault_seed || (st.fault_ext & 1);
    if (!grow) {
      float ms = 0;
      for (int k = 0; k < 4; k++) {
        if (hipEventElapsedTime(&ms, a->ev[k], a->ev[k + 1]) == hipSuccess) a->timings[k] = ms;
      }
      if (hipEventElapsedTime(&ms, a->ev[0], a->ev[4]) == hipSuccess) a->timings[THM_T_TOTAL] = ms;
      a->synced = true;
      return THM_OK;
    }
    if (st.fault_seed) a->smem_cap = std::max<uint64_t>(a->smem_cap * 2, st.smem_used + 1024);
    if (st.total_hits > a->cand_cap) a->cand_cap = st.total_hits + st.total_hits / 8 + 1024;
    if (st.ops_used > a->cand_ops_cap) a->cand_ops_cap = st.ops_used + st.ops_used / 2 + 65536;
    if (a->cand_cap * sizeof(Cand) > (160ull << 30))
      return fail(a, THM_ERR_OOM, "batch has %llu seed hits: candidate pool would exceed 160 GiB", st.total_hits);
    HIPCHK(a, hipMemcpyAsync(a->d_counters.p, a->d_counters.as<uint8_t>() + THM_N_COUNTERS * 8, THM_N_COUNTERS * 8,
                             hipMemcpyDeviceToDevice, a->stream));
    a->n_replays++;
    rc = enqueue_run(a);
    if (rc != THM_OK) return rc;
  }
  return fail(a, THM_ERR_INTERNAL, "pools kept overflowing after 6 attempts");
}

int32_t thm_batch_fetch(thm_aligner* a, thm_batch_view* out) {
  if (!a || !out) return THM_ERR_INVALID_ARG;
  memset(out, 0, sizeof(*out));
  int rc = thm_batch_sync(a);
  if (rc != THM_OK) return rc;
  const uint64_t n = a->n_reads;
// ... 97 lines not shown
```

Baseline: 90.17 million.

## Add seed-stage fast finish for exact and single-substitution unique reads

Adds a finish kernel that runs after seeding. It fully resolves reads whose seeds show an exact unique full-length match, or a single substitution between two unique adjacent SMEMs, and emits their candidate directly. Those reads are marked so the extend stage and SWG skip them. Their ops point into a precomputed match/substitution run buffer through ops_off offsets instead of being written per read. The cost is an extra kernel launch, extra host-side tables and branching, and a correctness risk in matching extend semantics for exon and gene classification.

```diff
diff --git a/thermite_amd/capi.py b/thermite_amd/capi.py
--- a/thermite_amd/capi.py
+++ b/thermite_amd/capi.py
@@ -318,6 +318,12 @@
     if hasattr(L, "thm_debug_set_pool_caps"):
         L.thm_debug_set_pool_caps.restype = i32
         L.thm_debug_set_pool_caps.argtypes = [vp, u64, u64, u64, vp]
+    if hasattr(L, "thm_debug_host_table"):
+        L.thm_debug_host_table.restype = i32
+        L.thm_debug_host_table.argtypes = [vp, i32, vp, u64, vp]
+    if hasattr(L, "thm_debug_smem_finish_stats"):
+        L.thm_debug_smem_finish_stats.restype = i32
+        L.thm_debug_smem_finish_stats.argtypes = [vp, vp]
     if hasattr(L, "thm_debug_set_flags"):
         L.thm_debug_set_flags.restype = i32
         L.thm_debug_set_flags.argtypes = [vp, C.c_uint32]
@@ -520,6 +526,18 @@
             raise ThermiteError(ERR_INTERNAL, "thm_debug_host_lut")
         return out
 
+    HOST_TABLES = ("ref_bin", "ref_recs", "exon_grid_off", "exon_grid", "gene_grid_off", "gene_grid")
+
+    def debug_host_table(self, name):
+        which = self.HOST_TABLES.index(name)
+        n = C.c_uint64()
+        if lib().thm_debug_host_table(self.h, which, None, 0, C.byref(n)) != 0:
+            raise ThermiteError(ERR_INTERNAL, "thm_debug_host_table")
+        out = np.zeros(n.value, np.uint8)
+        if lib().thm_debug_host_table(self.h, which, _ptr(out), out.nbytes, C.byref(n)) != 0:
+            raise ThermiteError(ERR_INTERNAL, "thm_debug_host_table")
+        return out
+
     def idx_to_ref(self, idx):
         off = C.c_uint64()
         r = lib().thm_index_idx_to_ref(self.h, idx, C.byref(off))
@@ -806,17 +824,25 @@
         self._chk(lib().thm_debug_set_pool_caps(self.h, smem_cap, cand_cap, ops_cap, C.byref(n)))
         return n.value
 
-    def debug_set_flags(self, tpr=None, rounds=0, seed_infer=None, seed_stats=None, seed_direct=None):
+    def debug_set_flags(self, tpr=None, rounds=0, seed_infer=None, seed_stats=None, seed_direct=None, finish_exact=None,
+                        finish_subst=None):
         word = (0 if tpr is None else (2 if tpr else 1)) | (int(rounds) << 8)
         word |= 0 if seed_infer is None else (16 if seed_infer else 4)
         word |= 0 if seed_stats is None else (8 if seed_stats else 32)
         word |= 0 if seed_direct is None else (128 if seed_direct else 64)
+        word |= 0 if finish_exact is None else (0x2000 if finish_exact else 0x1000)
+        word |= 0 if finish_subst is None else (0x8000 if finish_subst else 0x4000)
         self._chk(lib().thm_debug_set_flags(self.h, word))
 
     def debug_seed_stats(self):
         out = np.zeros(2, "<u8")
         self._chk(lib().thm_debug_seed_stats(self.h, _ptr(out)))
         return int(out[0]), int(out[1])
+
+    def debug_smem_finish_stats(self):
+        out = np.zeros(4, "<u8")
+        self._chk(lib().thm_debug_smem_finish_stats(self.h, _ptr(out)))
+        return tuple(int(x) for x in out)
 
     def debug_seed_direct_stats(self):
         out = np.zeros(4, "<u8")
diff --git a/thermite_amd/csrc/aligner.hip b/thermite_amd/csrc/aligner.hip
--- a/thermite_amd/csrc/aligner.hip
+++ b/thermite_amd/csrc/aligner.hip
@@ -241,7 +241,7 @@
   if (a->stream3) (void)hipStreamSynchronize(a->stream3);
   if (a->stream4) (void)hipStreamSynchronize(a->stream4);
   DBuf* all[] = {&a->d_counters, &a->d_ctl, &a->b0, &a->b1, &a->b2, &a->b3, &a->b4,
-                 &a->b5, &a->b6, &a->b7, &a->b8, &a->r_bases, &a->r_offsets, &a->r_san, &a->s_ms_end, &a->s_ms_lo, &a->s_ms_hi, &a->s_work_reads, &a->s_work_long, &a->s_work_cells, &a->s_fill_keys, &a->s_fill_perm, &a->s_fill_hist, &a->s_sel_scratch, &a->s_heavy, &a->s_slow, &a->s_team, &a->r_status, &a->e_slow, &a->e_recs, &a->e_wcnt, &a->t_memos, &a->t_recs, &a->t_dpops, &a->t_qlist, &a->t_act[0], &a->t_act[1], &a->t_ctl, &a->t_bail, &a->t_queue2, &a->t_trace, &a->t_ttrace, &a->t_hdr, &a->t_sums, &a->s_smems, &a->s_off, &a->s_cnt,
+                 &a->b5, &a->b6, &a->b7, &a->b8, &a->r_bases, &a->r_offsets, &a->r_san, &a->s_ms_end, &a->s_ms_lo, &a->s_ms_hi, &a->s_work_reads, &a->s_work_long, &a->s_work_cells, &a->s_fill_keys, &a->s_fill_perm, &a->s_fill_hist, &a->s_sel_scratch, &a->s_heavy, &a->s_slow, &a->s_team, &a->r_status, &a->e_slow, &a->e_recs, &a->e_wcnt, &a->e_finstats, &a->t_memos, &a->t_recs, &a->t_dpops, &a->t_qlist, &a->t_act[0], &a->t_act[1], &a->t_ctl, &a->t_bail, &a->t_queue2, &a->t_trace, &a->t_ttrace, &a->t_hdr, &a->t_sums, &a->s_smems, &a->s_off, &a->s_cnt,
                  &a->s_hits, &a->s_cand_off, &a->scan_tmp, &a->e_cands, &a->e_heavy, &a->e_rel, &a->e_order, &a->e_ops, &a->e_nalns,
                  &a->e_opbytes, &a->e_aln_off, &a->e_ops_off, &a->e_trace, &a->o_alns, &a->o_ops, &a->o_mems,
                  &a->sh_bases, &a->sh_san, &a->sh_off, &a->sh_hits, &a->sh_read, &a->sh_bw, &a->sh_xd, &a->sh_list, &a->sh_out,
@@ -584,6 +584,22 @@
   if (flags & 32u) a->dbg_seed_stats = false;
   if (flags & 64u) a->dbg_seed_nodirect = true;
   if (flags & 128u) a->dbg_seed_nodirect = false;
+  if (flags & 0x1000u) a->fin_classes &= ~1u;
+  if (flags & 0x2000u) a->fin_classes |= 1u;
+  if (flags & 0x4000u) a->fin_classes &= ~2u;
+  if (flags & 0x8000u) a->fin_classes |= 2u;
+  return THM_OK;
+}
+int32_t thm_debug_smem_finish_stats(thm_aligner* a, uint64_t stats[4]) {
+  if (!a || !stats) return THM_ERR_INVALID_ARG;
+  stats[0] = stats[1] = stats[2] = stats[3] = 0;
+  if (!a->fin_blocks || !a->e_finstats.p) return THM_OK;
+  HIPCHK(a, hipSetDevice(a->device));
+  HIPCHK(a, hipStreamSynchronize(a->stream));
+  std::vector<unsigned long long> rows((size_t)a->fin_blocks * 4);
+  HIPCHK(a, hipMemcpy(rows.data(), a->e_finstats.p, rows.size() * 8, hipMemcpyDeviceToHost));
+  for (size_t b = 0; b < a->fin_blocks; b++)
+    for (int k = 0; k < 4; k++) stats[k] += rows[b * 4 + k];
   return THM_OK;
 }
 int32_t thm_debug_seed_stats(thm_aligner* a, uint64_t stats[2]) {
diff --git a/thermite_amd/csrc/aligner_internal.h b/thermite_amd/csrc/aligner_internal.h
--- a/thermite_amd/csrc/aligner_internal.h
+++ b/thermite_amd/csrc/aligner_internal.h
@@ -141,6 +141,12 @@
   uint32_t dbg_band_clip = 0;
   bool dbg_seed_noinfer = false, dbg_seed_stats = false;
   bool dbg_seed_nodirect = false;
+  uint32_t fin_classes = 3;
+  const void* ops_run_ptr = nullptr;
+  size_t ops_run_cap = 0;
+  uint32_t ops_run_half = 0;
+  uint32_t fin_run_classes = 0, fin_blocks = 0;
+  DBuf e_finstats;
   uint32_t n_replays = 0;
   bool ran = false, synced = false;
   hipEvent_t ev[6] = {nullptr, nullptr, nullptr, nullptr, nullptr, nullptr};
diff --git a/thermite_amd/csrc/index.cpp b/thermite_amd/csrc/index.cpp
--- a/thermite_amd/csrc/index.cpp
+++ b/thermite_amd/csrc/index.cpp
@@ -600,6 +600,30 @@
   return THM_OK;
 }
 
+int32_t thm_debug_host_table(const thm_index* ix, int32_t which, void* out, uint64_t cap, uint64_t* bytes) {
+  if (!ix || !bytes) return THM_ERR_INVALID_ARG;
+  const void* src = nullptr;
+  uint64_t have = 0;
+  auto pick = [&](const auto& v) {
+    src = v.data();
+    have = (uint64_t)v.size() * sizeof(v[0]);
+  };
+  switch (which) {
+    case 0: pick(ix->ref_bin); break;
+    case 1: ix->wide ? pick(ix->ref_recs64) : pick(ix->ref_recs); break;
+    case 2: pick(ix->exon_grid_off); break;
+    case 3: ix->wide ? pick(ix->exon_grid64) : pick(ix->exon_grid); break;
+    case 4: pick(ix->gene_grid_off); break;
+    case 5: ix->wide ? pick(ix->gene_grid64) : pick(ix->gene_grid); break;
+    default: return THM_ERR_INVALID_ARG;
+  }
+  *bytes = have;
+  if (!out) return THM_OK;
+  if (cap < have) return THM_ERR_INVALID_ARG;
+  if (have) memcpy(out, src, have);
+  return THM_OK;
+}
+
 uint64_t thm_index_text_len(const thm_index* ix) { return ix ? ix->n : 0; }
 const uint32_t* thm_index_suffix_array(const thm_index* ix) { return (ix && !ix->wide) ? ix->sa.data() : nullptr; }
 
diff --git a/thermite_amd/csrc/kernels_finish.hip b/thermite_amd/csrc/kernels_finish.hip
--- /dev/null
+++ b/thermite_amd/csrc/kernels_finish.hip
@@ -0,0 +1,138 @@
+#include <hip/hip_runtime.h>
+
+#include "launch.h"
+#include "smem_finish.h"
+
+namespace thm {
+namespace dev {
+
+constexpr int FIN_SLOTS = THM_N_COUNTERS + 4;
+
+template <class C>
+__global__ __launch_bounds__(256) void smem_finish_kernel(FinishParamsT<C> p) {
+  __shared__ unsigned long long part[FIN_SLOTS];
+  if (*p.fault_seed != 0) {
+    if (threadIdx.x < 4) p.stats[(size_t)blockIdx.x * 4 + threadIdx.x] = 0;
+    return;
+  }
+  if (threadIdx.x < FIN_SLOTS) part[threadIdx.x] = 0;
+  __syncthreads();
+  fin::Tables<C> tb;
+  tb.ref_bin = p.ix.ref_bin;
+  tb.ref_recs = p.ix.ref_recs;
+  tb.n_refs = p.ix.n_refs;
+  tb.exon_grid_off = p.ix.exon_grid_off;
+  tb.exon_grid = p.ix.exon_grid;
+  tb.gene_grid_off = p.ix.gene_grid_off;
+  tb.gene_grid = p.ix.gene_grid;
+  unsigned k_reads = 0, k_alns = 0, k_type[3] = {0, 0, 0}, k_calls = 0, k_opb = 0, k_win = 0, k_st[4] = {0, 0, 0, 0};
+  const uint64_t n = p.reads.n_reads, step = (uint64_t)gridDim.x * 256;
+  for (uint64_t r = (uint64_t)blockIdx.x * 256 + threadIdx.x; r < n; r += step) {
+    const ReadRecT<C> rec = p.recs[r];
+    if (rec.len == 0 || rec.len > p.max_read_len) continue;
+    if (rec.cand_off + (uint64_t)rec.n_hits > p.cand_cap) continue;
+    const int L = (int)rec.len;
+    const uint64_t occ0 = (uint64_t)(rec.hi0 - rec.lo0);
+    fin::Outcome o;
+    o.what = fin::LEAVE;
+    o.shape = fin::SHAPE_NONE;
+    if ((p.classes & fin::CLASS_E) && fin::shape_exact(rec.smem_cnt, rec.n_hits, rec.qpos0, rec.len0, occ0, rec.len)) {
+      o = fin::finish_exact<C>(tb, rec.sa0, L, fin::setup(p.opts, L, p.max_bw, (int)p.cpl), p.run_half);
+    } else if ((p.classes & fin::CLASS_S) && rec.smem_cnt == 2 && rec.n_hits == 2 && occ0 == 1) {
+      const SmemT<C> s1 = p.smems[rec.smem_off + 1];
+      if (s1.hi > s1.lo && s1.hi - s1.lo == 1) {
+        fin::Hit<C> h1, h2;
+        h1.hr = rec.sa0;
+        h1.q = rec.qpos0;
+        h1.len = rec.len0;
+        h2.hr = p.ix.sa[s1.hi - 1];
+        h2.q = s1.qpos;
+        h2.len = s1.len;
+        int sp = 0;
+        C a0 = 0;
+        if (fin::shape_subst<C>(rec.smem_cnt, rec.n_hits, 1, 1, h1, h2, rec.len, sp, a0))
+          o = fin::finish_subst<C>(tb, p.reads.bases + rec.base_off, h1, h2, L, sp, a0, fin::setup(p.opts, L, p.max_bw, (int)p.cpl), p.run_half);
+      }
+    }
+    if (o.shape != fin::SHAPE_NONE) k_st[2 * (o.shape - 1) + (o.what == fin::FINISHED ? 0 : 1)]++;
+    if (o.what != fin::FINISHED) continue;
+    if (o.accepted) {
+      Cand cd;
+      cd.ystart = o.ystart;
+      cd.yend = o.yend;
+      cd.ylen = o.ylen;
+      cd.tx_ystart = o.tx_ystart;
+      cd.tx_yend = o.tx_yend;
+      cd.tx_ylen = o.tx_ylen;
+      cd.ops_off = o.ops_off;
+      cd.tx_ops_off = o.tx_ops_off;
+      cd.score = o.score;
+      cd.ref_id = o.ref_id;
+      cd.xstart = 0;
+      cd.xend = rec.len;
+      cd.ops_len = rec.len;
+      const bool exonic = o.aln_type == THM_ALN_EXONIC;
+      cd.tx_ops_len = exonic ? rec.len : 0u;
+      cd.tx_or_gene_idx = o.type_idx;
+      cd.tx_score = exonic ? o.score : 0;
+      cd.tx_xstart = 0;
+      cd.tx_xend = exonic ? rec.len : 0u;
+      cd.name_rank = o.name_rank;
+      cd.strand = o.strand;
+      cd.aln_type = o.aln_type;
+      cd.primary = 0;
+      cd.pad_ = 0;
+      p.cands[rec.cand_off] = cd;
+      p.order[2 * rec.cand_off] = 0;
+      k_alns++;
+      k_type[0] += o.aln_type == THM_ALN_EXONIC;
+      k_type[1] += o.aln_type == THM_ALN_INTRONIC;
+      k_type[2] += o.aln_type == THM_ALN_INTERGENIC;
+      k_opb += o.op_bytes;
+    }
+    p.read_n_alns[r] = (uint32_t)o.accepted;
+    p.read_op_bytes[r] = o.accepted ? (uint64_t)o.op_bytes : 0ull;
+    p.recs[r].len = fin::MARK;
+    k_reads++;
+    k_calls += o.calls;
+    k_win += o.window_bytes;
+  }
+  unsigned v[11] = {k_reads, k_alns, k_type[0], k_type[1], k_type[2], k_calls, k_opb, k_win, k_st[0], k_st[1], k_st[2]};
+  unsigned v11 = k_st[3];
+#pragma unroll
+  for (int o = 32; o > 0; o >>= 1) {
+#pragma unroll
+    for (int k = 0; k < 11; k++) v[k] += __shfl_xor(v[k], o);
+    v11 += __shfl_xor(v11, o);
+  }
+  if ((threadIdx.x & 63u) == 0) {
+    const int slot[11] = {THM_CNT_READS, THM_CNT_ALNS, THM_CNT_EXONIC, THM_CNT_INTRONIC, THM_CNT_INTERGENIC, THM_CNT_SWG_CALLS,
+                          THM_CNT_OP_BYTES, THM_CNT_WINDOW_BYTES, THM_N_COUNTERS + 0, THM_N_COUNTERS + 1, THM_N_COUNTERS + 2};
+#pragma unroll
+    for (int k = 0; k < 11; k++)
+      if (v[k]) atomicAdd(&part[slot[k]], (unsigned long long)v[k]);
+    if (v11) atomicAdd(&part[THM_N_COUNTERS + 3], (unsigned long long)v11);
+  }
+  __syncthreads();
+  if (threadIdx.x < THM_N_COUNTERS) {
+    unsigned long long w = part[threadIdx.x];
+    if (threadIdx.x == THM_CNT_ALIGNED) w = part[THM_CNT_ALNS];
+    if (threadIdx.x == THM_CNT_UNMAPPED) w = part[THM_CNT_READS] - part[THM_CNT_ALNS];
+    if (w) p.rows[(size_t)blockIdx.x * THM_N_COUNTERS + threadIdx.x] = w;
+  } else if (threadIdx.x < FIN_SLOTS) {
+    p.stats[(size_t)blockIdx.x * 4 + (threadIdx.x - THM_N_COUNTERS)] = part[threadIdx.x];
+  }
+}
+
+}
+
+template <class C>
+static hipError_t launch_smem_finish_t(const FinishParamsT<C>& p, int n_blocks, hipStream_t s) {
+  if (n_blocks <= 0 || p.reads.n_reads == 0) return hipSuccess;
+  hipLaunchKernelGGL(dev::smem_finish_kernel<C>, dim3((unsigned)n_blocks), dim3(256), 0, s, p);
+  return hipGetLastError();
+}
+hipError_t launch_smem_finish(const FinishParamsT<uint32_t>& p, int n_blocks, hipStream_t s) { return launch_smem_finish_t(p, n_blocks, s); }
+hipError_t launch_smem_finish(const FinishParamsT<uint64_t>& p, int n_blocks, hipStream_t s) { return launch_smem_finish_t(p, n_blocks, s); }
+
+}
diff --git a/thermite_amd/csrc/kernels_seed.hip b/thermite_amd/csrc/kernels_seed.hip
--- a/thermite_amd/csrc/kernels_seed.hip
+++ b/thermite_amd/csrc/kernels_seed.hip
@@ -878,6 +878,7 @@
 __global__ __launch_bounds__(256) void plan_pack_kernel(PlanParams p, PackParamsT<C> q) {
   const uint64_t r = (uint64_t)blockIdx.x * 256 + threadIdx.x;
   const bool active = r < p.n_reads;
+  if (r == 0 && p.ops_start) *p.ops_cursor = p.ops_start;
   uint64_t b0 = 0, L = 0, hits = 0;
   if (active) {
     b0 = p.offsets[r];
diff --git a/thermite_amd/csrc/launch.h b/thermite_amd/csrc/launch.h
--- a/thermite_amd/csrc/launch.h
+++ b/thermite_amd/csrc/launch.h
@@ -138,6 +138,8 @@
   int32_t* read_status;
   uint32_t* read_n_alns;
   uint64_t* read_op_bytes;
+  unsigned long long* ops_cursor;
+  uint64_t ops_start;
 };
 
 template <class C>
@@ -266,6 +268,29 @@
 inline bool team_fits_lds(size_t lds4) { return lds4 / 4 * TEAM_WAVES + TEAM_STATIC_LDS + 256 <= EXTEND_LDS_LIMIT; }
 hipError_t launch_extend(const ExtendParamsT<uint32_t>& p, int cpl, int n_blocks, hipStream_t s, bool team = false);
 hipError_t launch_extend(const ExtendParamsT<uint64_t>& p, int cpl, int n_blocks, hipStream_t s, bool team = false);
+template <class C>
+struct FinishParamsT {
+  DeviceIndexT<C> ix;
+  ReadBatch reads;
+  thm_align_opts opts;
+  const SmemT<C>* smems;
+  ReadRecT<C>* recs;
+  Cand* cands;
+  uint64_t cand_cap;
+  uint32_t* order;
+  uint32_t* read_n_alns;
+  uint64_t* read_op_bytes;
+  unsigned long long* rows;
+  unsigned long long* stats;
+  const int* fault_seed;
+  uint32_t max_read_len, max_bw, cpl;
+  uint32_t classes;
+  uint32_t run_half;
+};
+hipError_t launch_smem_finish(const FinishParamsT<uint32_t>& p, int n_blocks, hipStream_t s);
+hipError_t launch_smem_finish(const FinishParamsT<uint64_t>& p, int n_blocks, hipStream_t s);
+constexpr int FINISH_BLOCKS_PER_CU = 8;
+
 enum : uint16_t {
   SK_EMPTY = 0,
   SK_SINGLE = 1,
diff --git a/thermite_amd/csrc/pipeline.hip b/thermite_amd/csrc/pipeline.hip
--- a/thermite_amd/csrc/pipeline.hip
+++ b/thermite_amd/csrc/pipeline.hip
@@ -4,6 +4,7 @@
 #include <cstring>
 
 #include "aligner_internal.h"
+#include "smem_finish.h"
 
 using namespace thm;
 
@@ -281,12 +282,36 @@
   const int dpt_blocks = tpr ? a->n_cu * dpt_per_cu : 0;
   const int bail_blocks = tpr ? std::min(ext_blocks, a->n_cu) : 0;
   const uint64_t tpr_rows = (uint64_t)ctl_blocks + (uint64_t)bail_blocks * 4;
-  const uint64_t n_rows = main_rows + team_rows + slow_waves + tpr_rows;
+  const int fin_blocks = (!tpr && a->fin_run_classes && n > 0) ? (int)std::min<uint64_t>((n + 255) / 256, (uint64_t)a->n_cu * FINISH_BLOCKS_PER_CU) : 0;
+  a->fin_blocks = (uint32_t)fin_blocks;
+  const uint64_t n_rows = main_rows + team_rows + slow_waves + tpr_rows + (uint64_t)fin_blocks;
   HIPCHK(a, a->e_wcnt.ensure(n_rows * THM_N_COUNTERS * 8 + 64));
   if (a->wcnt_clean_cap != a->e_wcnt.cap) HIPCHK(a, hipMemsetAsync(a->e_wcnt.p, 0, a->e_wcnt.cap, s));
   a->wcnt_clean_cap = 0;
   ep.wave_counters = a->e_wcnt.as<unsigned long long>();
   ep.skip_scan = 0;
+  FinishParamsT<C> fp;
+  if (fin_blocks) {
+    HIPCHK(a, a->e_finstats.ensure((size_t)fin_blocks * 4 * 8));
+    fp.ix = ep.ix;
+    fp.reads = ep.reads;
+    fp.opts = ep.opts;
+    fp.smems = ep.smems;
+    fp.recs = a->e_recs.as<ReadRecT<C>>();
+    fp.cands = ep.cands;
+    fp.cand_cap = ep.cand_cap;
+    fp.order = ep.order;
+    fp.read_n_alns = ep.read_n_alns;
+    fp.read_op_bytes = ep.read_op_bytes;
+    fp.rows = ep.wave_counters + (main_rows + team_rows + slow_waves + tpr_rows) * THM_N_COUNTERS;
+    fp.stats = a->e_finstats.as<unsigned long long>();
+    fp.fault_seed = ep.fault_seed;
+    fp.max_read_len = ep.max_read_len;
+    fp.max_bw = ep.max_bw;
+    fp.cpl = (uint32_t)cpl;
+    fp.classes = a->fin_run_classes;
+    fp.run_half = a->ops_run_half;
+  }
   if (tpr) {
     const uint64_t rec_cap = std::min<uint64_t>(4 * n + 65536, 64ull << 20);
     HIPCHK(a, a->t_memos.ensure(n * sizeof(ReadMemo) + 64));
@@ -413,6 +438,7 @@
     tp.list_only = 1;
     tp.wave_counters = ep.wave_counters + main_rows * THM_N_COUNTERS;
     tp.trace_scratch = ep.trace_scratch + main_trace_waves * trace_per_wave / 8;
+    if (fin_blocks) HIPCHK(a, launch_smem_finish(fp, fin_blocks, s));
     HIPCHK(a, hipEventRecord(a->ev_fork, s));
     HIPCHK(a, launch_extend(tp, cpl, a->n_cu, s, true));
     HIPCHK(a, hipStreamWaitEvent(a->stream2, a->ev_fork, 0));
@@ -420,6 +446,7 @@
     HIPCHK(a, hipEventRecord(a->ev_join, a->stream2));
     HIPCHK(a, hipStreamWaitEvent(s, a->ev_join, 0));
   } else {
+    if (fin_blocks) HIPCHK(a, launch_smem_finish(fp, fin_blocks, s));
     HIPCHK(a, launch_extend(ep, cpl, ext_blocks, s));
   }
   if (cls.n_slow || retry_possible) {
@@ -467,7 +494,7 @@
   HIPCHK(a, a->e_aln_off.ensure((n + 2) * 8));
   HIPCHK(a, a->e_ops_off.ensure((n + 2) * 8));
   HIPCHK(a, a->o_alns.ensure(a->cand_cap * sizeof(thm_aln)));
-  HIPCHK(a, a->o_ops.ensure(a->cand_ops_cap + 64));
+  HIPCHK(a, a->o_ops.ensure(a->cand_ops_cap + 2 * a->n_bases + 64));
   HIPCHK(a, a->s_heavy.ensure((n + 1) * 8));
   HIPCHK(a, a->s_slow.ensure((n + 1) * 8));
   HIPCHK(a, a->s_team.ensure((n + 1) * 8));
@@ -478,6 +505,19 @@
   a->n_slow_host = cls.n_slow;
   a->fast_max_len = cls.fast_max;
   a->slow_max_len = cls.slow_max;
+  const bool run_valid = a->ops_run_half > 0 && a->ops_run_ptr == a->e_ops.p && a->ops_run_cap == a->e_ops.cap;
+  if (!run_valid) a->ops_run_half = 0;
+  const bool fin_wanted = !a->use_tpr && a->fin_classes && cls.fast_len > 0;
+  if (fin_wanted && a->ops_run_half < cls.fast_len && fin::run_bytes(cls.fast_len) <= a->cand_ops_cap) {
+    HIPCHK(a, hipMemsetAsync(a->e_ops.p, THM_OP_MATCH, fin::run_bytes(cls.fast_len), s));
+    HIPCHK(a, hipMemsetAsync(a->e_ops.as<uint8_t>() + cls.fast_len, THM_OP_SUBST, 1, s));
+    a->ops_run_ptr = a->e_ops.p;
+    a->ops_run_cap = a->e_ops.cap;
+    a->ops_run_half = cls.fast_len;
+  }
+  if (a->ops_run_half && fin::run_bytes(a->ops_run_half) > a->cand_ops_cap) a->ops_run_half = 0;
+  const uint64_t ops_start = a->ops_run_half ? fin::run_bytes(a->ops_run_half) : 0;
+  a->fin_run_classes = (fin_wanted && a->ops_run_half >= cls.fast_len) ? a->fin_classes : 0;
   PlanParams pp;
   pp.offsets = a->r_offsets.as<uint64_t>();
   pp.read_hits = a->s_hits.as<uint64_t>();
@@ -498,6 +538,8 @@
   pp.read_status = a->r_status.as<int32_t>();
   pp.read_n_alns = a->e_nalns.as<uint32_t>();
   pp.read_op_bytes = a->e_opbytes.as<uint64_t>();
+  pp.ops_cursor = a->d_cursors.as<unsigned long long>() + 1;
+  pp.ops_start = ops_start;
   rc = a->dix->wide ? enqueue_plan_pack_t<uint64_t>(a, pp) : enqueue_plan_pack_t<uint32_t>(a, pp);
   if (rc != THM_OK) return rc;
   HIPCHK(a, hipEventRecord(a->ev[2], s));
@@ -523,7 +565,7 @@
   cp.ops = a->o_ops.as<uint8_t>();
   cp.fault = a->d_fault.as<int>();
   cp.alns_cap = a->cand_cap;
-  cp.ops_cap = a->cand_ops_cap;
+  cp.ops_cap = a->cand_ops_cap + 2 * a->n_bases;
   cp.heavy_cap = a->cand_cap / 2 + 16;
   cp.heavy_cnt = a->d_cursors.as<unsigned long long>() + 2;
   cp.heavy_list = a->e_heavy.as<uint64_t>();
diff --git a/thermite_amd/csrc/smem_finish.h b/thermite_amd/csrc/smem_finish.h
--- /dev/null
+++ b/thermite_amd/csrc/smem_finish.h
@@ -0,0 +1,418 @@
+#ifndef THERMITE_SMEM_FINISH_H
+#define THERMITE_SMEM_FINISH_H
+#include <cstdint>
+
+#include "thermite_internal.h"
+
+#if defined(__HIPCC__)
+#define FIN_HD __host__ __device__ inline
+#define FIN_UNROLL _Pragma("unroll")
+#else
+#define FIN_HD inline
+#define FIN_UNROLL
+#endif
+
+namespace thm {
+namespace fin {
+
+constexpr uint32_t CLASS_E = 1u, CLASS_S = 2u;
+constexpr uint32_t MARK = 0xFFFFFFFFu;
+constexpr uint32_t MAX_GRID = 32;
+constexpr uint32_t MAX_RANGE = 1u << 20;
+
+enum : int { LEAVE = 0, FINISHED = 1 };
+enum : int { SHAPE_NONE = 0, SHAPE_E = 1, SHAPE_S = 2 };
+
+FIN_HD uint64_t run_bytes(uint32_t half) { return ((uint64_t)2 * half + 1 + 15) & ~15ull; }
+
+struct Outcome {
+  int what;
+  int shape;
+  int accepted;
+  uint64_t ystart, yend, ylen;
+  uint64_t tx_ystart, tx_yend, tx_ylen;
+  uint32_t ops_off, tx_ops_off;
+  int32_t score;
+  uint32_t ref_id, name_rank, type_idx;
+  uint8_t strand, aln_type;
+  uint32_t calls, window_bytes, op_bytes;
+};
+
+struct Setup {
+  int min_aln_score, band, x_drop, range;
+  bool intron_mode;
+  bool ok;
+};
+FIN_HD Setup setup(const thm_align_opts& o, int L, uint32_t max_bw, int cpl) {
+  Setup s;
+  const float prod = o.min_aln_score_percent * (float)L;
+  const int ms_pct = (prod != prod) ? 0 : (prod >= 2147483648.0f ? 2147483647 : (prod <= -2147483648.0f ? (-2147483647 - 1) : (int)prod));
+  s.min_aln_score = ms_pct > o.min_aln_score ? ms_pct : o.min_aln_score;
+  s.band = (s.min_aln_score < 0) ? 0 : (L - s.min_aln_score > 0 ? L - s.min_aln_score : 0);
+  s.x_drop = s.band;
+  s.range = (int)(o.multimap_score_range > MAX_RANGE ? MAX_RANGE : o.multimap_score_range);
+  s.intron_mode = o.intron_mode != 0;
+  s.ok = o.multimap_score_range <= MAX_RANGE && !((uint32_t)s.band > max_bw || (cpl > 0 && 2 * s.band + 1 > 64 * cpl));
+  return s;
+}
+
+template <class C>
+FIN_HD uint32_t ref_of(uint32_t bin_first, const RefRecT<C>* ref_recs, uint32_t n_refs, C idx, RefRecT<C>& r) {
+  uint32_t lo = bin_first;
+  r = ref_recs[lo];
+  while (r.end <= idx && lo + 1 < n_refs) {
+    lo++;
+    r = ref_recs[lo];
+  }
+  return lo;
+}
+
+template <class C>
+FIN_HD bool genome_window(C hr, int len, int L, int bw, const RefRecT<C>& ref, C a0, uint32_t& bytes) {
+  if (a0 < ref.start || ref.end < 1 || (uint64_t)a0 + (uint64_t)L > (uint64_t)ref.end - 1) return false;
+  if (sizeof(C) == 4 && (uint64_t)hr + (uint64_t)(len + L + bw) > 0x7fffffffull) return false;
+  const int64_t h = (int64_t)hr, ext = (int64_t)(L + bw);
+  int64_t seq_start = h > ext ? h - ext : 0;
+  if (seq_start < (int64_t)ref.start) seq_start = (int64_t)ref.start;
+  int64_t seq_end = h + (int64_t)len + ext;
+  if (seq_end > (int64_t)ref.end - 1) seq_end = (int64_t)ref.end - 1;
+  bytes = (uint32_t)(seq_end - seq_start);
+  return true;
+}
+
+template <class C>
+FIN_HD bool by_coords(const ExonEntryT<C>& e, C qs, C a0, int L) {
+  return e.prev_end <= qs && e.start <= a0 && (uint64_t)a0 + (uint64_t)L <= (uint64_t)e.end;
+}
+template <class C>
+FIN_HD uint32_t tx_window_bytes(const ExonEntryT<C>& e, C hr, int len, int L, int bw) {
+  const int tr = (int)(hr - e.start) + (int)e.txoff, tlen = (int)e.seq_len;
+  const int ws = (tr > L + bw) ? tr - (L + bw) : 0;
+  const int we = (tlen < tr + len + L + bw + 1) ? tlen : tr + len + L + bw + 1;
+  return (uint32_t)(we - ws);
+}
+
+template <class C>
+FIN_HD int grid_rank(C start, C end, uint32_t rank, C qs, C qe, uint32_t b0) {
+  const bool overlap = qs < end && start < qe;
+  const uint32_t sb = (uint32_t)(start >> GRID_SHIFT), home = b0 > sb ? b0 : sb;
+  const bool primary = (rank & 0xffu) == (home & 0xffu);
+  return (overlap && primary) ? (int)(rank >> 8) : -1;
+}
+
+struct GridSpan {
+  uint32_t e0, cnt;
+};
+template <class C>
+FIN_HD GridSpan grid_span(const uint32_t* off, C qs, C qe) {
+  const uint32_t b0 = (uint32_t)(qs >> GRID_SHIFT), b1 = (uint32_t)((qe > qs ? qe - 1 : qs) >> GRID_SHIFT);
+  GridSpan g;
+  g.e0 = off[b0];
+  g.cnt = off[b1 + 1] - g.e0;
+  return g;
+}
+
+template <class C>
+struct ExonScan {
+  C qs, qe;
+  uint32_t b0;
+  int bw, bw_n;
+  uint32_t n, win_all, win_all_n;
+  int best;
+  bool all_by_coords;
+  bool first_by_coords;
+  uint32_t first_win;
+  C first_start, first_end;
+  uint32_t first_value, first_txoff, first_seq_len;
+};
+template <class C>
+FIN_HD void scan_begin(ExonScan<C>& s, C qs, C qe, int bw, int bw_n) {
+  s.qs = qs;
+  s.qe = qe;
+  s.b0 = (uint32_t)(qs >> GRID_SHIFT);
+  s.bw = bw;
+  s.bw_n = bw_n;
+  s.n = s.win_all = s.win_all_n = 0;
+  s.best = 0x7fffffff;
+  s.all_by_coords = true;
+  s.first_by_coords = false;
+  s.first_win = 0;
+  s.first_start = s.first_end = 0;
+  s.first_value = s.first_txoff = s.first_seq_len = 0;
+}
+template <class C>
+FIN_HD void scan_visit(ExonScan<C>& s, const ExonEntryT<C>& e, C a0, int L) {
+  const int r = grid_rank<C>(e.start, e.end, e.rank, s.qs, s.qe, s.b0);
+  if (r < 0) return;
+  s.n++;
+  const bool ok = by_coords<C>(e, s.qs, a0, L);
+  const int len = (int)(s.qe - s.qs);
+  uint32_t w = 0;
+  if (ok) {
+    w = tx_window_bytes<C>(e, s.qs, len, L, s.bw);
+    s.win_all += w;
+    s.win_all_n += tx_window_bytes<C>(e, s.qs, len, L, s.bw_n);
+  } else {
+    s.all_by_coords = false;
+  }
+  if (r < s.best) {
+    s.best = r;
+    s.first_by_coords = ok;
+    s.first_win = w;
+    s.first_start = e.start;
+    s.first_end = e.end;
+    s.first_value = e.value;
+    s.first_txoff = e.txoff;
+    s.first_seq_len = e.seq_len;
+  }
+}
+template <class C>
+FIN_HD bool exon_scan(const ExonEntryT<C>* grid, const GridSpan& g, C a0, int L, ExonScan<C>& s1, ExonScan<C>* s2) {
+  if (g.cnt > MAX_GRID) return false;
+  for (uint32_t i = 0; i < g.cnt; i += 4) {
+    ExonEntryT<C> e[4];
+    FIN_UNROLL
+    for (uint32_t k = 0; k < 4; k++) e[k] = grid[g.e0 + (i + k < g.cnt ? i + k : g.cnt - 1)];
+    FIN_UNROLL
+    for (uint32_t k = 0; k < 4; k++) {
+      if (i + k < g.cnt) {
+        scan_visit<C>(s1, e[k], a0, L);
+        if (s2) scan_visit<C>(*s2, e[k], a0, L);
+      }
+    }
+  }
+  return true;
+}
+template <class C>
+FIN_HD int gene_first(const GridEntryT<C>* grid, const GridSpan& g, C qs, C qe, uint32_t& gene) {
+  if (g.cnt > MAX_GRID) return -1;
+  const uint32_t b0 = (uint32_t)(qs >> GRID_SHIFT);
+  int best = 0x7fffffff;
+  for (uint32_t i = 0; i < g.cnt; i += 4) {
+    GridEntryT<C> e[4];
+    FIN_UNROLL
+    for (uint32_t k = 0; k < 4; k++) e[k] = grid[g.e0 + (i + k < g.cnt ? i + k : g.cnt - 1)];
+    FIN_UNROLL
+    for (uint32_t k = 0; k < 4; k++) {
+      const int r = (i + k < g.cnt) ? grid_rank<C>(e[k].start, e[k].end, e[k].rank, qs, qe, b0) : -1;
+      if (r >= 0 && r < best) {
+        best = r;
+        gene = e[k].value;
+      }
+    }
+  }
+  return best != 0x7fffffff ? 1 : 0;
+}
+
+template <class C>
+FIN_HD void fill_record(Outcome& o, C a0, int L, int sc, int p, uint32_t half, const RefRecT<C>& ref, uint32_t ref_id,
+                        bool exonic, const ExonScan<C>& e, bool have_gene, uint32_t gene) {
+  const bool fwd = ref.strand != 0;
+  const C cy0 = a0, cy1 = (C)(a0 + (C)L);
+  if (fwd) {
+    o.ystart = (uint64_t)(C)(cy0 - ref.start);
+    o.yend = (uint64_t)(C)(cy1 - ref.start);
+  } else {
+    o.ystart = (uint64_t)(C)(ref.len - (C)(cy1 - ref.start));
+    o.yend = (uint64_t)(C)(ref.len - (C)(cy0 - ref.start));
+  }
+  o.ylen = ref.len;
+  o.score = sc;
+  o.ref_id = ref_id;
+  o.name_rank = ref.name_rank;
+  o.strand = fwd ? 1 : 0;
+  const int pg = (p < 0) ? -1 : (fwd ? p : L - 1 - p);
+  o.ops_off = (pg < 0) ? 0u : half - (uint32_t)pg;
+  o.tx_ops_off = 0;
+  o.tx_ystart = o.tx_yend = o.tx_ylen = 0;
+  o.op_bytes = (uint32_t)L;
+  if (exonic) {
+    o.aln_type = THM_ALN_EXONIC;
+    o.type_idx = e.first_value;
+    o.tx_ystart = (uint64_t)(a0 - e.first_start) + e.first_txoff;
+    o.tx_yend = o.tx_ystart + (uint64_t)L;
+    o.tx_ylen = e.first_seq_len;
+    o.tx_ops_off = (p < 0) ? 0u : half - (uint32_t)p;
+    o.op_bytes = 2u * (uint32_t)L;
+  } else if (have_gene) {
+    o.aln_type = THM_ALN_INTRONIC;
+    o.type_idx = gene;
+  } else {
+    o.aln_type = THM_ALN_INTERGENIC;
+    o.type_idx = THM_NO_IDX;
+  }
+}
+
+template <class C>
+struct Tables {
+  const uint32_t* ref_bin;
+  const RefRecT<C>* ref_recs;
+  uint32_t n_refs;
+  const uint32_t* exon_grid_off;
+  const ExonEntryT<C>* exon_grid;
+  const uint32_t* gene_grid_off;
+  const GridEntryT<C>* gene_grid;
+};
+
+FIN_HD bool shape_exact(uint32_t smem_cnt, uint32_t n_hits, uint32_t qpos0, uint32_t len0, uint64_t occ0, uint32_t L) {
+  return smem_cnt == 1 && n_hits == 1 && occ0 == 1 && qpos0 == 0 && len0 == L && L > 0;
+}
+
+template <class C>
+FIN_HD Outcome finish_exact(const Tables<C>& ix, C hr, int L, const Setup& st, uint32_t half) {
+  Outcome o;
+  o.what = LEAVE;
+  o.shape = SHAPE_E;
+  o.accepted = 0;
+  o.calls = o.window_bytes = o.op_bytes = 0;
+  if (!st.ok || (uint32_t)L > half) return o;
+  const C qe = (C)(hr + (C)L);
+  const uint32_t bin_first = ix.ref_bin[hr >> GRID_SHIFT];
+  const GridSpan es = grid_span<C>(ix.exon_grid_off, hr, qe);
+  GridSpan gs;
+  gs.e0 = gs.cnt = 0;
+  if (st.intron_mode) gs = grid_span<C>(ix.gene_grid_off, hr, qe);
+  RefRecT<C> ref;
+  const uint32_t ref_id = ref_of<C>(bin_first, ix.ref_recs, ix.n_refs, hr, ref);
+  ExonScan<C> e;
+  scan_begin<C>(e, hr, qe, st.band, st.band);
+  if (!exon_scan<C>(ix.exon_grid, es, hr, L, e, nullptr)) return o;
+  uint32_t gwin = 0;
+  if (!genome_window<C>(hr, L, L, st.band, ref, hr, gwin)) return o;
+  o.calls = 2;
+  o.window_bytes = gwin;
+  const bool exonic = e.n > 0;
+  if (exonic) {
+    if (!e.first_by_coords) return o;
+    o.calls += 2;
+    o.window_bytes += e.first_win;
+  }
+  const bool accept = (st.intron_mode || exonic) && L >= st.min_aln_score && L >= st.min_aln_score - st.range;
+  uint32_t gene = 0;
+  bool have_gene = false;
+  if (accept && !exonic) {
+    const int g = gene_first<C>(ix.gene_grid, gs, hr, qe, gene);
+    if (g < 0) return o;
+    have_gene = g > 0;
+  }
+  o.what = FINISHED;
+  if (accept) {
+    o.accepted = 1;
+    fill_record<C>(o, hr, L, L, -1, half, ref, ref_id, exonic, e, have_gene, gene);
+  }
+  return o;
+}
+
+template <class C>
+struct Hit {
+  C hr;
+  uint32_t q, len;
+};
+template <class C>
+FIN_HD bool shape_subst(uint32_t smem_cnt, uint32_t n_hits, uint64_t occ1, uint64_t occ2, const Hit<C>& h1, const Hit<C>& h2, uint32_t L,
+                        int& p, C& a0) {
+  if (smem_cnt != 2 || n_hits != 2 || occ1 != 1 || occ2 != 1) return false;
+  const bool first_is_a = h1.q == 0;
+  const Hit<C>& A = first_is_a ? h1 : h2;
+  const Hit<C>& B = first_is_a ? h2 : h1;
+  if (A.q != 0 || A.len == 0 || B.q != A.len + 1 || B.len == 0 || B.q + B.len != L) return false;
+  if (B.hr <= A.hr || (uint64_t)(B.hr - A.hr) != (uint64_t)A.len + 1) return false;
+  p = (int)A.len;
+  a0 = A.hr;
+  return true;
+}
+FIN_HD bool is_acgt(uint8_t b) { return b == 'A' || b == 'C' || b == 'G' || b == 'T'; }
+
+struct SubstState {
+  int bw, xd, max_score;
+  uint32_t calls, win, n_acc;
+};
+template <class C>
+FIN_HD bool subst_hit(const Hit<C>& h, C a0, int L, const RefRecT<C>& ref, const Setup& st, SubstState& ss, const ExonScan<C>& scan, bool narrowed,
+                      bool& acc) {
+  const int sc = L - 2;
+  if (ss.xd < 1) return false;
+  uint32_t gwin = 0;
+  if (!genome_window<C>(h.hr, (int)h.len, L, ss.bw, ref, a0, gwin)) return false;
+  if (!scan.all_by_coords) return false;
+  ss.calls += 2 + 2 * scan.n;
+  ss.win += gwin + (narrowed ? scan.win_all_n : scan.win_all);
+  const bool exonic = scan.n > 0;
+  acc = (st.intron_mode || exonic) && sc >= st.min_aln_score && sc >= ss.max_score - st.range;
+  if (acc) {
+    ss.n_acc++;
+    const int lim = L + st.range - sc > 0 ? L + st.range - sc : 0;
+    ss.bw = ss.bw < lim ? ss.bw : lim;
+    ss.xd = ss.xd < lim ? ss.xd : lim;
+    ss.max_score = ss.max_score > sc ? ss.max_score : sc;
+  }
+  return true;
+}
+
+template <class C>
+FIN_HD Outcome finish_subst(const Tables<C>& ix, const uint8_t* rd, const Hit<C>& h1, const Hit<C>& h2, int L, int p, C a0, const Setup& st,
+                            uint32_t half) {
+  Outcome o;
+  o.what = LEAVE;
+  o.shape = SHAPE_S;
+  o.accepted = 0;
+  o.calls = o.window_bytes = o.op_bytes = 0;
+  if (!st.ok || (uint32_t)L > half) return o;
+  if (L - p < 3 || p + 1 < 3) return o;
+  const uint8_t c = rd[p];
+  if (!is_acgt(c)) return o;
+  {
+    int t = p + 1;
+    while (t < L && rd[t] == c) t++;
+    if (t == L) return o;
+    t = p - 1;
+    while (t >= 0 && rd[t] == c) t--;
+    if (t < 0) return o;
+  }
+  const C ae = (C)(a0 + (C)L);
+  const uint32_t bin_first = ix.ref_bin[h1.hr >> GRID_SHIFT];
+  const GridSpan es = grid_span<C>(ix.exon_grid_off, a0, ae);
+  GridSpan gs;
+  gs.e0 = gs.cnt = 0;
+  if (st.intron_mode) gs = grid_span<C>(ix.gene_grid_off, a0, ae);
+  RefRecT<C> ref;
+  const uint32_t ref_id = ref_of<C>(bin_first, ix.ref_recs, ix.n_refs, h1.hr, ref);
+  SubstState ss;
+  ss.bw = st.band;
+  ss.xd = st.x_drop;
+  ss.max_score = st.min_aln_score;
+  ss.calls = ss.win = ss.n_acc = 0;
+  const int sc = L - 2;
+  const int lim = 2 + st.range;
+  const int bw_n = st.band < lim ? st.band : lim;
+  ExonScan<C> s1, s2;
+  scan_begin<C>(s1, h1.hr, (C)(h1.hr + (C)h1.len), st.band, st.band);
+  scan_begin<C>(s2, h2.hr, (C)(h2.hr + (C)h2.len), st.band, bw_n);
+  if (!exon_scan<C>(ix.exon_grid, es, a0, L, s1, &s2)) return o;
+  bool acc1 = false, acc2 = false;
+  if (!subst_hit<C>(h1, a0, L, ref, st, ss, s1, false, acc1)) return o;
+  if (!subst_hit<C>(h2, a0, L, ref, st, ss, s2, acc1, acc2)) return o;
+  const uint32_t n_acc = ss.n_acc;
+  if (s1.n != s2.n || acc1 != acc2) return o;
+  const bool exonic = s1.n > 0;
+  if (exonic && (s1.best != s2.best || s1.first_start != s2.first_start || s1.first_end != s2.first_end || s1.first_value != s2.first_value)) return o;
+  uint32_t gene = 0;
+  bool have_gene = false;
+  if (n_acc && !exonic) {
+    const int g = gene_first<C>(ix.gene_grid, gs, a0, ae, gene);
+    if (g < 0) return o;
+    have_gene = g > 0;
+  }
+  o.what = FINISHED;
+  o.calls = ss.calls;
+  o.window_bytes = ss.win;
+  if (n_acc) {
+    o.accepted = 1;
+    fill_record<C>(o, a0, L, sc, p, half, ref, ref_id, exonic, s1, have_gene, gene);
+  }
+  return o;
+}
+
+}
+}
+#endif
```

New measurement: 93.85 million (median of 6 runs). 4.1% higher.
